# ivclab/CPG

Measured on AMD Instinct MI355X. Metric: images/sec per CPG train-prune-retrain cycle, VGG16 task-1, higher is better.
Workload: dtype f32; 1 GPU; configs[1]: VGG16-BN custom_vgg 224x224, task-1 CPG cycle (finetune -> prune 0.0->0.1 -> recovery, validate after every 20th train step), batch 256 per GPU; task=1, arch=vgg16, global_batch=256, per_gpu_batch=256, parallelism=dp1, epoch_steps=20

## Files before the change

### cpg_amd/_lib.py

```python
import ctypes
import os
import sys

import torch

_HERE = os.path.dirname(os.path.abspath(__file__))
LIB_PATH = os.environ.get('CPG_HIP_LIB') or os.path.join(_HERE, 'lib', 'libcpg_hip.so')

ABI_VERSION = 3
CPG_OK = 0
CPG_E_KRANGE = 2
CPG_E_INVALID = -1
MODE_FINETUNE = 0
MODE_PRUNE = 1



class ConvDesc(ctypes.Structure):
    _fields_ = [(n, ctypes.c_int32) for n in
                ('N', 'C', 'H', 'W', 'K', 'R', 'S', 'stride_h', 'stride_w', 'pad_h', 'pad_w', 'dil_h', 'dil_w', 'groups')]


class PruneResult(ctypes.Structure):
    _fields_ = [('n_candidates', ctypes.c_int64), ('k', ctypes.c_int64), ('n_released', ctypes.c_int64),
# ... 26 lines not shown
assert ctypes.sizeof(ResampleItem) == ctypes.sizeof(TensorItem) == 48

_vp, _int, _i32, _i64, _sz, _f32, _f64 = (ctypes.c_void_p, ctypes.c_int, ctypes.c_int32, ctypes.c_int64, ctypes.c_size_t, ctypes.c_float,
                                         ctypes.c_double)
_desc = ctypes.POINTER(ConvDesc)
_SIGNATURES = {
    'cpg_version': (_int, []),
    'cpg_set_shared_chip_hint': (_int, [_i32]),
    'cpg_get_shared_chip_hint': (_i32, []),
    'cpg_set_option': (_int, [ctypes.c_char_p, _i32]),
    'cpg_get_option': (_int, [ctypes.c_char_p, ctypes.POINTER(_i32)]),
    'cpg_last_error': (ctypes.c_char_p, []),
    'cpg_binarize_mask_weight': (_int, [_vp, _vp, _f32, _vp, _i64, _vp]),
    'cpg_conv2d_workspace_bytes': (_sz, [_desc]),
    'cpg_conv2d_fwd': (_int, [_desc, _vp, _vp, _vp, _f32, _vp, _vp, _vp, _sz, _vp]),
    'cpg_conv2d_dgrad': (_int, [_desc, _vp, _vp, _vp, _f32, _vp, _vp, _sz, _vp]),
    'cpg_conv2d_dgrad_add_supported': (_i32, [_desc]),
    'cpg_conv2d_dgrad_add': (_int, [_desc, _vp, _vp, _vp, _f32, _vp, _vp, _vp, _sz, _vp]),
    'cpg_conv2d_wgrad': (_int, [_desc, _vp, _vp, _vp, _vp, _f32, _vp, _vp, _vp, _vp, _sz, _vp]),
    'cpg_conv2d_pack_bytes': (_sz, [_desc, _i32]),
    'cpg_conv2d_pack': (_int, [_desc, _vp, _vp, _f32, _i32, _vp, _sz, _i32, _vp, _sz, _vp]),
    'cpg_conv2d_use_packed': (_int, [_vp, _sz]),
    'cpg_bn_relu_bwd_reduce': (_int, [_vp] * 9 + [_i32] * 3 + [_vp, _sz, _vp]),
    'cpg_conv2d_wgrad_rider_supported': (_i32, [_desc]),
    'cpg_conv2d_wgrad_attach_bn_bwd': (_int, [_vp] * 4 + [_i32] * 3),
    'cpg_linear_workspace_bytes': (_sz, [_i32, _i32, _i32]),
    'cpg_linear_fwd': (_int, [_vp, _vp, _vp, _f32, _vp, _vp, _i32, _i32, _i32, _vp, _sz, _vp]),
    'cpg_linear_dgrad': (_int, [_vp, _vp, _vp, _f32, _vp, _i32, _i32, _i32, _vp, _sz, _vp]),
    'cpg_linear_wgrad': (_int, [_vp, _vp, _vp, _vp, _f32, _vp, _vp, _vp, _i32, _i32, _i32, _vp, _sz, _vp]),
    'cpg_route_grads': (_int, [_vp, _vp, _vp, _i32, _f32, _vp, _i32, _i64, _vp]),
    'cpg_rank_prune_workspace_bytes': (_sz, []),
    'cpg_rank_prune': (_int, [_vp, _vp, _i32, _f64, _i64, _vp, _vp, _sz, _vp]),
    'cpg_rank_prune_zero': (_int, [_vp, _vp, _i32, _f64, _i64, _vp, _vp, _sz, _vp]),
    'cpg_mask_hist': (_int, [_vp, _vp, _i32, _i64, _vp, _vp]),
    'cpg_apply_mask': (_int, [_vp, _vp, _i32, _i64, _vp]),
    'cpg_zero_pruned': (_int, [_vp, _vp, _i64, _vp]),
    'cpg_claim_free': (_int, [_vp, _i32, _i64, _vp]),
    'cpg_owned_num_blocks': (_i64, [_i64]),
    'cpg_owned_block_counts': (_int, [_vp, _i32, _i32, _i64, _vp, _vp]),
    'cpg_pack_owned': (_int, [_vp, _vp, _i32, _i32, _i64, _vp, _vp, _vp]),
    'cpg_unpack_owned': (_int, [_vp, _vp, _i32, _i32, _i64, _vp, _vp, _vp]),
    'cpg_sgd_route_step': (_int, [_vp, _vp, _vp, _vp, _i32, _f32, _f32, _f32, _i32, _i32, _i64, _vp]),
    'cpg_multi_tensor_max': (_i32, []),
    'cpg_sgd_route_step_multi': (_int, [ctypes.POINTER(SgdItem), _i32, _i32, _f32, _f32, _f32, _i32, _i32, _vp]),
    'cpg_adam_route_step_multi': (_int, [ctypes.POINTER(AdamItem), _i32, _i32, _i32, _f64, _f64, _f64, _f64, _i32, _vp]),
    'cpg_sgd_route_zero_step': (_int, [_vp, _vp, _vp, _vp, _i32, _f32, _f32, _f32, _i32, _i32, _i64, _vp]),
    'cpg_sgd_route_zero_step_multi': (_int, [ctypes.POINTER(SgdItem), _i32, _i32, _f32, _f32, _f32, _i32, _i32, _vp]),
    'cpg_adam_route_step': (_int, [_vp, _vp, _vp, _vp, _vp, _i32, _i32, _f64, _f64, _f64, _f64, _i32, _i64, _vp]),
    'cpg_bn_workspace_bytes': (_sz, [_i32, _i32, _i32]),
    'cpg_bn_relu_fwd_train': (_int, [_vp, _vp, _vp, _f32, _f32, _vp, _vp, _vp, _vp, _vp, _i32, _i32, _i32, _i32, _vp, _sz, _vp]),
    'cpg_bn_relu_fwd_eval': (_int, [_vp, _vp, _vp, _vp, _vp, _vp, _i32, _i32, _i32, _i32, _vp]),
    'cpg_bn_relu_pool_fwd': (_int, [_vp, _vp, _vp, _f32, _f32, _vp, _vp, _vp, _vp, _vp, _i32, _i32, _i32, _i32, _i32, _vp, _sz, _vp]),
    'cpg_bn_relu_pool_bwd': (_int, [_vp, _vp, _vp, _vp, _vp, _vp, _vp, _vp, _vp, _i32, _i32, _i32, _i32, _i32, _vp, _sz, _vp]),
    'cpg_bn_relu_bwd': (_int, [_vp, _vp, _vp, _vp, _vp, _vp, _vp, _vp, _vp, _i32, _i32, _i32, _i32, _i32, _vp, _sz, _vp]),
    'cpg_conv2d_winograd': (_i32, [_desc, _i32]),
    'cpg_conv2d_bnstats_tiles': (_i32, [_desc]),
    'cpg_conv2d_fwd_bnstats': (_int, [_desc, _vp, _vp, _vp, _f32, _vp, _vp, _vp, _sz, _vp, _sz, _vp]),
    'cpg_conv2d_fwd_bn_eval_supported': (_i32, [_desc]),
    'cpg_conv2d_fwd_bn_eval': (_int, [_desc, _vp, _vp, _vp, _f32, _vp, _vp, _vp, _vp, _vp, _f32, _i32, _vp, _vp, _vp, _sz, _vp]),
    'cpg_conv2d_bf16_supported': (_i32, [_desc]),
    'cpg_conv2d_bf16_workspace_bytes': (_sz, [_desc]),
    'cpg_conv2d_fwd_bf16': (_int, [_desc, _vp, _vp, _vp, _f32, _vp, _vp, _vp, _sz, _vp]),
    'cpg_conv2d_wgrad_bf16_supported': (_i32, [_desc]),
    'cpg_conv2d_wgrad_bf16_workspace_bytes': (_sz, [_desc]),
    'cpg_conv2d_wgrad_bf16': (_int, [_desc, _vp, _vp, _vp, _vp, _f32, _vp, _vp, _vp, _sz, _vp]),
    'cpg_conv2d_fwd_bf16x3': (_int, [_desc, _vp, _vp, _vp, _f32, _vp, _vp, _vp, _sz, _vp]),
    'cpg_conv2d_dgrad_bf16x3': (_int, [_desc, _vp, _vp, _vp, _f32, _vp, _vp, _sz, _vp]),
    'cpg_conv2d_wgrad_bf16x3': (_int, [_desc, _vp, _vp, _vp, _vp, _f32, _vp, _vp, _vp, _sz, _vp]),
    'cpg_conv2d_dgrad_bf16': (_int, [_desc, _vp, _vp, _vp, _f32, _vp, _vp, _sz, _vp]),
    'cpg_conv2d_dgrad_bnbwd_tiles': (_i32, [_desc]),
    'cpg_conv2d_dgrad_bnbwd': (_int, [_desc, _vp, _vp, _vp, _f32, _vp, _vp, _vp, _vp, _vp, _vp, _vp, _sz, _vp, _sz, _vp]),
    'cpg_bn_bwd_from_partials': (_int, [_vp, _i32, _vp, _vp, _vp, _vp, _vp, _vp, _vp, _vp, _vp, _i32, _i32, _i32, _vp, _sz, _vp]),
    'cpg_bn_bwd_finalize_partials': (_int, [_vp, _i32, _i32, _i32, _i32, _vp, _vp, _vp, _vp]),
    'cpg_stem_bn_supported': (_i32, [_desc]),
    'cpg_stem_bn_tiles': (_i32, [_desc]),
    'cpg_stem_bn_stats': (_int, [_desc, _vp, _vp, _vp, _f32, _vp, _vp, _sz, _vp]),
    'cpg_stem_bn_relu_fwd': (_int, [_desc, _vp, _vp, _vp, _f32, _vp, _vp, _vp, _vp, _vp, _vp, _vp]),
    'cpg_stem_bn_relu_bwd_reduce': (_int, [_desc, _vp, _vp, _vp, _f32, _vp, _vp, _vp, _vp, _vp, _vp, _vp, _sz, _vp]),
    'cpg_stem_bn_relu_bwd_apply': (_int, [_desc, _vp, _vp, _vp, _f32, _vp, _vp, _vp, _vp, _vp, _vp, _vp, _vp, _vp]),
    'cpg_stem_bn_wgrad_workspace': (_sz, [_desc]),
    'cpg_stem_bn_relu_bwd_wgrad': (_int, [_desc, _vp, _vp, _vp, _f32, _vp, _vp, _vp, _vp, _vp, _vp, _vp, _vp, _vp, _vp, _sz, _vp]),
    'cpg_bn_stats_finalize_count': (_int, [_vp, _i32, _i32, _i32, _i32, _f32, _f32, _vp, _vp, _vp, _vp, _vp, _vp]),
    'cpg_bn_stats_finalize': (_int, [_vp, _i32, _i32, _i32, _i32, _f32, _f32, _vp, _vp, _vp, _vp, _vp]),
    'cpg_bn_add_relu_mask_bytes': (_sz, [_i32, _i32, _i32]),
    'cpg_bn_add_relu_fwd': (_int, [_vp, _vp, _vp, _vp, _f32, _f32, _vp, _vp, _vp, _vp, _vp, _i32, _i32, _i32, _i32, _vp, _sz, _vp, _vp]),
    'cpg_bn_relu_pool3_supported': (_i32, [_i32, _i32]),
    'cpg_bn_relu_pool3_fwd': (_int, [_vp] * 6 + [_i32] * 4 + [_vp]),
    'cpg_bn_relu_pool3_bwd': (_int, [_vp] * 9 + [_i32] * 5 + [_vp, _sz, _vp]),
    'cpg_bn_add_relu_bwd': (_int, [_vp] * 11 + [_i32] * 4 + [_vp, _sz, _vp, _vp]),
    'cpg_prelu_fwd': (_int, [_vp, _vp, _vp, _vp, _i32, _i32, _i32, _i32, _vp]),
    'cpg_prelu_bwd_bias': (_int, [_vp] * 6 + [_i32] * 4 + [_vp, _sz, _vp]),
    'cpg_prelu_workspace_bytes': (_sz, [_i32, _i32, _i32]),
    'cpg_prelu_bwd': (_int, [_vp, _vp, _vp, _vp, _vp, _i32, _i32, _i32, _i32, _vp, _sz, _vp]),
    'cpg_image_resample_workspace_bytes': (_sz, [ctypes.POINTER(ResampleItem), _i32]),
    'cpg_image_resample': (_int, [_vp, _i64, ctypes.POINTER(ResampleItem), _i32, _vp, _i64, _vp, _sz, _vp]),
    'cpg_image_to_tensor': (_int, [_vp, _i64, ctypes.POINTER(TensorItem), _i32, _i32, _i32, ctypes.POINTER(_f32), ctypes.POINTER(_f32), _vp,
                                           _i64, _vp]),
    'cpg_pair_distance': (_int, [_vp, _i64, _vp, _i64, _i64, _i32, _i32, _vp, _vp, _vp]),
    'cpg_pair_sweep': (_int, [_vp, _vp, _i64, ctypes.POINTER(_f64), _i32, _i32, _vp, _vp, _vp]),
    'cpg_loss_heads_workspace_bytes': (_sz, [_i32, _i32, _i32]),
    'cpg_softmax_xent_fwd': (_int, [_vp, _vp, _vp, _i32, _i32, _vp, _vp, _vp, _sz, _vp]),
    'cpg_softmax_xent_fwd_bwd': (_int, [_vp, _vp, _vp, _vp, _i32, _i32, _vp, _vp, _vp, _vp, _sz, _vp]),
    'cpg_angle_head_fwd': (_int, [_vp, _vp, _vp, _i32, _i32, _i32, _i32, _f32, _f64] + [_vp] * 7 + [_sz, _vp]),
    'cpg_angle_head_bwd': (_int, [_vp] * 7 + [_i32, _i32, _i32, _i32, _f32, _f64, _vp, _vp, _vp, _sz, _vp]),
}
EXPORTS = tuple(_SIGNATURES)
# ... 116 lines not shown
```

### cpg_amd/csrc/bn_kernels.hip

```cpp
#include "cpg_common.h"

using namespace cpg;

namespace {

constexpr int kThreads = 256;

struct BnDims {
    int N, C, HW;
    int slices;
    int imgs_per_slice;
};

__device__ __forceinline__ double block_sum(double v, double *red) {
    for (int off = 32; off > 0; off >>= 1) v += __shfl_down(v, off);
    const int w = threadIdx.x >> 6, l = threadIdx.x & 63;
    __syncthreads();
    if (l == 0) red[w] = v;
    __syncthreads();
    return red[0] + red[1] + red[2] + red[3];
}

template <class F, class FL>
__device__ __forceinline__ void walk_planes(int P, int n0, int n1, F &&f, FL &&flush) {
// ... 513 lines not shown
    float *coef = (float *)(partial + (size_t)C * d.slices * 2);
    hipLaunchKernelGGL(k_bn_bwd_reduce<true>, dim3(C, d.slices), dim3(kThreads), 0, stream, x, gy, d, mean, invstd, gamma, beta, partial);
    hipLaunchKernelGGL(k_bn_bwd_finalize, dim3((C + 63) / 64), dim3(64), 0, stream, partial, d, dgamma, dbeta, coef, table, mean, invstd,
                       gamma, beta);
    CPG_CHECK_LAUNCH("cpg_bn_relu_bwd_reduce");
    return CPG_OK;
}

extern "C" int cpg_bn_add_relu_bwd(const float *x, const float *out, const float *gy, const float *gamma, const float *beta,
                                   const float *mean, const float *invstd, float *gx, float *gz, float *dgamma, float *dbeta, int32_t N,
                                   int32_t C, int32_t HW, int32_t train, void *ws, size_t ws_bytes, void *stream_v, const uint8_t *relu_mask) {
    BnDims d;
    int rc = make_dims(N, C, HW, d);
    if (rc) return rc;
    CPG_REQUIRE(x && (out || relu_mask) && gy && gamma && beta && mean && invstd && gx && gz && dgamma && dbeta && ws, "cpg_bn_add_relu_bwd: null pointer");
    if (relu_mask != nullptr)
        CPG_REQUIRE(HW % 4 == 0 && ((((uintptr_t)x) | ((uintptr_t)gy) | ((uintptr_t)gz)) & 15) == 0,
                    "cpg_bn_add_relu_bwd: the ReLU mask needs 4 | HW and 16-byte aligned tensors");
    if (ws_bytes < cpg_bn_workspace_bytes(N, C, HW)) return fail(CPG_E_WORKSPACE, "cpg_bn_add_relu_bwd: workspace too small");
    hipStream_t stream = (hipStream_t)stream_v;
    double *partial = (double *)ws;
    float *coef = (float *)(partial + (size_t)C * d.slices * 2);
    hipLaunchKernelGGL((k_bn_bwd_reduce<false, true>), dim3(C, d.slices), dim3(kThreads), 0, stream, x, gy, d, mean, invstd, gamma, beta,
                       partial, out, gz, relu_mask);
    hipLaunchKernelGGL(k_bn_bwd_finalize, dim3((C + 63) / 64), dim3(64), 0, stream, partial, d, dgamma, dbeta, coef);
    if (train) launch_bwd_apply<false, true>(d, x, gz, gx, mean, invstd, gamma, beta, coef, stream);
    else launch_bwd_apply<false, false>(d, x, gz, gx, mean, invstd, gamma, beta, coef, stream);
    CPG_CHECK_LAUNCH("cpg_bn_add_relu_bwd");
    return CPG_OK;
}

namespace {

struct PoolDims {
    int H, W, OW, wins;
};

struct Win {
    float v[4];
};
__device__ __forceinline__ Win load_win(const float *plane, int W, int pr, int pc) {
    const float2 a = *reinterpret_cast<const float2 *>(plane + (2 * pr) * W + 2 * pc);
    const float2 b = *reinterpret_cast<const float2 *>(plane + (2 * pr + 1) * W + 2 * pc);
    return Win{{a.x, a.y, b.x, b.y}};
}
__device__ __forceinline__ int win_argmax(const float (&y)[4]) {
    int idx = 0;
#pragma unroll
    for (int k = 1; k < 4; ++k)
        if (y[k] > y[idx]) idx = k;
    return idx;
}

template <int GROUP>
__global__ __launch_bounds__(kThreads) void k_bnp_apply(const float *__restrict__ x, float *__restrict__ yp, BnDims d, PoolDims p,
                                                        const float *__restrict__ mean, const float *__restrict__ invstd,
                                                        const float *__restrict__ gamma, const float *__restrict__ beta) {
    const int64_t planes = (int64_t)d.N * d.C;
    const int gl = threadIdx.x % GROUP;
    const int64_t g0 = (int64_t)blockIdx.x * (kThreads / GROUP) + threadIdx.x / GROUP;
    const int64_t gstride = (int64_t)gridDim.x * (kThreads / GROUP);
    for (int64_t pl = g0; pl < planes; pl += gstride) {
        const int c = (int)(pl % d.C);
        const float m = mean[c], is = invstd[c], ga = gamma[c], be = beta[c];
        const float *plane = x + pl * d.HW;
        float *out = yp + pl * p.wins;
        for (int i = gl; i < p.wins; i += GROUP) {
            const int pr = i / p.OW, pc = i - pr * p.OW;
            const Win w = load_win(plane, p.W, pr, pc);
            float best = 0.0f;
#pragma unroll
            for (int k = 0; k < 4; ++k) best = fmaxf(best, bn_affine(w.v[k], m, is, ga, be));
            out[i] = best;
        }
    }
}

__global__ __launch_bounds__(kThreads) void k_bnp_bwd_reduce(const float *__restrict__ x, const float *__restrict__ gp, BnDims d,
                                                             PoolDims p, const float *__restrict__ mean,
                                                             const float *__restrict__ invstd, const float *__restrict__ gamma,
                                                             const float *__restrict__ beta, double *__restrict__ partial) {
    __shared__ double red[4];
    const int c = blockIdx.x, s = blockIdx.y;
    const int n0 = s * d.imgs_per_slice, n1 = min(d.N, n0 + d.imgs_per_slice);
    const float m = mean[c], is = invstd[c], ga = gamma[c], be = beta[c];
    double dsg = 0.0, dsgx = 0.0;
    float sg = 0.f, sgx = 0.f;
    walk_planes(p.wins, n0, n1, [&](int n, int wi) {
        const int pr = wi / p.OW, pc = wi - pr * p.OW;
        const int64_t pl = (int64_t)n * d.C + c;
        const Win w = load_win(x + pl * d.HW, p.W, pr, pc);
        const float g = gp[pl * p.wins + wi];
        float y[4];
#pragma unroll
        for (int k = 0; k < 4; ++k) y[k] = bn_affine(w.v[k], m, is, ga, be);
        const int idx = win_argmax(y);
        if (y[idx] > 0.f) {
            sg += g;
            sgx += g * ((w.v[idx] - m) * is);
        }
    }, [&]() {
        dsg += (double)sg; dsgx += (double)sgx; sg = 0.f; sgx = 0.f;
    });
    const double t0 = block_sum(dsg, red);
    const double t1 = block_sum(dsgx, red);
    if (threadIdx.x == 0) {
        partial[((int64_t)c * d.slices + s) * 2 + 0] = t0;
        partial[((int64_t)c * d.slices + s) * 2 + 1] = t1;
    }
}

template <bool TRAIN, int GROUP>
__global__ __launch_bounds__(kThreads) void k_bnp_bwd_apply(const float *__restrict__ x, const float *__restrict__ gp,
                                                            float *__restrict__ gx, BnDims d, PoolDims p,
                                                            const float *__restrict__ mean, const float *__restrict__ invstd,
                                                            const float *__restrict__ gamma, const float *__restrict__ beta,
                                                            const float *__restrict__ coef) {
    const int64_t planes = (int64_t)d.N * d.C;
    const int gl = threadIdx.x % GROUP;
    const int64_t g0 = (int64_t)blockIdx.x * (kThreads / GROUP) + threadIdx.x / GROUP;
    const int64_t gstride = (int64_t)gridDim.x * (kThreads / GROUP);
    for (int64_t pl = g0; pl < planes; pl += gstride) {
        const int c = (int)(pl % d.C);
        const float m = mean[c], is = invstd[c], ga = gamma[c], be = beta[c];
        const float mg = TRAIN ? coef[2 * c] : 0.f, mgx = TRAIN ? coef[2 * c + 1] : 0.f;
        const float scale = is * ga;
        const float *plane = x + pl * d.HW;
        float *gplane = gx + pl * d.HW;
        for (int i = gl; i < p.wins; i += GROUP) {
            const int pr = i / p.OW, pc = i - pr * p.OW;
            const Win w = load_win(plane, p.W, pr, pc);
            float y[4], r[4];
#pragma unroll
            for (int k = 0; k < 4; ++k) y[k] = bn_affine(w.v[k], m, is, ga, be);
            const int idx = win_argmax(y);
            const float g = (y[idx] > 0.f) ? gp[pl * p.wins + i] : 0.f;
#pragma unroll
            for (int k = 0; k < 4; ++k) {
                const float gk = (k == idx) ? g : 0.f;
                r[k] = TRAIN ? (gk - mg - ((w.v[k] - m) * is) * mgx) * scale : gk * scale;
            }
            *reinterpret_cast<float2 *>(gplane + (2 * pr) * p.W + 2 * pc) = make_float2(r[0], r[1]);
            *reinterpret_cast<float2 *>(gplane + (2 * pr + 1) * p.W + 2 * pc) = make_float2(r[2], r[3]);
        }
    }
}

int make_pool(int H, int W, PoolDims &p) {
    CPG_REQUIRE(H > 0 && W > 0 && (H % 2) == 0 && (W % 2) == 0, "bn_relu_pool: H and W must be even (got %d x %d)", H, W);
    p.H = H; p.W = W; p.OW = W / 2; p.wins = (H / 2) * (W / 2);
    return CPG_OK;
}
unsigned pool_grid(const BnDims &d, const PoolDims &p, bool wave) {
    int64_t groups = (int64_t)d.N * d.C;
    if (wave) groups = (groups + 3) / 4;
    const int64_t cap = (int64_t)kCUs * 16;
    return (unsigned)(groups < cap ? groups : cap);
}

}

extern "C" int cpg_bn_relu_pool_fwd(const float *x, const float *gamma, const float *beta, float eps, float momentum,
                                    float *running_mean, float *running_var, float *mean, float *invstd, float *y_pooled,
                                    int32_t N, int32_t C, int32_t H, int32_t W, int32_t train, void *ws, size_t ws_bytes,
                                    void *stream_v) {
    BnDims d;
    PoolDims p;
    int rc = make_dims(N, C, H * W, d);
    if (rc) return rc;
    rc = make_pool(H, W, p);
    if (rc) return rc;
    CPG_REQUIRE(x && gamma && beta && mean && invstd && y_pooled, "cpg_bn_relu_pool_fwd: null pointer");
    CPG_REQUIRE((((uintptr_t)x) & 7) == 0, "cpg_bn_relu_pool_fwd: x must be 8-byte aligned");
    hipStream_t stream = (hipStream_t)stream_v;
    if (train) {
        CPG_REQUIRE(ws != nullptr, "cpg_bn_relu_pool_fwd: workspace required in training mode");
        if (ws_bytes < cpg_bn_workspace_bytes(N, C, H * W)) return fail(CPG_E_WORKSPACE, "cpg_bn_relu_pool_fwd: workspace too small");
        double *partial = (double *)ws;
        hipLaunchKernelGGL(k_bn_stats, dim3(C, d.slices), dim3(kThreads), 0, stream, x, d, partial);
        hipLaunchKernelGGL(k_bn_finalize, dim3((C + 63) / 64), dim3(64), 0, stream, partial, d, eps, momentum, mean, invstd,
                           running_mean, running_var);
    }
    const bool wave = p.wins < 1024;
    if (wave)
        hipLaunchKernelGGL(k_bnp_apply<64>, dim3(pool_grid(d, p, true)), dim3(kThreads), 0, stream, x, y_pooled, d, p, mean, invstd, gamma, beta);
    else
        hipLaunchKernelGGL(k_bnp_apply<256>, dim3(pool_grid(d, p, false)), dim3(kThreads), 0, stream, x, y_pooled, d, p, mean, invstd, gamma, beta);
    CPG_CHECK_LAUNCH("cpg_bn_relu_pool_fwd");
    return CPG_OK;
}

extern "C" int cpg_bn_relu_pool_bwd(const float *x, const float *g_pooled, const float *gamma, const float *beta,
                                    const float *mean, const float *invstd, float *gx, float *dgamma, float *dbeta, int32_t N,
                                    int32_t C, int32_t H, int32_t W, int32_t train, void *ws, size_t ws_bytes, void *stream_v) {
    BnDims d;
    PoolDims p;
    int rc = make_dims(N, C, H * W, d);
    if (rc) return rc;
    rc = make_pool(H, W, p);
    if (rc) return rc;
    CPG_REQUIRE(x && g_pooled && gamma && beta && mean && invstd && gx && dgamma && dbeta && ws, "cpg_bn_relu_pool_bwd: null pointer");
    CPG_REQUIRE((((uintptr_t)x) & 7) == 0 && (((uintptr_t)gx) & 7) == 0, "cpg_bn_relu_pool_bwd: x / gx must be 8-byte aligned");
    if (ws_bytes < cpg_bn_workspace_bytes(N, C, H * W)) return fail(CPG_E_WORKSPACE, "cpg_bn_relu_pool_bwd: workspace too small");
    hipStream_t stream = (hipStream_t)stream_v;
    double *partial = (double *)ws;
    float *coef = (float *)(partial + (size_t)C * d.slices * 2);
    hipLaunchKernelGGL(k_bnp_bwd_reduce, dim3(C, d.slices), dim3(kThreads), 0, stream, x, g_pooled, d, p, mean, invstd, gamma, beta, partial);
    hipLaunchKernelGGL(k_bn_bwd_finalize, dim3((C + 63) / 64), dim3(64), 0, stream, partial, d, dgamma, dbeta, coef);
    const bool wave = p.wins < 1024;
    const dim3 grid(pool_grid(d, p, wave)), block(kThreads);
    if (wave && train) hipLaunchKernelGGL((k_bnp_bwd_apply<true, 64>), grid, block, 0, stream, x, g_pooled, gx, d, p, mean, invstd, gamma, beta, coef);
    else if (wave) hipLaunchKernelGGL((k_bnp_bwd_apply<false, 64>), grid, block, 0, stream, x, g_pooled, gx, d, p, mean, invstd, gamma, beta, coef);
    else if (train) hipLaunchKernelGGL((k_bnp_bwd_apply<true, 256>), grid, block, 0, stream, x, g_pooled, gx, d, p, mean, invstd, gamma, beta, coef);
    else hipLaunchKernelGGL((k_bnp_bwd_apply<false, 256>), grid, block, 0, stream, x, g_pooled, gx, d, p, mean, invstd, gamma, beta, coef);
    CPG_CHECK_LAUNCH("cpg_bn_relu_pool_bwd");
    return CPG_OK;
}


namespace {

struct Pool3Dims {
    int H, W, OH, OW;
    int strips;
};
constexpr int kPool3SR = 8;

__device__ __forceinline__ void pool3_stage(const float *__restrict__ plane, float *zs, const Pool3Dims &p, int r0, int nrows, float m,
                                            float is, float ga, float be) {
    const int h0 = 2 * r0 - 1;
    const int lo = max(h0, 0), hi = min(h0 + nrows, p.H);
    const float *src = plane + lo * p.W;
    float *dst = zs + (lo - h0) * p.W;
    const int n = (hi - lo) * p.W;
    if ((n & 3) == 0 && (((uintptr_t)src) & 15) == 0 && (((lo - h0) * p.W) & 3) == 0) {
        for (int i = threadIdx.x; i < n / 4; i += kThreads) {
            float4 v = reinterpret_cast<const float4 *>(src)[i];
            v.x = fmaxf(bn_affine(v.x, m, is, ga, be), 0.f); v.y = fmaxf(bn_affine(v.y, m, is, ga, be), 0.f);
            v.z = fmaxf(bn_affine(v.z, m, is, ga, be), 0.f); v.w = fmaxf(bn_affine(v.w, m, is, ga, be), 0.f);
            reinterpret_cast<float4 *>(dst)[i] = v;
        }
    } else {
        for (int i = threadIdx.x; i < n; i += kThreads) dst[i] = fmaxf(bn_affine(src[i], m, is, ga, be), 0.f);
    }
}

__device__ __forceinline__ int pool3_argmax(const float *zs, const Pool3Dims &p, int h0, int ph, int pw, float *best_out = nullptr) {
    float best = -1.0f;
    int arg = 0;
#pragma unroll
    for (int r = 0; r < 3; ++r) {
        const int h = 2 * ph - 1 + r;
        if ((unsigned)h >= (unsigned)p.H) continue;
#pragma unroll
        for (int q = 0; q < 3; ++q) {
            const int w = 2 * pw - 1 + q;
            if ((unsigned)w >= (unsigned)p.W) continue;
            const float v = zs[(h - h0) * p.W + w];
            if (v > best || v != v) best = v, arg = h * p.W + w;
        }
    }
    if (best_out) *best_out = best;
    return arg;
}

__global__ __launch_bounds__(kThreads) void k_bnp3_apply(const float *__restrict__ x, float *__restrict__ y, BnDims d, Pool3Dims p,
                                                         const float *__restrict__ mean, const float *__restrict__ invstd,
                                                         const float *__restrict__ gamma, const float *__restrict__ beta) {
    extern __shared__ __attribute__((aligned(16))) float dyn[];
// ... 349 lines not shown
```

### cpg_amd/csrc/conv3x3_wino_wgrad.hip

```cpp
#include <algorithm>
#include "cpg_dispatch.h"
#include "wino_acc.h"

using namespace cpg;

namespace {

typedef float f32x2 __attribute__((ext_vector_type(2)));
typedef int i32x4 __attribute__((ext_vector_type(4)));
typedef int i32x2 __attribute__((ext_vector_type(2)));

constexpr int WW_XR = 34, WW_XC = 138, WW_GR = 30, WW_GC = 62;
constexpr int WW_XS = 32 * WW_XC;
constexpr int WW_STAGE = WW_XS + 32 * WW_GC;

struct WwGeom {
    int N, C, K, H, W;
    int th, tw, nseg;
    unsigned nstages;
    int nkb, ncb, nsplit;
    unsigned su;
    int span;
    int xcd;
};

struct WwRider {
    const float *y, *gz;
    float *gy;
    const float *table;
    int C, HW, p4, ipp;
    int bytes;
    unsigned total, per;
};

#ifdef WG_TIMING
__device__ unsigned long long ww_dbg[65536 * 8];
#define WW_STAMP(i) do { if (lane == 0 && u < 65536) ww_dbg[u * 8 + (i)] = wall_clock64(); } while (0)
#else
#define WW_STAMP(i)
#endif
template <bool NARROW, int GS = 0, int RI = 0>
__global__ __launch_bounds__(256) __attribute__((amdgpu_waves_per_eu(1, 1)))
void k_wgw(WwGeom g, const float *__restrict__ x, const float *__restrict__ gy, float *__restrict__ part, WwRider rd) {
    static_assert(GS == 0 || GS == 4 || (!NARROW && GS == 2), "shared staging: groups of 4 waves, or 2 on wide maps");
    static_assert(RI == 0 || (GS == 4 && RI <= 2), "the rider's schedule slots exist in the GS = 4 bodies: one or two items per stage");
    constexpr int NG = GS ? 4 / GS : 0;
    constexpr bool TS = GS == 4;
    constexpr int WW_BS = 2 * 16 * 64;
    __shared__ __attribute__((aligned(16))) float smem_all[GS ? NG * 2 * WW_XS + 4 * 32 * WW_GC + (TS ? WW_BS : 0) : 4 * WW_STAGE];
    const int tid = threadIdx.x, lane = tid & 63, wave = __builtin_amdgcn_readfirstlane(tid >> 6);
    const int li = lane & 31, lh = lane >> 5;
    const int gw = GS ? wave % GS : 0;
    float *smem = GS ? smem_all : smem_all + wave * WW_STAGE;
    float *xb0 = GS ? smem_all + (wave / (GS ? GS : 1)) * 2 * WW_XS : smem;
    float *xb1 = GS ? xb0 + WW_XS : smem;
    float *gyp = GS ? smem_all + NG * 2 * WW_XS + wave * 32 * WW_GC : smem + WW_XS;
    float *bsh = smem_all + NG * 2 * WW_XS + 4 * 32 * WW_GC;
    const int HW = g.H * g.W;
    const unsigned npairs = (unsigned)(g.nkb * g.ncb);
    const unsigned u = (g.xcd ? xcd_remap(blockIdx.x, gridDim.x) : blockIdx.x) * 4 + wave;
    if (u >= npairs * (unsigned)g.nsplit) return;
    const unsigned pair = u % npairs, split = u / npairs;
    const int kb = (int)(pair % (unsigned)g.nkb), cb = (int)(pair / (unsigned)g.nkb);
    const int k0 = __builtin_amdgcn_readfirstlane(min(kb * 32, g.K - 32)), c0 = __builtin_amdgcn_readfirstlane(min(cb * 32, g.C - 32));
    const unsigned s_begin = split * g.su;
    const int nst = (int)min(g.su, g.nstages - s_begin);
    WW_STAMP(0);
#ifdef WG_TIMING
    if (lane == 0 && u < 65536) ww_dbg[u * 8 + 6] = __builtin_amdgcn_s_getreg(63492), ww_dbg[u * 8 + 7] = __builtin_amdgcn_s_getreg(63508);
#endif
    const unsigned per_img = (unsigned)(g.th * g.nseg);
    int n = (int)(s_begin / per_img) * (NARROW ? 2 : 1);
    const unsigned r0 = s_begin % per_img;
    int ty = (int)(r0 / (unsigned)g.nseg), tseg = (int)(r0 % (unsigned)g.nseg);
    const int n0 = n;
    const int nimg_here = min(g.span, g.N - n0);
    const __amdgpu_buffer_rsrc_t srd_x = __builtin_amdgcn_make_buffer_rsrc(
        (void *)(x + (int64_t)n0 * g.C * HW - (g.W + 4)), 0, nimg_here * g.C * HW * 4 + (g.W + 4) * 4, 0x00020000);
    const __amdgpu_buffer_rsrc_t srd_g =
        __builtin_amdgcn_make_buffer_rsrc((void *)(gy + (int64_t)n0 * g.K * HW), 0, nimg_here * g.K * HW * 4, 0x00020000);

    constexpr int kOOR = (int)0x80000000;
    const int qd = min(lane & 7, 6), rem = lane >> 3;
    const int xrow = NARROW ? rem >> 1 : rem & 3, half = rem & 1;
    const int vx_const = NARROW ? (half * g.C * HW + xrow * g.W + gw * HW) * 4 + qd * 8 + 16
                                : ((rem >> 2) * HW + xrow * g.W + gw * 2 * HW) * 4 + qd * 16 + 16;
    const int vg_const = NARROW ? ((rem >> 2) * HW + half * g.K * HW + ((rem >> 1) & 1) * g.W) * 4 + qd * 8
                                : ((rem >> 1) * HW + (rem & 1) * g.W) * 4 + qd * 16;
    const int hside = lane & 1, hrow = (lane >> 1) & 3;
    const int vh_const = ((lane >> 3) * HW + hrow * g.W + gw * 8 * HW) * 4 + (hside ? 28 * 4 + 16 : 12);
    const int xw_addr = NARROW ? xrow * WW_XR + 16 * half + 2 + 2 * qd + gw * WW_XC : (rem >> 2) * WW_XC + xrow * WW_XR + 2 + 4 * qd + gw * 2 * WW_XC;
    const int gw_addr = NARROW ? (rem >> 2) * WW_GC + ((rem >> 1) & 1) * WW_GR + 14 * half + 2 * qd
                               : (rem >> 1) * WW_GC + (rem & 1) * WW_GR + 4 * qd;
    const int hw_addr = (lane >> 3) * WW_XC + hrow * WW_XR + (hside ? 30 : 1) + gw * 8 * WW_XC;
    if constexpr (NARROW) {
        for (int i = lane; i < 32 * 4 * 6; i += 64) {
            const int rowi = i / 6, col = i % 6;
            xb0[(rowi >> 2) * WW_XC + (rowi & 3) * WW_XR + (col >> 1) * 16 + (col & 1)] = 0.0f;
// ... 125 lines not shown
            const f32x2 own = *reinterpret_cast<const f32x2 *>(r);
            const f32x2 lo = *reinterpret_cast<const f32x2 *>(r - 2), hi = *reinterpret_cast<const f32x2 *>(r + 2);
            B[m * 4 + 0] = lo[1], B[m * 4 + 1] = own[0], B[m * 4 + 2] = own[1], B[m * 4 + 3] = hi[0];
        } else if (m == 4) {
            const f32x2 y0 = *reinterpret_cast<const f32x2 *>(gyp + gr_base + kKs * ks);
            const f32x2 y1 = *reinterpret_cast<const f32x2 *>(gyp + gr_base + kKs * ks + WW_GR);
            A[0] = y0[0], A[3] = y0[1], A[12] = y1[0], A[15] = y1[1];
        } else if (m < 7) {
#pragma unroll
            for (int j = 2 * (m - 5); j < 2 * (m - 5) + 2; ++j) {
                const float d0 = B[0 * 4 + j], d1 = B[1 * 4 + j], d2 = B[2 * 4 + j], d3 = B[3 * 4 + j];
                B[0 * 4 + j] = d0 - d2, B[1 * 4 + j] = d1 + d2, B[2 * 4 + j] = d2 - d1, B[3 * 4 + j] = d1 - d3;
                asm volatile("" : "+v"(B[0 * 4 + j]), "+v"(B[1 * 4 + j]), "+v"(B[2 * 4 + j]), "+v"(B[3 * 4 + j]));
            }
        } else if (m < 11) {
            const int i = m - 7;
            const float t0 = B[i * 4 + 0], t1 = B[i * 4 + 1], t2 = B[i * 4 + 2], t3 = B[i * 4 + 3];
            B[i * 4 + 0] = t0 - t2, B[i * 4 + 1] = t1 + t2, B[i * 4 + 2] = t2 - t1, B[i * 4 + 3] = t1 - t3;
            asm volatile("" : "+v"(B[i * 4 + 0]), "+v"(B[i * 4 + 1]), "+v"(B[i * 4 + 2]), "+v"(B[i * 4 + 3]));
        } else if (m == 11) {
            A[4] = A[0] + A[12], A[7] = A[3] + A[15], A[8] = A[0] - A[12], A[11] = A[3] - A[15];
            asm volatile("" : "+v"(A[4]), "+v"(A[7]), "+v"(A[8]), "+v"(A[11]));
        } else if (m == 12) {
            A[1] = A[0] + A[3], A[2] = A[0] - A[3], A[5] = A[4] + A[7], A[6] = A[4] - A[7];
            asm volatile("" : "+v"(A[1]), "+v"(A[2]), "+v"(A[5]), "+v"(A[6]));
        } else if (m == 13) {
            A[9] = A[8] + A[11], A[10] = A[8] - A[11], A[13] = A[12] + A[15], A[14] = A[12] - A[15];
            asm volatile("" : "+v"(A[9]), "+v"(A[10]), "+v"(A[13]), "+v"(A[14]));
        }
    };

    const int b_ra = wave == 0 ? 0 : (wave == 2 ? 2 : 1), b_rb = wave == 3 ? 3 : (wave == 2 ? 1 : 2);
    const float b_sg = wave == 1 ? 1.0f : -1.0f;
    float ta[4], tb[4];
    auto b_micro = [&](int m, int ks, int buf, float (&B)[16], const float *xb) {
        if (m < 2) {
            const float *r = xb + xr_base + kKs * ks + (m == 0 ? b_ra : b_rb) * WW_XR;
            const f32x2 own = *reinterpret_cast<const f32x2 *>(r);
            const f32x2 lo = *reinterpret_cast<const f32x2 *>(r - 2), hi = *reinterpret_cast<const f32x2 *>(r + 2);
            float (&t)[4] = m == 0 ? ta : tb;
            t[0] = lo[1], t[1] = own[0], t[2] = own[1], t[3] = hi[0];
        } else if (m == 2) {
            float e[4];
#pragma unroll
            for (int j = 0; j < 4; ++j) e[j] = __builtin_fmaf(b_sg, tb[j], ta[j]);
            f32x4 v;
            v[0] = e[0] - e[2], v[1] = e[1] + e[2], v[2] = e[2] - e[1], v[3] = e[1] - e[3];
            *reinterpret_cast<f32x4 *>(bsh + ((buf * 4 + wave) * 64 + lane) * 4) = v;
        } else {
            const f32x4 v = *reinterpret_cast<const f32x4 *>(bsh + ((buf * 4 + (m - 3)) * 64 + lane) * 4);
            B[(m - 3) * 4 + 0] = v[0], B[(m - 3) * 4 + 1] = v[1], B[(m - 3) * 4 + 2] = v[2], B[(m - 3) * 4 + 3] = v[3];
        }
    };
    constexpr int RJ = RI > 0 ? RI : 1;
    typedef const float __attribute__((address_space(4))) *ww_cptr;
    const __amdgpu_buffer_rsrc_t srd_ry = __builtin_amdgcn_make_buffer_rsrc((void *)rd.y, 0, rd.bytes, 0x00020000);
    const __amdgpu_buffer_rsrc_t srd_rz = __builtin_amdgcn_make_buffer_rsrc((void *)rd.gz, 0, rd.bytes, 0x00020000);
    const __amdgpu_buffer_rsrc_t srd_ro = __builtin_amdgcn_make_buffer_rsrc((void *)rd.gy, 0, rd.bytes, 0x00020000);
    unsigned rq = 0, rq_end = 0, r_plane = 0;
    int r_sub = 0, r_c = 0;
    if constexpr (RI > 0) {
        rq = __builtin_amdgcn_readfirstlane(min(u * rd.per, rd.total));
        rq_end = min(rq + rd.per, rd.total);
        r_plane = rq / (unsigned)rd.ipp, r_sub = (int)(rq % (unsigned)rd.ipp), r_c = (int)(r_plane % (unsigned)rd.C);
    }
    f32x4 r_y[RJ], r_z[RJ];
    float r_t[RJ][7];
    int r_vo[RJ], r_so[RJ];
    auto r_micro = [&](int j, int m) {
        if (m == 0) {
            const int left = rq < rq_end ? rd.p4 - r_sub * 64 : 0;
            r_vo[j] = lane < left ? lane * 16 : kOOR;
            r_so[j] = (int)(r_plane * (unsigned)rd.HW + (unsigned)r_sub * 256u) * 4;
            r_y[j] = __builtin_bit_cast(f32x4, __builtin_amdgcn_raw_buffer_load_b128(srd_ry, r_vo[j], r_so[j], 0));
        } else if (m == 1) {
            r_z[j] = __builtin_bit_cast(f32x4, __builtin_amdgcn_raw_buffer_load_b128(srd_rz, r_vo[j], r_so[j], 0));
            ww_cptr t = (ww_cptr)rd.table + r_c * 8;
#pragma unroll
            for (int k = 0; k < 7; ++k) r_t[j][k] = t[k];
            if (rq < rq_end) {
                ++rq;
                if (++r_sub == rd.ipp) {
                    r_sub = 0, ++r_plane;
                    if (++r_c == rd.C) r_c = 0;
                }
            }
        } else {
            const int e = m - 2;
            r_y[j][e] = bn_bwd_apply_one<true, true>(r_y[j][e], r_z[j][e], r_t[j][0], r_t[j][1], r_t[j][2], r_t[j][3], r_t[j][4], r_t[j][5], r_t[j][6]);
            if (m == 5) __builtin_amdgcn_raw_buffer_store_b128(__builtin_bit_cast(i32x4, r_y[j]), srd_ro, r_vo[j], r_so[j], 0);
        }
    };
    (void)r_micro;
    WW_STAMP(1);
    WACC_ZERO_ALL();
    float A0[16], B0[16], A1[16], B1[16];
    stage_offsets();
    if constexpr (GS > 0) {
#pragma unroll
        for (int i = 0; i < NSI; ++i) g_load_s(i);
#pragma unroll
        for (int i = 0; i < NSI; ++i) w_store_s(i, xb0);
        __syncthreads();
    } else {
#pragma unroll
        for (int i = 0; i < (NARROW ? 48 : 28); ++i) g_load(i, 0);
#pragma unroll
        for (int i = 0; i < (NARROW ? 48 : 28); ++i) w_store(i);
    }
    advance_stage();
    if constexpr (TS) {
#pragma unroll
        for (int m = 0; m < 3; ++m) b_micro(m, 0, 0, B0, xb0);
        WACC_LDS_BARRIER();
#pragma unroll
        for (int m = 3; m < 7; ++m) b_micro(m, 0, 0, B0, xb0);
        t_micro(4, 0, A0, B0, xb0), t_micro(11, 0, A0, B0, xb0), t_micro(12, 0, A0, B0, xb0), t_micro(13, 0, A0, B0, xb0);
    } else {
#pragma unroll
        for (int m = 0; m < 14; ++m) t_micro(m, 0, A0, B0, xb0);
    }

    WW_STAMP(2);
    for (int st = 0; st < nst; st += 2) {
        if constexpr (NARROW && GS == 4) {
        {
            const int nst_idx = st + 0 + 1;
            (void)nst_idx;
            WACC_MMA_0(A0[0], B0[0]); b_micro(0, 1, 1, B1, xb0); WACC_FENCE();
            WACC_MMA_1(A0[1], B0[1]); b_micro(1, 1, 1, B1, xb0); WACC_FENCE();
            WACC_MMA_2(A0[2], B0[2]); t_micro(4, 1, A1, B1, xb0); WACC_FENCE();
            WACC_MMA_3(A0[3], B0[3]); b_micro(2, 1, 1, B1, xb0); WACC_FENCE();
            WACC_MMA_4(A0[4], B0[4]); t_micro(11, 1, A1, B1, xb0); WACC_FENCE();
            WACC_MMA_5(A0[5], B0[5]); t_micro(12, 1, A1, B1, xb0); WACC_FENCE();
            WACC_MMA_6(A0[6], B0[6]); t_micro(13, 1, A1, B1, xb0); WACC_FENCE();
            WACC_MMA_7(A0[7], B0[7]); WACC_LDS_BARRIER(); WACC_FENCE();
            WACC_MMA_8(A0[8], B0[8]); b_micro(3, 1, 1, B1, xb0); WACC_FENCE();
            WACC_MMA_9(A0[9], B0[9]); b_micro(4, 1, 1, B1, xb0); WACC_FENCE();
            WACC_MMA_10(A0[10], B0[10]); b_micro(5, 1, 1, B1, xb0); WACC_FENCE();
            WACC_MMA_11(A0[11], B0[11]); b_micro(6, 1, 1, B1, xb0); WACC_FENCE();
            WACC_MMA_12(A0[12], B0[12]); if constexpr (RI > 0) r_micro(0, 0); WACC_FENCE();
            WACC_MMA_13(A0[13], B0[13]); if constexpr (RI > 0) r_micro(0, 1); WACC_FENCE();
            WACC_MMA_14(A0[14], B0[14]); if constexpr (RI > 1) r_micro(1, 0); WACC_FENCE();
            WACC_MMA_15(A0[15], B0[15]); if constexpr (RI > 1) r_micro(1, 1); WACC_FENCE();
            WACC_MMA_0(A1[0], B1[0]); b_micro(0, 2, 0, B0, xb0); g_load_s(0); WACC_FENCE();
            WACC_MMA_1(A1[1], B1[1]); b_micro(1, 2, 0, B0, xb0); g_load_s(1); WACC_FENCE();
            WACC_MMA_2(A1[2], B1[2]); t_micro(4, 2, A0, B0, xb0); g_load_s(2); WACC_FENCE();
            WACC_MMA_3(A1[3], B1[3]); b_micro(2, 2, 0, B0, xb0); g_load_s(3); WACC_FENCE();
            WACC_MMA_4(A1[4], B1[4]); t_micro(11, 2, A0, B0, xb0); g_load_s(4); WACC_FENCE();
            WACC_MMA_5(A1[5], B1[5]); t_micro(12, 2, A0, B0, xb0); g_load_s(5); WACC_FENCE();
            WACC_MMA_6(A1[6], B1[6]); t_micro(13, 2, A0, B0, xb0); g_load_s(6); WACC_FENCE();
            WACC_MMA_7(A1[7], B1[7]); WACC_LDS_BARRIER(); g_load_s(7); WACC_FENCE();
            WACC_MMA_8(A1[8], B1[8]); b_micro(3, 2, 0, B0, xb0); g_load_s(8); WACC_FENCE();
            WACC_MMA_9(A1[9], B1[9]); b_micro(4, 2, 0, B0, xb0); g_load_s(9); WACC_FENCE();
            WACC_MMA_10(A1[10], B1[10]); b_micro(5, 2, 0, B0, xb0); g_load_s(10); WACC_FENCE();
            WACC_MMA_11(A1[11], B1[11]); b_micro(6, 2, 0, B0, xb0); g_load_s(11); WACC_FENCE();
            WACC_MMA_12(A1[12], B1[12]); g_load_s(12); WACC_FENCE();
            WACC_MMA_13(A1[13], B1[13]); g_load_s(13); WACC_FENCE();
            WACC_MMA_14(A1[14], B1[14]); g_load_s(14); WACC_FENCE();
            WACC_MMA_15(A1[15], B1[15]); g_load_s(15); WACC_FENCE();
            WACC_MMA_0(A0[0], B0[0]); b_micro(0, 3, 1, B1, xb0); g_load_s(16); WACC_FENCE();
            WACC_MMA_1(A0[1], B0[1]); b_micro(1, 3, 1, B1, xb0); g_load_s(17); WACC_FENCE();
            WACC_MMA_2(A0[2], B0[2]); t_micro(4, 3, A1, B1, xb0); g_load_s(18); WACC_FENCE();
            WACC_MMA_3(A0[3], B0[3]); b_micro(2, 3, 1, B1, xb0); g_load_s(19); WACC_FENCE();
            WACC_MMA_4(A0[4], B0[4]); t_micro(11, 3, A1, B1, xb0); g_load_s(20); WACC_FENCE();
            WACC_MMA_5(A0[5], B0[5]); t_micro(12, 3, A1, B1, xb0); g_load_s(21); WACC_FENCE();
            WACC_MMA_6(A0[6], B0[6]); t_micro(13, 3, A1, B1, xb0); g_load_s(22); WACC_FENCE();
            WACC_MMA_7(A0[7], B0[7]); WACC_LDS_BARRIER(); g_load_s(23); WACC_FENCE();
            WACC_MMA_8(A0[8], B0[8]); b_micro(3, 3, 1, B1, xb0); WACC_FENCE();
            WACC_MMA_9(A0[9], B0[9]); b_micro(4, 3, 1, B1, xb0); WACC_FENCE();
            WACC_MMA_10(A0[10], B0[10]); b_micro(5, 3, 1, B1, xb0); WACC_FENCE();
            WACC_MMA_11(A0[11], B0[11]); b_micro(6, 3, 1, B1, xb0); WACC_FENCE();
            WACC_MMA_12(A0[12], B0[12]); ; WACC_FENCE();
            WACC_MMA_13(A0[13], B0[13]); ; WACC_FENCE();
            WACC_MMA_14(A0[14], B0[14]); ; WACC_FENCE();
            WACC_MMA_15(A0[15], B0[15]); ; WACC_FENCE();
            WACC_MMA_0(A1[0], B1[0]); b_micro(0, 4, 0, B0, xb0); WACC_FENCE();
            WACC_MMA_1(A1[1], B1[1]); b_micro(1, 4, 0, B0, xb0); WACC_FENCE();
            WACC_MMA_2(A1[2], B1[2]); t_micro(4, 4, A0, B0, xb0); WACC_FENCE();
            WACC_MMA_3(A1[3], B1[3]); b_micro(2, 4, 0, B0, xb0); WACC_FENCE();
            WACC_MMA_4(A1[4], B1[4]); t_micro(11, 4, A0, B0, xb0); WACC_FENCE();
            WACC_MMA_5(A1[5], B1[5]); t_micro(12, 4, A0, B0, xb0); WACC_FENCE();
            WACC_MMA_6(A1[6], B1[6]); t_micro(13, 4, A0, B0, xb0); WACC_FENCE();
            WACC_MMA_7(A1[7], B1[7]); WACC_LDS_BARRIER(); WACC_FENCE();
            WACC_MMA_8(A1[8], B1[8]); b_micro(3, 4, 0, B0, xb0); WACC_FENCE();
            WACC_MMA_9(A1[9], B1[9]); b_micro(4, 4, 0, B0, xb0); WACC_FENCE();
            WACC_MMA_10(A1[10], B1[10]); b_micro(5, 4, 0, B0, xb0); WACC_FENCE();
            WACC_MMA_11(A1[11], B1[11]); b_micro(6, 4, 0, B0, xb0); WACC_FENCE();
            WACC_MMA_12(A1[12], B1[12]); ; WACC_FENCE();
            WACC_MMA_13(A1[13], B1[13]); ; WACC_FENCE();
            WACC_MMA_14(A1[14], B1[14]); ; WACC_FENCE();
            WACC_MMA_15(A1[15], B1[15]); ; WACC_FENCE();
            WACC_MMA_0(A0[0], B0[0]); b_micro(0, 5, 1, B1, xb0); WACC_FENCE();
            WACC_MMA_1(A0[1], B0[1]); b_micro(1, 5, 1, B1, xb0); WACC_FENCE();
            WACC_MMA_2(A0[2], B0[2]); t_micro(4, 5, A1, B1, xb0); WACC_FENCE();
            WACC_MMA_3(A0[3], B0[3]); b_micro(2, 5, 1, B1, xb0); WACC_FENCE();
            WACC_MMA_4(A0[4], B0[4]); t_micro(11, 5, A1, B1, xb0); WACC_FENCE();
            WACC_MMA_5(A0[5], B0[5]); t_micro(12, 5, A1, B1, xb0); WACC_FENCE();
            WACC_MMA_6(A0[6], B0[6]); t_micro(13, 5, A1, B1, xb0); WACC_FENCE();
            WACC_MMA_7(A0[7], B0[7]); WACC_LDS_BARRIER(); WACC_FENCE();
            WACC_MMA_8(A0[8], B0[8]); b_micro(3, 5, 1, B1, xb0); WACC_FENCE();
            WACC_MMA_9(A0[9], B0[9]); b_micro(4, 5, 1, B1, xb0); WACC_FENCE();
            WACC_MMA_10(A0[10], B0[10]); b_micro(5, 5, 1, B1, xb0); WACC_FENCE();
            WACC_MMA_11(A0[11], B0[11]); b_micro(6, 5, 1, B1, xb0); WACC_FENCE();
            WACC_MMA_12(A0[12], B0[12]); if constexpr (RI > 0) r_micro(0, 2); WACC_FENCE();
            WACC_MMA_13(A0[13], B0[13]); if constexpr (RI > 0) r_micro(0, 3); WACC_FENCE();
            WACC_MMA_14(A0[14], B0[14]); if constexpr (RI > 0) r_micro(0, 4); WACC_FENCE();
            WACC_MMA_15(A0[15], B0[15]); if constexpr (RI > 0) r_micro(0, 5); WACC_FENCE();
            WACC_MMA_0(A1[0], B1[0]); b_micro(0, 6, 0, B0, xb0); WACC_FENCE();
            WACC_MMA_1(A1[1], B1[1]); b_micro(1, 6, 0, B0, xb0); WACC_FENCE();
            WACC_MMA_2(A1[2], B1[2]); t_micro(4, 6, A0, B0, xb0); WACC_FENCE();
            WACC_MMA_3(A1[3], B1[3]); b_micro(2, 6, 0, B0, xb0); WACC_FENCE();
            WACC_MMA_4(A1[4], B1[4]); t_micro(11, 6, A0, B0, xb0); WACC_FENCE();
            WACC_MMA_5(A1[5], B1[5]); t_micro(12, 6, A0, B0, xb0); WACC_FENCE();
            WACC_MMA_6(A1[6], B1[6]); t_micro(13, 6, A0, B0, xb0); WACC_FENCE();
            WACC_MMA_7(A1[7], B1[7]); WACC_LDS_BARRIER(); WACC_FENCE();
            WACC_MMA_8(A1[8], B1[8]); b_micro(3, 6, 0, B0, xb0); WACC_FENCE();
            WACC_MMA_9(A1[9], B1[9]); b_micro(4, 6, 0, B0, xb0); WACC_FENCE();
            WACC_MMA_10(A1[10], B1[10]); b_micro(5, 6, 0, B0, xb0); WACC_FENCE();
            WACC_MMA_11(A1[11], B1[11]); b_micro(6, 6, 0, B0, xb0); WACC_FENCE();
            WACC_MMA_12(A1[12], B1[12]); if constexpr (RI > 1) r_micro(1, 2); WACC_FENCE();
            WACC_MMA_13(A1[13], B1[13]); if constexpr (RI > 1) r_micro(1, 3); WACC_FENCE();
            WACC_MMA_14(A1[14], B1[14]); if constexpr (RI > 1) r_micro(1, 4); WACC_FENCE();
            WACC_MMA_15(A1[15], B1[15]); if constexpr (RI > 1) r_micro(1, 5); WACC_FENCE();
            WACC_MMA_0(A0[0], B0[0]); w_store_s(0, xb1); w_store_s(1, xb1); w_store_s(2, xb1); w_store_s(3, xb1); WACC_FENCE();
            WACC_MMA_1(A0[1], B0[1]); w_store_s(4, xb1); w_store_s(5, xb1); w_store_s(6, xb1); w_store_s(7, xb1); WACC_FENCE();
            WACC_MMA_2(A0[2], B0[2]); w_store_s(8, xb1); w_store_s(9, xb1); w_store_s(10, xb1); w_store_s(11, xb1); WACC_FENCE();
            WACC_MMA_3(A0[3], B0[3]); w_store_s(12, xb1); w_store_s(13, xb1); w_store_s(14, xb1); w_store_s(15, xb1); WACC_FENCE();
            WACC_MMA_4(A0[4], B0[4]); w_store_s(16, xb1); w_store_s(17, xb1); w_store_s(18, xb1); w_store_s(19, xb1); WACC_FENCE();
            WACC_MMA_5(A0[5], B0[5]); w_store_s(20, xb1); w_store_s(21, xb1); w_store_s(22, xb1); w_store_s(23, xb1); WACC_FENCE();
            WACC_MMA_6(A0[6], B0[6]); WACC_LDS_BARRIER(); WACC_FENCE();
            WACC_MMA_7(A0[7], B0[7]); b_micro(0, 0, 1, B1, xb1); WACC_FENCE();
            WACC_MMA_8(A0[8], B0[8]); b_micro(1, 0, 1, B1, xb1); WACC_FENCE();
            WACC_MMA_9(A0[9], B0[9]); t_micro(4, 0, A1, B1, xb1); WACC_FENCE();
            WACC_MMA_10(A0[10], B0[10]); b_micro(2, 0, 1, B1, xb1); WACC_FENCE();
            WACC_MMA_11(A0[11], B0[11]); t_micro(11, 0, A1, B1, xb1); t_micro(12, 0, A1, B1, xb1); t_micro(13, 0, A1, B1, xb1); WACC_FENCE();
            WACC_MMA_12(A0[12], B0[12]); WACC_LDS_BARRIER(); WACC_FENCE();
            WACC_MMA_13(A0[13], B0[13]); b_micro(3, 0, 1, B1, xb1); b_micro(4, 0, 1, B1, xb1); WACC_FENCE();
            WACC_MMA_14(A0[14], B0[14]); b_micro(5, 0, 1, B1, xb1); b_micro(6, 0, 1, B1, xb1); WACC_FENCE();
            WACC_MMA_15(A0[15], B0[15]); ; WACC_FENCE();
            advance_stage();
        }
        {
            const int nst_idx = st + 1 + 1;
            (void)nst_idx;
            if (st + 1 >= nst) break;
            WACC_MMA_0(A1[0], B1[0]); b_micro(0, 1, 0, B0, xb1); WACC_FENCE();
            WACC_MMA_1(A1[1], B1[1]); b_micro(1, 1, 0, B0, xb1); WACC_FENCE();
            WACC_MMA_2(A1[2], B1[2]); t_micro(4, 1, A0, B0, xb1); WACC_FENCE();
            WACC_MMA_3(A1[3], B1[3]); b_micro(2, 1, 0, B0, xb1); WACC_FENCE();
            WACC_MMA_4(A1[4], B1[4]); t_micro(11, 1, A0, B0, xb1); WACC_FENCE();
            WACC_MMA_5(A1[5], B1[5]); t_micro(12, 1, A0, B0, xb1); WACC_FENCE();
            WACC_MMA_6(A1[6], B1[6]); t_micro(13, 1, A0, B0, xb1); WACC_FENCE();
            WACC_MMA_7(A1[7], B1[7]); WACC_LDS_BARRIER(); WACC_FENCE();
            WACC_MMA_8(A1[8], B1[8]); b_micro(3, 1, 0, B0, xb1); WACC_FENCE();
            WACC_MMA_9(A1[9], B1[9]); b_micro(4, 1, 0, B0, xb1); WACC_FENCE();
            WACC_MMA_10(A1[10], B1[10]); b_micro(5, 1, 0, B0, xb1); WACC_FENCE();
            WACC_MMA_11(A1[11], B1[11]); b_micro(6, 1, 0, B0, xb1); WACC_FENCE();
            WACC_MMA_12(A1[12], B1[12]); if constexpr (RI > 0) r_micro(0, 0); WACC_FENCE();
            WACC_MMA_13(A1[13], B1[13]); if constexpr (RI > 0) r_micro(0, 1); WACC_FENCE();
            WACC_MMA_14(A1[14], B1[14]); if constexpr (RI > 1) r_micro(1, 0); WACC_FENCE();
            WACC_MMA_15(A1[15], B1[15]); if constexpr (RI > 1) r_micro(1, 1); WACC_FENCE();
            WACC_MMA_0(A0[0], B0[0]); b_micro(0, 2, 1, B1, xb1); g_load_s(0); WACC_FENCE();
            WACC_MMA_1(A0[1], B0[1]); b_micro(1, 2, 1, B1, xb1); g_load_s(1); WACC_FENCE();
            WACC_MMA_2(A0[2], B0[2]); t_micro(4, 2, A1, B1, xb1); g_load_s(2); WACC_FENCE();
            WACC_MMA_3(A0[3], B0[3]); b_micro(2, 2, 1, B1, xb1); g_load_s(3); WACC_FENCE();
            WACC_MMA_4(A0[4], B0[4]); t_micro(11, 2, A1, B1, xb1); g_load_s(4); WACC_FENCE();
            WACC_MMA_5(A0[5], B0[5]); t_micro(12, 2, A1, B1, xb1); g_load_s(5); WACC_FENCE();
            WACC_MMA_6(A0[6], B0[6]); t_micro(13, 2, A1, B1, xb1); g_load_s(6); WACC_FENCE();
            WACC_MMA_7(A0[7], B0[7]); WACC_LDS_BARRIER(); g_load_s(7); WACC_FENCE();
            WACC_MMA_8(A0[8], B0[8]); b_micro(3, 2, 1, B1, xb1); g_load_s(8); WACC_FENCE();
            WACC_MMA_9(A0[9], B0[9]); b_micro(4, 2, 1, B1, xb1); g_load_s(9); WACC_FENCE();
            WACC_MMA_10(A0[10], B0[10]); b_micro(5, 2, 1, B1, xb1); g_load_s(10); WACC_FENCE();
            WACC_MMA_11(A0[11], B0[11]); b_micro(6, 2, 1, B1, xb1); g_load_s(11); WACC_FENCE();
            WACC_MMA_12(A0[12], B0[12]); g_load_s(12); WACC_FENCE();
            WACC_MMA_13(A0[13], B0[13]); g_load_s(13); WACC_FENCE();
            WACC_MMA_14(A0[14], B0[14]); g_load_s(14); WACC_FENCE();
            WACC_MMA_15(A0[15], B0[15]); g_load_s(15); WACC_FENCE();
            WACC_MMA_0(A1[0], B1[0]); b_micro(0, 3, 0, B0, xb1); g_load_s(16); WACC_FENCE();
            WACC_MMA_1(A1[1], B1[1]); b_micro(1, 3, 0, B0, xb1); g_load_s(17); WACC_FENCE();
            WACC_MMA_2(A1[2], B1[2]); t_micro(4, 3, A0, B0, xb1); g_load_s(18); WACC_FENCE();
            WACC_MMA_3(A1[3], B1[3]); b_micro(2, 3, 0, B0, xb1); g_load_s(19); WACC_FENCE();
            WACC_MMA_4(A1[4], B1[4]); t_micro(11, 3, A0, B0, xb1); g_load_s(20); WACC_FENCE();
            WACC_MMA_5(A1[5], B1[5]); t_micro(12, 3, A0, B0, xb1); g_load_s(21); WACC_FENCE();
            WACC_MMA_6(A1[6], B1[6]); t_micro(13, 3, A0, B0, xb1); g_load_s(22); WACC_FENCE();
            WACC_MMA_7(A1[7], B1[7]); WACC_LDS_BARRIER(); g_load_s(23); WACC_FENCE();
            WACC_MMA_8(A1[8], B1[8]); b_micro(3, 3, 0, B0, xb1); WACC_FENCE();
            WACC_MMA_9(A1[9], B1[9]); b_micro(4, 3, 0, B0, xb1); WACC_FENCE();
            WACC_MMA_10(A1[10], B1[10]); b_micro(5, 3, 0, B0, xb1); WACC_FENCE();
            WACC_MMA_11(A1[11], B1[11]); b_micro(6, 3, 0, B0, xb1); WACC_FENCE();
            WACC_MMA_12(A1[12], B1[12]); ; WACC_FENCE();
            WACC_MMA_13(A1[13], B1[13]); ; WACC_FENCE();
            WACC_MMA_14(A1[14], B1[14]); ; WACC_FENCE();
            WACC_MMA_15(A1[15], B1[15]); ; WACC_FENCE();
            WACC_MMA_0(A0[0], B0[0]); b_micro(0, 4, 1, B1, xb1); WACC_FENCE();
            WACC_MMA_1(A0[1], B0[1]); b_micro(1, 4, 1, B1, xb1); WACC_FENCE();
            WACC_MMA_2(A0[2], B0[2]); t_micro(4, 4, A1, B1, xb1); WACC_FENCE();
            WACC_MMA_3(A0[3], B0[3]); b_micro(2, 4, 1, B1, xb1); WACC_FENCE();
            WACC_MMA_4(A0[4], B0[4]); t_micro(11, 4, A1, B1, xb1); WACC_FENCE();
            WACC_MMA_5(A0[5], B0[5]); t_micro(12, 4, A1, B1, xb1); WACC_FENCE();
            WACC_MMA_6(A0[6], B0[6]); t_micro(13, 4, A1, B1, xb1); WACC_FENCE();
            WACC_MMA_7(A0[7], B0[7]); WACC_LDS_BARRIER(); WACC_FENCE();
            WACC_MMA_8(A0[8], B0[8]); b_micro(3, 4, 1, B1, xb1); WACC_FENCE();
            WACC_MMA_9(A0[9], B0[9]); b_micro(4, 4, 1, B1, xb1); WACC_FENCE();
            WACC_MMA_10(A0[10], B0[10]); b_micro(5, 4, 1, B1, xb1); WACC_FENCE();
            WACC_MMA_11(A0[11], B0[11]); b_micro(6, 4, 1, B1, xb1); WACC_FENCE();
            WACC_MMA_12(A0[12], B0[12]); ; WACC_FENCE();
            WACC_MMA_13(A0[13], B0[13]); ; WACC_FENCE();
            WACC_MMA_14(A0[14], B0[14]); ; WACC_FENCE();
            WACC_MMA_15(A0[15], B0[15]); ; WACC_FENCE();
            WACC_MMA_0(A1[0], B1[0]); b_micro(0, 5, 0, B0, xb1); WACC_FENCE();
            WACC_MMA_1(A1[1], B1[1]); b_micro(1, 5, 0, B0, xb1); WACC_FENCE();
            WACC_MMA_2(A1[2], B1[2]); t_micro(4, 5, A0, B0, xb1); WACC_FENCE();
            WACC_MMA_3(A1[3], B1[3]); b_micro(2, 5, 0, B0, xb1); WACC_FENCE();
            WACC_MMA_4(A1[4], B1[4]); t_micro(11, 5, A0, B0, xb1); WACC_FENCE();
            WACC_MMA_5(A1[5], B1[5]); t_micro(12, 5, A0, B0, xb1); WACC_FENCE();
            WACC_MMA_6(A1[6], B1[6]); t_micro(13, 5, A0, B0, xb1); WACC_FENCE();
            WACC_MMA_7(A1[7], B1[7]); WACC_LDS_BARRIER(); WACC_FENCE();
            WACC_MMA_8(A1[8], B1[8]); b_micro(3, 5, 0, B0, xb1); WACC_FENCE();
            WACC_MMA_9(A1[9], B1[9]); b_micro(4, 5, 0, B0, xb1); WACC_FENCE();
            WACC_MMA_10(A1[10], B1[10]); b_micro(5, 5, 0, B0, xb1); WACC_FENCE();
            WACC_MMA_11(A1[11], B1[11]); b_micro(6, 5, 0, B0, xb1); WACC_FENCE();
            WACC_MMA_12(A1[12], B1[12]); if constexpr (RI > 0) r_micro(0, 2); WACC_FENCE();
            WACC_MMA_13(A1[13], B1[13]); if constexpr (RI > 0) r_micro(0, 3); WACC_FENCE();
            WACC_MMA_14(A1[14], B1[14]); if constexpr (RI > 0) r_micro(0, 4); WACC_FENCE();
            WACC_MMA_15(A1[15], B1[15]); if constexpr (RI > 0) r_micro(0, 5); WACC_FENCE();
            WACC_MMA_0(A0[0], B0[0]); b_micro(0, 6, 1, B1, xb1); WACC_FENCE();
            WACC_MMA_1(A0[1], B0[1]); b_micro(1, 6, 1, B1, xb1); WACC_FENCE();
            WACC_MMA_2(A0[2], B0[2]); t_micro(4, 6, A1, B1, xb1); WACC_FENCE();
            WACC_MMA_3(A0[3], B0[3]); b_micro(2, 6, 1, B1, xb1); WACC_FENCE();
            WACC_MMA_4(A0[4], B0[4]); t_micro(11, 6, A1, B1, xb1); WACC_FENCE();
            WACC_MMA_5(A0[5], B0[5]); t_micro(12, 6, A1, B1, xb1); WACC_FENCE();
            WACC_MMA_6(A0[6], B0[6]); t_micro(13, 6, A1, B1, xb1); WACC_FENCE();
            WACC_MMA_7(A0[7], B0[7]); WACC_LDS_BARRIER(); WACC_FENCE();
            WACC_MMA_8(A0[8], B0[8]); b_micro(3, 6, 1, B1, xb1); WACC_FENCE();
            WACC_MMA_9(A0[9], B0[9]); b_micro(4, 6, 1, B1, xb1); WACC_FENCE();
            WACC_MMA_10(A0[10], B0[10]); b_micro(5, 6, 1, B1, xb1); WACC_FENCE();
            WACC_MMA_11(A0[11], B0[11]); b_micro(6, 6, 1, B1, xb1); WACC_FENCE();
            WACC_MMA_12(A0[12], B0[12]); if constexpr (RI > 1) r_micro(1, 2); WACC_FENCE();
            WACC_MMA_13(A0[13], B0[13]); if constexpr (RI > 1) r_micro(1, 3); WACC_FENCE();
            WACC_MMA_14(A0[14], B0[14]); if constexpr (RI > 1) r_micro(1, 4); WACC_FENCE();
            WACC_MMA_15(A0[15], B0[15]); if constexpr (RI > 1) r_micro(1, 5); WACC_FENCE();
            WACC_MMA_0(A1[0], B1[0]); w_store_s(0, xb0); w_store_s(1, xb0); w_store_s(2, xb0); w_store_s(3, xb0); WACC_FENCE();
            WACC_MMA_1(A1[1], B1[1]); w_store_s(4, xb0); w_store_s(5, xb0); w_store_s(6, xb0); w_store_s(7, xb0); WACC_FENCE();
            WACC_MMA_2(A1[2], B1[2]); w_store_s(8, xb0); w_store_s(9, xb0); w_store_s(10, xb0); w_store_s(11, xb0); WACC_FENCE();
            WACC_MMA_3(A1[3], B1[3]); w_store_s(12, xb0); w_store_s(13, xb0); w_store_s(14, xb0); w_store_s(15, xb0); WACC_FENCE();
            WACC_MMA_4(A1[4], B1[4]); w_store_s(16, xb0); w_store_s(17, xb0); w_store_s(18, xb0); w_store_s(19, xb0); WACC_FENCE();
            WACC_MMA_5(A1[5], B1[5]); w_store_s(20, xb0); w_store_s(21, xb0); w_store_s(22, xb0); w_store_s(23, xb0); WACC_FENCE();
            WACC_MMA_6(A1[6], B1[6]); WACC_LDS_BARRIER(); WACC_FENCE();
            WACC_MMA_7(A1[7], B1[7]); b_micro(0, 0, 0, B0, xb0); WACC_FENCE();
            WACC_MMA_8(A1[8], B1[8]); b_micro(1, 0, 0, B0, xb0); WACC_FENCE();
            WACC_MMA_9(A1[9], B1[9]); t_micro(4, 0, A0, B0, xb0); WACC_FENCE();
            WACC_MMA_10(A1[10], B1[10]); b_micro(2, 0, 0, B0, xb0); WACC_FENCE();
            WACC_MMA_11(A1[11], B1[11]); t_micro(11, 0, A0, B0, xb0); t_micro(12, 0, A0, B0, xb0); t_micro(13, 0, A0, B0, xb0); WACC_FENCE();
            WACC_MMA_12(A1[12], B1[12]); WACC_LDS_BARRIER(); WACC_FENCE();
            WACC_MMA_13(A1[13], B1[13]); b_micro(3, 0, 0, B0, xb0); b_micro(4, 0, 0, B0, xb0); WACC_FENCE();
            WACC_MMA_14(A1[14], B1[14]); b_micro(5, 0, 0, B0, xb0); b_micro(6, 0, 0, B0, xb0); WACC_FENCE();
            WACC_MMA_15(A1[15], B1[15]); ; WACC_FENCE();
            advance_stage();
        }

        } else if constexpr (NARROW) {
        {
            const int nst_idx = st + 0 + 1;
            (void)nst_idx;
            WACC_MMA_0(A0[0], B0[0]); t_micro(0, 1, A1, B1, xb0); WACC_FENCE();
            WACC_MMA_1(A0[1], B0[1]); t_micro(1, 1, A1, B1, xb0); WACC_FENCE();
            WACC_MMA_2(A0[2], B0[2]); t_micro(2, 1, A1, B1, xb0); WACC_FENCE();
            WACC_MMA_3(A0[3], B0[3]); t_micro(3, 1, A1, B1, xb0); WACC_FENCE();
            WACC_MMA_4(A0[4], B0[4]); t_micro(4, 1, A1, B1, xb0); WACC_FENCE();
            WACC_MMA_5(A0[5], B0[5]); t_micro(5, 1, A1, B1, xb0); WACC_FENCE();
            WACC_MMA_6(A0[6], B0[6]); t_micro(6, 1, A1, B1, xb0); WACC_FENCE();
            WACC_MMA_7(A0[7], B0[7]); t_micro(7, 1, A1, B1, xb0); WACC_FENCE();
            WACC_MMA_8(A0[8], B0[8]); t_micro(8, 1, A1, B1, xb0); WACC_FENCE();
            WACC_MMA_9(A0[9], B0[9]); t_micro(9, 1, A1, B1, xb0); WACC_FENCE();
            WACC_MMA_10(A0[10], B0[10]); t_micro(10, 1, A1, B1, xb0); WACC_FENCE();
            WACC_MMA_11(A0[11], B0[11]); t_micro(11, 1, A1, B1, xb0); WACC_FENCE();
            WACC_MMA_12(A0[12], B0[12]); t_micro(12, 1, A1, B1, xb0); WACC_FENCE();
            WACC_MMA_13(A0[13], B0[13]); t_micro(13, 1, A1, B1, xb0); WACC_FENCE();
            WACC_MMA_14(A0[14], B0[14]); ; WACC_FENCE();
            WACC_MMA_15(A0[15], B0[15]); ; WACC_FENCE();
            WACC_MMA_0(A1[0], B1[0]); t_micro(0, 2, A0, B0, xb0); g_load(0, nst_idx); WACC_FENCE();
            WACC_MMA_1(A1[1], B1[1]); t_micro(1, 2, A0, B0, xb0); g_load(1, nst_idx); WACC_FENCE();
            WACC_MMA_2(A1[2], B1[2]); t_micro(2, 2, A0, B0, xb0); g_load(2, nst_idx); WACC_FENCE();
            WACC_MMA_3(A1[3], B1[3]); t_micro(3, 2, A0, B0, xb0); g_load(3, nst_idx); WACC_FENCE();
            WACC_MMA_4(A1[4], B1[4]); t_micro(4, 2, A0, B0, xb0); g_load(4, nst_idx); WACC_FENCE();
            WACC_MMA_5(A1[5], B1[5]); t_micro(5, 2, A0, B0, xb0); g_load(5, nst_idx); WACC_FENCE();
            WACC_MMA_6(A1[6], B1[6]); t_micro(6, 2, A0, B0, xb0); g_load(6, nst_idx); WACC_FENCE();
            WACC_MMA_7(A1[7], B1[7]); t_micro(7, 2, A0, B0, xb0); g_load(7, nst_idx); WACC_FENCE();
            WACC_MMA_8(A1[8], B1[8]); t_micro(8, 2, A0, B0, xb0); g_load(8, nst_idx); WACC_FENCE();
            WACC_MMA_9(A1[9], B1[9]); t_micro(9, 2, A0, B0, xb0); g_load(9, nst_idx); WACC_FENCE();
            WACC_MMA_10(A1[10], B1[10]); t_micro(10, 2, A0, B0, xb0); g_load(10, nst_idx); WACC_FENCE();
            WACC_MMA_11(A1[11], B1[11]); t_micro(11, 2, A0, B0, xb0); g_load(11, nst_idx); WACC_FENCE();
            WACC_MMA_12(A1[12], B1[12]); t_micro(12, 2, A0, B0, xb0); g_load(12, nst_idx); WACC_FENCE();
            WACC_MMA_13(A1[13], B1[13]); t_micro(13, 2, A0, B0, xb0); g_load(13, nst_idx); WACC_FENCE();
// ... 166 lines not shown
            WACC_MMA_14(A1[14], B1[14]); ; WACC_FENCE();
            WACC_MMA_15(A1[15], B1[15]); ; WACC_FENCE();
            WACC_MMA_0(A0[0], B0[0]); t_micro(0, 6, A1, B1, xb1); WACC_FENCE();
            WACC_MMA_1(A0[1], B0[1]); t_micro(1, 6, A1, B1, xb1); WACC_FENCE();
            WACC_MMA_2(A0[2], B0[2]); t_micro(2, 6, A1, B1, xb1); WACC_FENCE();
            WACC_MMA_3(A0[3], B0[3]); t_micro(3, 6, A1, B1, xb1); WACC_FENCE();
            WACC_MMA_4(A0[4], B0[4]); t_micro(4, 6, A1, B1, xb1); WACC_FENCE();
            WACC_MMA_5(A0[5], B0[5]); t_micro(5, 6, A1, B1, xb1); WACC_FENCE();
            WACC_MMA_6(A0[6], B0[6]); t_micro(6, 6, A1, B1, xb1); WACC_FENCE();
            WACC_MMA_7(A0[7], B0[7]); t_micro(7, 6, A1, B1, xb1); WACC_FENCE();
            WACC_MMA_8(A0[8], B0[8]); t_micro(8, 6, A1, B1, xb1); WACC_FENCE();
            WACC_MMA_9(A0[9], B0[9]); t_micro(9, 6, A1, B1, xb1); WACC_FENCE();
            WACC_MMA_10(A0[10], B0[10]); t_micro(10, 6, A1, B1, xb1); WACC_FENCE();
            WACC_MMA_11(A0[11], B0[11]); t_micro(11, 6, A1, B1, xb1); WACC_FENCE();
            WACC_MMA_12(A0[12], B0[12]); t_micro(12, 6, A1, B1, xb1); WACC_FENCE();
            WACC_MMA_13(A0[13], B0[13]); t_micro(13, 6, A1, B1, xb1); WACC_FENCE();
            WACC_MMA_14(A0[14], B0[14]); ; WACC_FENCE();
            WACC_MMA_15(A0[15], B0[15]); ; WACC_FENCE();
            WACC_MMA_0(A1[0], B1[0]); w_store(0); w_store(1); w_store(2); w_store(3); w_store(4); w_store(5); w_store(6); WACC_FENCE();
            WACC_MMA_1(A1[1], B1[1]); w_store(7); w_store(8); w_store(9); w_store(10); w_store(11); w_store(12); w_store(13); WACC_FENCE();
            WACC_MMA_2(A1[2], B1[2]); w_store(14); w_store(15); w_store(16); w_store(17); w_store(18); w_store(19); w_store(20); WACC_FENCE();
            WACC_MMA_3(A1[3], B1[3]); w_store(21); w_store(22); w_store(23); w_store(24); w_store(25); w_store(26); w_store(27); WACC_FENCE();
            WACC_MMA_4(A1[4], B1[4]); w_store(28); w_store(29); w_store(30); w_store(31); w_store(32); w_store(33); w_store(34); WACC_FENCE();
            WACC_MMA_5(A1[5], B1[5]); w_store(35); w_store(36); w_store(37); w_store(38); w_store(39); w_store(40); w_store(41); WACC_FENCE();
            WACC_MMA_6(A1[6], B1[6]); w_store(42); w_store(43); w_store(44); w_store(45); w_store(46); w_store(47); WACC_FENCE();
            WACC_MMA_7(A1[7], B1[7]); t_micro(0, 0, A0, B0, xb0); t_micro(1, 0, A0, B0, xb0); WACC_FENCE();
            WACC_MMA_8(A1[8], B1[8]); t_micro(2, 0, A0, B0, xb0); t_micro(3, 0, A0, B0, xb0); WACC_FENCE();
            WACC_MMA_9(A1[9], B1[9]); t_micro(4, 0, A0, B0, xb0); WACC_FENCE();
            WACC_MMA_10(A1[10], B1[10]); t_micro(5, 0, A0, B0, xb0); t_micro(6, 0, A0, B0, xb0); WACC_FENCE();
            WACC_MMA_11(A1[11], B1[11]); t_micro(7, 0, A0, B0, xb0); t_micro(8, 0, A0, B0, xb0); WACC_FENCE();
            WACC_MMA_12(A1[12], B1[12]); t_micro(9, 0, A0, B0, xb0); t_micro(10, 0, A0, B0, xb0); WACC_FENCE();
            WACC_MMA_13(A1[13], B1[13]); t_micro(11, 0, A0, B0, xb0); WACC_FENCE();
            WACC_MMA_14(A1[14], B1[14]); t_micro(12, 0, A0, B0, xb0); WACC_FENCE();
            WACC_MMA_15(A1[15], B1[15]); t_micro(13, 0, A0, B0, xb0); WACC_FENCE();
            advance_stage();
        }

        } else if constexpr (GS == 4) {
        {
            const int nst_idx = st + 0 + 1;
            (void)nst_idx;
            WACC_MMA_0(A0[0], B0[0]); b_micro(0, 1, 1, B1, xb0); WACC_FENCE();
            WACC_MMA_1(A0[1], B0[1]); b_micro(1, 1, 1, B1, xb0); WACC_FENCE();
            WACC_MMA_2(A0[2], B0[2]); t_micro(4, 1, A1, B1, xb0); WACC_FENCE();
            WACC_MMA_3(A0[3], B0[3]); b_micro(2, 1, 1, B1, xb0); WACC_FENCE();
            WACC_MMA_4(A0[4], B0[4]); t_micro(11, 1, A1, B1, xb0); WACC_FENCE();
            WACC_MMA_5(A0[5], B0[5]); t_micro(12, 1, A1, B1, xb0); WACC_FENCE();
            WACC_MMA_6(A0[6], B0[6]); t_micro(13, 1, A1, B1, xb0); WACC_FENCE();
            WACC_MMA_7(A0[7], B0[7]); WACC_LDS_BARRIER(); WACC_FENCE();
            WACC_MMA_8(A0[8], B0[8]); b_micro(3, 1, 1, B1, xb0); WACC_FENCE();
            WACC_MMA_9(A0[9], B0[9]); b_micro(4, 1, 1, B1, xb0); WACC_FENCE();
            WACC_MMA_10(A0[10], B0[10]); b_micro(5, 1, 1, B1, xb0); WACC_FENCE();
            WACC_MMA_11(A0[11], B0[11]); b_micro(6, 1, 1, B1, xb0); WACC_FENCE();
            WACC_MMA_12(A0[12], B0[12]); if constexpr (RI > 0) r_micro(0, 0); WACC_FENCE();
            WACC_MMA_13(A0[13], B0[13]); if constexpr (RI > 0) r_micro(0, 1); WACC_FENCE();
            WACC_MMA_14(A0[14], B0[14]); if constexpr (RI > 1) r_micro(1, 0); WACC_FENCE();
            WACC_MMA_15(A0[15], B0[15]); if constexpr (RI > 1) r_micro(1, 1); WACC_FENCE();
            WACC_MMA_0(A1[0], B1[0]); b_micro(0, 2, 0, B0, xb0); g_load_s(0); WACC_FENCE();
            WACC_MMA_1(A1[1], B1[1]); b_micro(1, 2, 0, B0, xb0); g_load_s(1); WACC_FENCE();
            WACC_MMA_2(A1[2], B1[2]); t_micro(4, 2, A0, B0, xb0); g_load_s(2); WACC_FENCE();
            WACC_MMA_3(A1[3], B1[3]); b_micro(2, 2, 0, B0, xb0); g_load_s(3); WACC_FENCE();
            WACC_MMA_4(A1[4], B1[4]); t_micro(11, 2, A0, B0, xb0); g_load_s(4); WACC_FENCE();
            WACC_MMA_5(A1[5], B1[5]); t_micro(12, 2, A0, B0, xb0); g_load_s(5); WACC_FENCE();
            WACC_MMA_6(A1[6], B1[6]); t_micro(13, 2, A0, B0, xb0); g_load_s(6); WACC_FENCE();
            WACC_MMA_7(A1[7], B1[7]); WACC_LDS_BARRIER(); g_load_s(7); WACC_FENCE();
            WACC_MMA_8(A1[8], B1[8]); b_micro(3, 2, 0, B0, xb0); g_load_s(8); WACC_FENCE();
            WACC_MMA_9(A1[9], B1[9]); b_micro(4, 2, 0, B0, xb0); g_load_s(9); WACC_FENCE();
            WACC_MMA_10(A1[10], B1[10]); b_micro(5, 2, 0, B0, xb0); g_load_s(10); WACC_FENCE();
            WACC_MMA_11(A1[11], B1[11]); b_micro(6, 2, 0, B0, xb0); g_load_s(11); WACC_FENCE();
            WACC_MMA_12(A1[12], B1[12]); g_load_s(12); WACC_FENCE();
            WACC_MMA_13(A1[13], B1[13]); ; WACC_FENCE();
            WACC_MMA_14(A1[14], B1[14]); ; WACC_FENCE();
            WACC_MMA_15(A1[15], B1[15]); ; WACC_FENCE();
            WACC_MMA_0(A0[0], B0[0]); b_micro(0, 3, 1, B1, xb0); WACC_FENCE();
            WACC_MMA_1(A0[1], B0[1]); b_micro(1, 3, 1, B1, xb0); WACC_FENCE();
            WACC_MMA_2(A0[2], B0[2]); t_micro(4, 3, A1, B1, xb0); WACC_FENCE();
            WACC_MMA_3(A0[3], B0[3]); b_micro(2, 3, 1, B1, xb0); WACC_FENCE();
            WACC_MMA_4(A0[4], B0[4]); t_micro(11, 3, A1, B1, xb0); WACC_FENCE();
            WACC_MMA_5(A0[5], B0[5]); t_micro(12, 3, A1, B1, xb0); WACC_FENCE();
            WACC_MMA_6(A0[6], B0[6]); t_micro(13, 3, A1, B1, xb0); WACC_FENCE();
            WACC_MMA_7(A0[7], B0[7]); WACC_LDS_BARRIER(); WACC_FENCE();
            WACC_MMA_8(A0[8], B0[8]); b_micro(3, 3, 1, B1, xb0); WACC_FENCE();
            WACC_MMA_9(A0[9], B0[9]); b_micro(4, 3, 1, B1, xb0); WACC_FENCE();
            WACC_MMA_10(A0[10], B0[10]); b_micro(5, 3, 1, B1, xb0); WACC_FENCE();
            WACC_MMA_11(A0[11], B0[11]); b_micro(6, 3, 1, B1, xb0); WACC_FENCE();
            WACC_MMA_12(A0[12], B0[12]); ; WACC_FENCE();
            WACC_MMA_13(A0[13], B0[13]); ; WACC_FENCE();
            WACC_MMA_14(A0[14], B0[14]); ; WACC_FENCE();
            WACC_MMA_15(A0[15], B0[15]); ; WACC_FENCE();
            WACC_MMA_0(A1[0], B1[0]); b_micro(0, 4, 0, B0, xb0); WACC_FENCE();
            WACC_MMA_1(A1[1], B1[1]); b_micro(1, 4, 0, B0, xb0); WACC_FENCE();
            WACC_MMA_2(A1[2], B1[2]); t_micro(4, 4, A0, B0, xb0); WACC_FENCE();
            WACC_MMA_3(A1[3], B1[3]); b_micro(2, 4, 0, B0, xb0); WACC_FENCE();
            WACC_MMA_4(A1[4], B1[4]); t_micro(11, 4, A0, B0, xb0); WACC_FENCE();
            WACC_MMA_5(A1[5], B1[5]); t_micro(12, 4, A0, B0, xb0); WACC_FENCE();
            WACC_MMA_6(A1[6], B1[6]); t_micro(13, 4, A0, B0, xb0); WACC_FENCE();
            WACC_MMA_7(A1[7], B1[7]); WACC_LDS_BARRIER(); WACC_FENCE();
            WACC_MMA_8(A1[8], B1[8]); b_micro(3, 4, 0, B0, xb0); WACC_FENCE();
            WACC_MMA_9(A1[9], B1[9]); b_micro(4, 4, 0, B0, xb0); WACC_FENCE();
            WACC_MMA_10(A1[10], B1[10]); b_micro(5, 4, 0, B0, xb0); WACC_FENCE();
            WACC_MMA_11(A1[11], B1[11]); b_micro(6, 4, 0, B0, xb0); WACC_FENCE();
            WACC_MMA_12(A1[12], B1[12]); ; WACC_FENCE();
            WACC_MMA_13(A1[13], B1[13]); ; WACC_FENCE();
            WACC_MMA_14(A1[14], B1[14]); ; WACC_FENCE();
            WACC_MMA_15(A1[15], B1[15]); ; WACC_FENCE();
            WACC_MMA_0(A0[0], B0[0]); b_micro(0, 5, 1, B1, xb0); WACC_FENCE();
            WACC_MMA_1(A0[1], B0[1]); b_micro(1, 5, 1, B1, xb0); WACC_FENCE();
            WACC_MMA_2(A0[2], B0[2]); t_micro(4, 5, A1, B1, xb0); WACC_FENCE();
            WACC_MMA_3(A0[3], B0[3]); b_micro(2, 5, 1, B1, xb0); WACC_FENCE();
            WACC_MMA_4(A0[4], B0[4]); t_micro(11, 5, A1, B1, xb0); WACC_FENCE();
            WACC_MMA_5(A0[5], B0[5]); t_micro(12, 5, A1, B1, xb0); WACC_FENCE();
            WACC_MMA_6(A0[6], B0[6]); t_micro(13, 5, A1, B1, xb0); WACC_FENCE();
            WACC_MMA_7(A0[7], B0[7]); WACC_LDS_BARRIER(); WACC_FENCE();
            WACC_MMA_8(A0[8], B0[8]); b_micro(3, 5, 1, B1, xb0); WACC_FENCE();
            WACC_MMA_9(A0[9], B0[9]); b_micro(4, 5, 1, B1, xb0); WACC_FENCE();
            WACC_MMA_10(A0[10], B0[10]); b_micro(5, 5, 1, B1, xb0); WACC_FENCE();
            WACC_MMA_11(A0[11], B0[11]); b_micro(6, 5, 1, B1, xb0); WACC_FENCE();
            WACC_MMA_12(A0[12], B0[12]); if constexpr (RI > 0) r_micro(0, 2); WACC_FENCE();
            WACC_MMA_13(A0[13], B0[13]); if constexpr (RI > 0) r_micro(0, 3); WACC_FENCE();
            WACC_MMA_14(A0[14], B0[14]); if constexpr (RI > 0) r_micro(0, 4); WACC_FENCE();
            WACC_MMA_15(A0[15], B0[15]); if constexpr (RI > 0) r_micro(0, 5); WACC_FENCE();
            WACC_MMA_0(A1[0], B1[0]); b_micro(0, 6, 0, B0, xb0); WACC_FENCE();
            WACC_MMA_1(A1[1], B1[1]); b_micro(1, 6, 0, B0, xb0); WACC_FENCE();
            WACC_MMA_2(A1[2], B1[2]); t_micro(4, 6, A0, B0, xb0); WACC_FENCE();
            WACC_MMA_3(A1[3], B1[3]); b_micro(2, 6, 0, B0, xb0); WACC_FENCE();
            WACC_MMA_4(A1[4], B1[4]); t_micro(11, 6, A0, B0, xb0); WACC_FENCE();
            WACC_MMA_5(A1[5], B1[5]); t_micro(12, 6, A0, B0, xb0); WACC_FENCE();
            WACC_MMA_6(A1[6], B1[6]); t_micro(13, 6, A0, B0, xb0); WACC_FENCE();
            WACC_MMA_7(A1[7], B1[7]); WACC_LDS_BARRIER(); WACC_FENCE();
            WACC_MMA_8(A1[8], B1[8]); b_micro(3, 6, 0, B0, xb0); WACC_FENCE();
            WACC_MMA_9(A1[9], B1[9]); b_micro(4, 6, 0, B0, xb0); WACC_FENCE();
            WACC_MMA_10(A1[10], B1[10]); b_micro(5, 6, 0, B0, xb0); WACC_FENCE();
            WACC_MMA_11(A1[11], B1[11]); b_micro(6, 6, 0, B0, xb0); WACC_FENCE();
            WACC_MMA_12(A1[12], B1[12]); if constexpr (RI > 1) r_micro(1, 2); WACC_FENCE();
            WACC_MMA_13(A1[13], B1[13]); if constexpr (RI > 1) r_micro(1, 3); WACC_FENCE();
            WACC_MMA_14(A1[14], B1[14]); if constexpr (RI > 1) r_micro(1, 4); WACC_FENCE();
            WACC_MMA_15(A1[15], B1[15]); if constexpr (RI > 1) r_micro(1, 5); WACC_FENCE();
            WACC_MMA_0(A0[0], B0[0]); w_store_s(0, xb1); w_store_s(1, xb1); w_store_s(2, xb1); WACC_FENCE();
            WACC_MMA_1(A0[1], B0[1]); w_store_s(3, xb1); w_store_s(4, xb1); WACC_FENCE();
            WACC_MMA_2(A0[2], B0[2]); w_store_s(5, xb1); w_store_s(6, xb1); WACC_FENCE();
            WACC_MMA_3(A0[3], B0[3]); w_store_s(7, xb1); w_store_s(8, xb1); WACC_FENCE();
            WACC_MMA_4(A0[4], B0[4]); w_store_s(9, xb1); w_store_s(10, xb1); WACC_FENCE();
            WACC_MMA_5(A0[5], B0[5]); w_store_s(11, xb1); w_store_s(12, xb1); WACC_FENCE();
            WACC_MMA_6(A0[6], B0[6]); WACC_LDS_BARRIER(); WACC_FENCE();
            WACC_MMA_7(A0[7], B0[7]); b_micro(0, 0, 1, B1, xb1); WACC_FENCE();
            WACC_MMA_8(A0[8], B0[8]); b_micro(1, 0, 1, B1, xb1); WACC_FENCE();
            WACC_MMA_9(A0[9], B0[9]); t_micro(4, 0, A1, B1, xb1); WACC_FENCE();
            WACC_MMA_10(A0[10], B0[10]); b_micro(2, 0, 1, B1, xb1); WACC_FENCE();
            WACC_MMA_11(A0[11], B0[11]); t_micro(11, 0, A1, B1, xb1); t_micro(12, 0, A1, B1, xb1); t_micro(13, 0, A1, B1, xb1); WACC_FENCE();
            WACC_MMA_12(A0[12], B0[12]); WACC_LDS_BARRIER(); WACC_FENCE();
            WACC_MMA_13(A0[13], B0[13]); b_micro(3, 0, 1, B1, xb1); b_micro(4, 0, 1, B1, xb1); WACC_FENCE();
            WACC_MMA_14(A0[14], B0[14]); b_micro(5, 0, 1, B1, xb1); b_micro(6, 0, 1, B1, xb1); WACC_FENCE();
            WACC_MMA_15(A0[15], B0[15]); ; WACC_FENCE();
            advance_stage();
        }
        {
            const int nst_idx = st + 1 + 1;
            (void)nst_idx;
            if (st + 1 >= nst) break;
            WACC_MMA_0(A1[0], B1[0]); b_micro(0, 1, 0, B0, xb1); WACC_FENCE();
            WACC_MMA_1(A1[1], B1[1]); b_micro(1, 1, 0, B0, xb1); WACC_FENCE();
            WACC_MMA_2(A1[2], B1[2]); t_micro(4, 1, A0, B0, xb1); WACC_FENCE();
            WACC_MMA_3(A1[3], B1[3]); b_micro(2, 1, 0, B0, xb1); WACC_FENCE();
            WACC_MMA_4(A1[4], B1[4]); t_micro(11, 1, A0, B0, xb1); WACC_FENCE();
            WACC_MMA_5(A1[5], B1[5]); t_micro(12, 1, A0, B0, xb1); WACC_FENCE();
            WACC_MMA_6(A1[6], B1[6]); t_micro(13, 1, A0, B0, xb1); WACC_FENCE();
            WACC_MMA_7(A1[7], B1[7]); WACC_LDS_BARRIER(); WACC_FENCE();
            WACC_MMA_8(A1[8], B1[8]); b_micro(3, 1, 0, B0, xb1); WACC_FENCE();
            WACC_MMA_9(A1[9], B1[9]); b_micro(4, 1, 0, B0, xb1); WACC_FENCE();
            WACC_MMA_10(A1[10], B1[10]); b_micro(5, 1, 0, B0, xb1); WACC_FENCE();
            WACC_MMA_11(A1[11], B1[11]); b_micro(6, 1, 0, B0, xb1); WACC_FENCE();
            WACC_MMA_12(A1[12], B1[12]); if constexpr (RI > 0) r_micro(0, 0); WACC_FENCE();
            WACC_MMA_13(A1[13], B1[13]); if constexpr (RI > 0) r_micro(0, 1); WACC_FENCE();
            WACC_MMA_14(A1[14], B1[14]); if constexpr (RI > 1) r_micro(1, 0); WACC_FENCE();
            WACC_MMA_15(A1[15], B1[15]); if constexpr (RI > 1) r_micro(1, 1); WACC_FENCE();
            WACC_MMA_0(A0[0], B0[0]); b_micro(0, 2, 1, B1, xb1); g_load_s(0); WACC_FENCE();
            WACC_MMA_1(A0[1], B0[1]); b_micro(1, 2, 1, B1, xb1); g_load_s(1); WACC_FENCE();
            WACC_MMA_2(A0[2], B0[2]); t_micro(4, 2, A1, B1, xb1); g_load_s(2); WACC_FENCE();
            WACC_MMA_3(A0[3], B0[3]); b_micro(2, 2, 1, B1, xb1); g_load_s(3); WACC_FENCE();
            WACC_MMA_4(A0[4], B0[4]); t_micro(11, 2, A1, B1, xb1); g_load_s(4); WACC_FENCE();
            WACC_MMA_5(A0[5], B0[5]); t_micro(12, 2, A1, B1, xb1); g_load_s(5); WACC_FENCE();
            WACC_MMA_6(A0[6], B0[6]); t_micro(13, 2, A1, B1, xb1); g_load_s(6); WACC_FENCE();
            WACC_MMA_7(A0[7], B0[7]); WACC_LDS_BARRIER(); g_load_s(7); WACC_FENCE();
            WACC_MMA_8(A0[8], B0[8]); b_micro(3, 2, 1, B1, xb1); g_load_s(8); WACC_FENCE();
            WACC_MMA_9(A0[9], B0[9]); b_micro(4, 2, 1, B1, xb1); g_load_s(9); WACC_FENCE();
            WACC_MMA_10(A0[10], B0[10]); b_micro(5, 2, 1, B1, xb1); g_load_s(10); WACC_FENCE();
            WACC_MMA_11(A0[11], B0[11]); b_micro(6, 2, 1, B1, xb1); g_load_s(11); WACC_FENCE();
            WACC_MMA_12(A0[12], B0[12]); g_load_s(12); WACC_FENCE();
            WACC_MMA_13(A0[13], B0[13]); ; WACC_FENCE();
            WACC_MMA_14(A0[14], B0[14]); ; WACC_FENCE();
            WACC_MMA_15(A0[15], B0[15]); ; WACC_FENCE();
            WACC_MMA_0(A1[0], B1[0]); b_micro(0, 3, 0, B0, xb1); WACC_FENCE();
            WACC_MMA_1(A1[1], B1[1]); b_micro(1, 3, 0, B0, xb1); WACC_FENCE();
            WACC_MMA_2(A1[2], B1[2]); t_micro(4, 3, A0, B0, xb1); WACC_FENCE();
            WACC_MMA_3(A1[3], B1[3]); b_micro(2, 3, 0, B0, xb1); WACC_FENCE();
            WACC_MMA_4(A1[4], B1[4]); t_micro(11, 3, A0, B0, xb1); WACC_FENCE();
            WACC_MMA_5(A1[5], B1[5]); t_micro(12, 3, A0, B0, xb1); WACC_FENCE();
            WACC_MMA_6(A1[6], B1[6]); t_micro(13, 3, A0, B0, xb1); WACC_FENCE();
            WACC_MMA_7(A1[7], B1[7]); WACC_LDS_BARRIER(); WACC_FENCE();
            WACC_MMA_8(A1[8], B1[8]); b_micro(3, 3, 0, B0, xb1); WACC_FENCE();
            WACC_MMA_9(A1[9], B1[9]); b_micro(4, 3, 0, B0, xb1); WACC_FENCE();
            WACC_MMA_10(A1[10], B1[10]); b_micro(5, 3, 0, B0, xb1); WACC_FENCE();
            WACC_MMA_11(A1[11], B1[11]); b_micro(6, 3, 0, B0, xb1); WACC_FENCE();
            WACC_MMA_12(A1[12], B1[12]); ; WACC_FENCE();
            WACC_MMA_13(A1[13], B1[13]); ; WACC_FENCE();
            WACC_MMA_14(A1[14], B1[14]); ; WACC_FENCE();
            WACC_MMA_15(A1[15], B1[15]); ; WACC_FENCE();
            WACC_MMA_0(A0[0], B0[0]); b_micro(0, 4, 1, B1, xb1); WACC_FENCE();
            WACC_MMA_1(A0[1], B0[1]); b_micro(1, 4, 1, B1, xb1); WACC_FENCE();
            WACC_MMA_2(A0[2], B0[2]); t_micro(4, 4, A1, B1, xb1); WACC_FENCE();
            WACC_MMA_3(A0[3], B0[3]); b_micro(2, 4, 1, B1, xb1); WACC_FENCE();
            WACC_MMA_4(A0[4], B0[4]); t_micro(11, 4, A1, B1, xb1); WACC_FENCE();
            WACC_MMA_5(A0[5], B0[5]); t_micro(12, 4, A1, B1, xb1); WACC_FENCE();
            WACC_MMA_6(A0[6], B0[6]); t_micro(13, 4, A1, B1, xb1); WACC_FENCE();
            WACC_MMA_7(A0[7], B0[7]); WACC_LDS_BARRIER(); WACC_FENCE();
            WACC_MMA_8(A0[8], B0[8]); b_micro(3, 4, 1, B1, xb1); WACC_FENCE();
            WACC_MMA_9(A0[9], B0[9]); b_micro(4, 4, 1, B1, xb1); WACC_FENCE();
            WACC_MMA_10(A0[10], B0[10]); b_micro(5, 4, 1, B1, xb1); WACC_FENCE();
            WACC_MMA_11(A0[11], B0[11]); b_micro(6, 4, 1, B1, xb1); WACC_FENCE();
            WACC_MMA_12(A0[12], B0[12]); ; WACC_FENCE();
            WACC_MMA_13(A0[13], B0[13]); ; WACC_FENCE();
            WACC_MMA_14(A0[14], B0[14]); ; WACC_FENCE();
            WACC_MMA_15(A0[15], B0[15]); ; WACC_FENCE();
            WACC_MMA_0(A1[0], B1[0]); b_micro(0, 5, 0, B0, xb1); WACC_FENCE();
            WACC_MMA_1(A1[1], B1[1]); b_micro(1, 5, 0, B0, xb1); WACC_FENCE();
            WACC_MMA_2(A1[2], B1[2]); t_micro(4, 5, A0, B0, xb1); WACC_FENCE();
            WACC_MMA_3(A1[3], B1[3]); b_micro(2, 5, 0, B0, xb1); WACC_FENCE();
            WACC_MMA_4(A1[4], B1[4]); t_micro(11, 5, A0, B0, xb1); WACC_FENCE();
            WACC_MMA_5(A1[5], B1[5]); t_micro(12, 5, A0, B0, xb1); WACC_FENCE();
            WACC_MMA_6(A1[6], B1[6]); t_micro(13, 5, A0, B0, xb1); WACC_FENCE();
            WACC_MMA_7(A1[7], B1[7]); WACC_LDS_BARRIER(); WACC_FENCE();
            WACC_MMA_8(A1[8], B1[8]); b_micro(3, 5, 0, B0, xb1); WACC_FENCE();
            WACC_MMA_9(A1[9], B1[9]); b_micro(4, 5, 0, B0, xb1); WACC_FENCE();
            WACC_MMA_10(A1[10], B1[10]); b_micro(5, 5, 0, B0, xb1); WACC_FENCE();
            WACC_MMA_11(A1[11], B1[11]); b_micro(6, 5, 0, B0, xb1); WACC_FENCE();
            WACC_MMA_12(A1[12], B1[12]); if constexpr (RI > 0) r_micro(0, 2); WACC_FENCE();
            WACC_MMA_13(A1[13], B1[13]); if constexpr (RI > 0) r_micro(0, 3); WACC_FENCE();
            WACC_MMA_14(A1[14], B1[14]); if constexpr (RI > 0) r_micro(0, 4); WACC_FENCE();
            WACC_MMA_15(A1[15], B1[15]); if constexpr (RI > 0) r_micro(0, 5); WACC_FENCE();
            WACC_MMA_0(A0[0], B0[0]); b_micro(0, 6, 1, B1, xb1); WACC_FENCE();
            WACC_MMA_1(A0[1], B0[1]); b_micro(1, 6, 1, B1, xb1); WACC_FENCE();
            WACC_MMA_2(A0[2], B0[2]); t_micro(4, 6, A1, B1, xb1); WACC_FENCE();
            WACC_MMA_3(A0[3], B0[3]); b_micro(2, 6, 1, B1, xb1); WACC_FENCE();
            WACC_MMA_4(A0[4], B0[4]); t_micro(11, 6, A1, B1, xb1); WACC_FENCE();
            WACC_MMA_5(A0[5], B0[5]); t_micro(12, 6, A1, B1, xb1); WACC_FENCE();
            WACC_MMA_6(A0[6], B0[6]); t_micro(13, 6, A1, B1, xb1); WACC_FENCE();
            WACC_MMA_7(A0[7], B0[7]); WACC_LDS_BARRIER(); WACC_FENCE();
            WACC_MMA_8(A0[8], B0[8]); b_micro(3, 6, 1, B1, xb1); WACC_FENCE();
            WACC_MMA_9(A0[9], B0[9]); b_micro(4, 6, 1, B1, xb1); WACC_FENCE();
            WACC_MMA_10(A0[10], B0[10]); b_micro(5, 6, 1, B1, xb1); WACC_FENCE();
            WACC_MMA_11(A0[11], B0[11]); b_micro(6, 6, 1, B1, xb1); WACC_FENCE();
            WACC_MMA_12(A0[12], B0[12]); if constexpr (RI > 1) r_micro(1, 2); WACC_FENCE();
            WACC_MMA_13(A0[13], B0[13]); if constexpr (RI > 1) r_micro(1, 3); WACC_FENCE();
            WACC_MMA_14(A0[14], B0[14]); if constexpr (RI > 1) r_micro(1, 4); WACC_FENCE();
            WACC_MMA_15(A0[15], B0[15]); if constexpr (RI > 1) r_micro(1, 5); WACC_FENCE();
            WACC_MMA_0(A1[0], B1[0]); w_store_s(0, xb0); w_store_s(1, xb0); w_store_s(2, xb0); WACC_FENCE();
            WACC_MMA_1(A1[1], B1[1]); w_store_s(3, xb0); w_store_s(4, xb0); WACC_FENCE();
            WACC_MMA_2(A1[2], B1[2]); w_store_s(5, xb0); w_store_s(6, xb0); WACC_FENCE();
            WACC_MMA_3(A1[3], B1[3]); w_store_s(7, xb0); w_store_s(8, xb0); WACC_FENCE();
            WACC_MMA_4(A1[4], B1[4]); w_store_s(9, xb0); w_store_s(10, xb0); WACC_FENCE();
            WACC_MMA_5(A1[5], B1[5]); w_store_s(11, xb0); w_store_s(12, xb0); WACC_FENCE();
            WACC_MMA_6(A1[6], B1[6]); WACC_LDS_BARRIER(); WACC_FENCE();
            WACC_MMA_7(A1[7], B1[7]); b_micro(0, 0, 0, B0, xb0); WACC_FENCE();
            WACC_MMA_8(A1[8], B1[8]); b_micro(1, 0, 0, B0, xb0); WACC_FENCE();
            WACC_MMA_9(A1[9], B1[9]); t_micro(4, 0, A0, B0, xb0); WACC_FENCE();
            WACC_MMA_10(A1[10], B1[10]); b_micro(2, 0, 0, B0, xb0); WACC_FENCE();
            WACC_MMA_11(A1[11], B1[11]); t_micro(11, 0, A0, B0, xb0); t_micro(12, 0, A0, B0, xb0); t_micro(13, 0, A0, B0, xb0); WACC_FENCE();
            WACC_MMA_12(A1[12], B1[12]); WACC_LDS_BARRIER(); WACC_FENCE();
            WACC_MMA_13(A1[13], B1[13]); b_micro(3, 0, 0, B0, xb0); b_micro(4, 0, 0, B0, xb0); WACC_FENCE();
            WACC_MMA_14(A1[14], B1[14]); b_micro(5, 0, 0, B0, xb0); b_micro(6, 0, 0, B0, xb0); WACC_FENCE();
            WACC_MMA_15(A1[15], B1[15]); ; WACC_FENCE();
            advance_stage();
        }

        } else if constexpr (GS == 2) {
        {
            const int nst_idx = st + 0 + 1;
            (void)nst_idx;
            WACC_MMA_0(A0[0], B0[0]); t_micro(0, 1, A1, B1, xb0); WACC_FENCE();
            WACC_MMA_1(A0[1], B0[1]); t_micro(1, 1, A1, B1, xb0); WACC_FENCE();
            WACC_MMA_2(A0[2], B0[2]); t_micro(2, 1, A1, B1, xb0); WACC_FENCE();
            WACC_MMA_3(A0[3], B0[3]); t_micro(3, 1, A1, B1, xb0); WACC_FENCE();
            WACC_MMA_4(A0[4], B0[4]); t_micro(4, 1, A1, B1, xb0); WACC_FENCE();
            WACC_MMA_5(A0[5], B0[5]); t_micro(5, 1, A1, B1, xb0); WACC_FENCE();
            WACC_MMA_6(A0[6], B0[6]); t_micro(6, 1, A1, B1, xb0); WACC_FENCE();
            WACC_MMA_7(A0[7], B0[7]); t_micro(7, 1, A1, B1, xb0); WACC_FENCE();
            WACC_MMA_8(A0[8], B0[8]); t_micro(8, 1, A1, B1, xb0); WACC_FENCE();
            WACC_MMA_9(A0[9], B0[9]); t_micro(9, 1, A1, B1, xb0); WACC_FENCE();
            WACC_MMA_10(A0[10], B0[10]); t_micro(10, 1, A1, B1, xb0); WACC_FENCE();
            WACC_MMA_11(A0[11], B0[11]); t_micro(11, 1, A1, B1, xb0); WACC_FENCE();
            WACC_MMA_12(A0[12], B0[12]); t_micro(12, 1, A1, B1, xb0); WACC_FENCE();
            WACC_MMA_13(A0[13], B0[13]); t_micro(13, 1, A1, B1, xb0); WACC_FENCE();
            WACC_MMA_14(A0[14], B0[14]); ; WACC_FENCE();
            WACC_MMA_15(A0[15], B0[15]); ; WACC_FENCE();
            WACC_MMA_0(A1[0], B1[0]); t_micro(0, 2, A0, B0, xb0); g_load_s(0); WACC_FENCE();
            WACC_MMA_1(A1[1], B1[1]); t_micro(1, 2, A0, B0, xb0); g_load_s(1); WACC_FENCE();
            WACC_MMA_2(A1[2], B1[2]); t_micro(2, 2, A0, B0, xb0); g_load_s(2); WACC_FENCE();
            WACC_MMA_3(A1[3], B1[3]); t_micro(3, 2, A0, B0, xb0); g_load_s(3); WACC_FENCE();
            WACC_MMA_4(A1[4], B1[4]); t_micro(4, 2, A0, B0, xb0); g_load_s(4); WACC_FENCE();
            WACC_MMA_5(A1[5], B1[5]); t_micro(5, 2, A0, B0, xb0); g_load_s(5); WACC_FENCE();
            WACC_MMA_6(A1[6], B1[6]); t_micro(6, 2, A0, B0, xb0); g_load_s(6); WACC_FENCE();
            WACC_MMA_7(A1[7], B1[7]); t_micro(7, 2, A0, B0, xb0); g_load_s(7); WACC_FENCE();
            WACC_MMA_8(A1[8], B1[8]); t_micro(8, 2, A0, B0, xb0); g_load_s(8); WACC_FENCE();
            WACC_MMA_9(A1[9], B1[9]); t_micro(9, 2, A0, B0, xb0); g_load_s(9); WACC_FENCE();
            WACC_MMA_10(A1[10], B1[10]); t_micro(10, 2, A0, B0, xb0); g_load_s(10); WACC_FENCE();
            WACC_MMA_11(A1[11], B1[11]); t_micro(11, 2, A0, B0, xb0); g_load_s(11); WACC_FENCE();
            WACC_MMA_12(A1[12], B1[12]); t_micro(12, 2, A0, B0, xb0); g_load_s(12); WACC_FENCE();
            WACC_MMA_13(A1[13], B1[13]); t_micro(13, 2, A0, B0, xb0); g_load_s(13); WACC_FENCE();
// ... 391 lines not shown
            WACC_MMA_2(A1[2], B1[2]); t_micro(2, 5, A0, B0, xb1); WACC_FENCE();
            WACC_MMA_3(A1[3], B1[3]); t_micro(3, 5, A0, B0, xb1); WACC_FENCE();
            WACC_MMA_4(A1[4], B1[4]); t_micro(4, 5, A0, B0, xb1); WACC_FENCE();
            WACC_MMA_5(A1[5], B1[5]); t_micro(5, 5, A0, B0, xb1); WACC_FENCE();
            WACC_MMA_6(A1[6], B1[6]); t_micro(6, 5, A0, B0, xb1); WACC_FENCE();
            WACC_MMA_7(A1[7], B1[7]); t_micro(7, 5, A0, B0, xb1); WACC_FENCE();
            WACC_MMA_8(A1[8], B1[8]); t_micro(8, 5, A0, B0, xb1); WACC_FENCE();
            WACC_MMA_9(A1[9], B1[9]); t_micro(9, 5, A0, B0, xb1); WACC_FENCE();
            WACC_MMA_10(A1[10], B1[10]); t_micro(10, 5, A0, B0, xb1); WACC_FENCE();
            WACC_MMA_11(A1[11], B1[11]); t_micro(11, 5, A0, B0, xb1); WACC_FENCE();
            WACC_MMA_12(A1[12], B1[12]); t_micro(12, 5, A0, B0, xb1); WACC_FENCE();
            WACC_MMA_13(A1[13], B1[13]); t_micro(13, 5, A0, B0, xb1); WACC_FENCE();
            WACC_MMA_14(A1[14], B1[14]); ; WACC_FENCE();
            WACC_MMA_15(A1[15], B1[15]); ; WACC_FENCE();
            WACC_MMA_0(A0[0], B0[0]); t_micro(0, 6, A1, B1, xb1); WACC_FENCE();
            WACC_MMA_1(A0[1], B0[1]); t_micro(1, 6, A1, B1, xb1); WACC_FENCE();
            WACC_MMA_2(A0[2], B0[2]); t_micro(2, 6, A1, B1, xb1); WACC_FENCE();
            WACC_MMA_3(A0[3], B0[3]); t_micro(3, 6, A1, B1, xb1); WACC_FENCE();
            WACC_MMA_4(A0[4], B0[4]); t_micro(4, 6, A1, B1, xb1); WACC_FENCE();
            WACC_MMA_5(A0[5], B0[5]); t_micro(5, 6, A1, B1, xb1); WACC_FENCE();
            WACC_MMA_6(A0[6], B0[6]); t_micro(6, 6, A1, B1, xb1); WACC_FENCE();
            WACC_MMA_7(A0[7], B0[7]); t_micro(7, 6, A1, B1, xb1); WACC_FENCE();
            WACC_MMA_8(A0[8], B0[8]); t_micro(8, 6, A1, B1, xb1); WACC_FENCE();
            WACC_MMA_9(A0[9], B0[9]); t_micro(9, 6, A1, B1, xb1); WACC_FENCE();
            WACC_MMA_10(A0[10], B0[10]); t_micro(10, 6, A1, B1, xb1); WACC_FENCE();
            WACC_MMA_11(A0[11], B0[11]); t_micro(11, 6, A1, B1, xb1); WACC_FENCE();
            WACC_MMA_12(A0[12], B0[12]); t_micro(12, 6, A1, B1, xb1); WACC_FENCE();
            WACC_MMA_13(A0[13], B0[13]); t_micro(13, 6, A1, B1, xb1); WACC_FENCE();
            WACC_MMA_14(A0[14], B0[14]); ; WACC_FENCE();
            WACC_MMA_15(A0[15], B0[15]); ; WACC_FENCE();
            WACC_MMA_0(A1[0], B1[0]); w_store(0); w_store(1); w_store(2); w_store(3); WACC_FENCE();
            WACC_MMA_1(A1[1], B1[1]); w_store(4); w_store(5); w_store(6); w_store(7); WACC_FENCE();
            WACC_MMA_2(A1[2], B1[2]); w_store(8); w_store(9); w_store(10); w_store(11); WACC_FENCE();
            WACC_MMA_3(A1[3], B1[3]); w_store(12); w_store(13); w_store(14); w_store(15); WACC_FENCE();
            WACC_MMA_4(A1[4], B1[4]); w_store(16); w_store(17); w_store(18); w_store(19); WACC_FENCE();
            WACC_MMA_5(A1[5], B1[5]); w_store(20); w_store(21); w_store(22); w_store(23); WACC_FENCE();
            WACC_MMA_6(A1[6], B1[6]); w_store(24); w_store(25); w_store(26); w_store(27); WACC_FENCE();
            WACC_MMA_7(A1[7], B1[7]); t_micro(0, 0, A0, B0, xb0); t_micro(1, 0, A0, B0, xb0); WACC_FENCE();
            WACC_MMA_8(A1[8], B1[8]); t_micro(2, 0, A0, B0, xb0); t_micro(3, 0, A0, B0, xb0); WACC_FENCE();
            WACC_MMA_9(A1[9], B1[9]); t_micro(4, 0, A0, B0, xb0); WACC_FENCE();
            WACC_MMA_10(A1[10], B1[10]); t_micro(5, 0, A0, B0, xb0); t_micro(6, 0, A0, B0, xb0); WACC_FENCE();
            WACC_MMA_11(A1[11], B1[11]); t_micro(7, 0, A0, B0, xb0); t_micro(8, 0, A0, B0, xb0); WACC_FENCE();
            WACC_MMA_12(A1[12], B1[12]); t_micro(9, 0, A0, B0, xb0); t_micro(10, 0, A0, B0, xb0); WACC_FENCE();
            WACC_MMA_13(A1[13], B1[13]); t_micro(11, 0, A0, B0, xb0); WACC_FENCE();
            WACC_MMA_14(A1[14], B1[14]); t_micro(12, 0, A0, B0, xb0); WACC_FENCE();
            WACC_MMA_15(A1[15], B1[15]); t_micro(13, 0, A0, B0, xb0); WACC_FENCE();
            advance_stage();
        }

        }
    }

    WW_STAMP(3);
    if constexpr (RI > 0) {
        while (rq < rq_end) {
#pragma unroll
            for (int m = 0; m < 6; ++m) r_micro(0, m);
        }
    }
    WACC_DRAIN();
    float *pout = part + ((int64_t)split * 9 * g.K + k0) * g.C + c0 + li;
    const int64_t tap_plane = (int64_t)g.K * g.C;
    auto out_e = [&](int e, float (&m)[16]) {
        m[3] = -m[3], m[7] = -m[7], m[11] = -m[11], m[12] = -m[12], m[13] = -m[13], m[14] = -m[14];
        float t[3][4];
#pragma unroll
        for (int j = 0; j < 4; ++j) {
            const float s = 0.5f * (m[4 + j] + m[8 + j]), d = 0.5f * (m[4 + j] - m[8 + j]);
            t[0][j] = m[j] + s, t[1][j] = d, t[2][j] = s + m[12 + j];
        }
        float *dst = pout + (int64_t)((e & 3) + 8 * (e >> 2) + 4 * lh) * g.C;
#pragma unroll
        for (int r = 0; r < 3; ++r) {
            const float s = 0.5f * (t[r][1] + t[r][2]), d = 0.5f * (t[r][1] - t[r][2]);
            dst[(r * 3 + 0) * tap_plane] = t[r][0] + s;
            dst[(r * 3 + 1) * tap_plane] = d;
            dst[(r * 3 + 2) * tap_plane] = s + t[r][3];
        }
    };
    {
        float m[16];
#define WW_OUT(e) WACC_RD16_##e(m); out_e(e, m);
        WACC_EACH16(WW_OUT)
#undef WW_OUT
    }
    WW_STAMP(4);
}

inline int pad_to(int v, int m) { return (v + m - 1) / m * m; }

struct WwPlan {
    WwGeom g;
    size_t ws_bytes;
    int64_t blocks;
    bool narrow;
    int gs;
};

bool ww_plan(const cpg_conv_desc *d, WwPlan &p) {
    if (opt_on(OPT_NO_WINO) || opt_on(OPT_NO_WINO_WGRAD)) return false;
    if (d->R != 3 || d->S != 3 || d->stride_h != 1 || d->stride_w != 1 || d->pad_h != 1 || d->pad_w != 1 || d->dil_h != 1 ||
        d->dil_w != 1 || d->groups != 1)
        return false;
    p.narrow = d->W == 14;
    if (d->H % 2 || (d->W % 28 && !p.narrow) || d->C < 32 || d->K < 32 || d->N < 1) return false;
    WwGeom &g = p.g;
    g.N = d->N, g.C = d->C, g.K = d->K, g.H = d->H, g.W = d->W;
    g.th = d->H / 2, g.tw = d->W / 2, g.nseg = p.narrow ? 1 : g.tw / 14;
    const int64_t nstages = (int64_t)(p.narrow ? (d->N + 1) / 2 : d->N) * g.th * g.nseg;
    if (nstages >= (1ll << 28)) return false;
    g.nstages = (unsigned)nstages;
    g.nkb = (d->K + 31) / 32, g.ncb = (d->C + 31) / 32;
    const int64_t npairs = (int64_t)g.nkb * g.ncb;
    int upw = shared_chip_hint() ? 2 : 1;
    const int64_t slots = 4 * kCUs;
    if (const int forced = opt(OPT_WW_UNITS); forced != OPT_UNSET) {
        upw = std::max(1, forced);
    } else {
        double best = -1.0;
        int best_r = upw;
        for (int r = upw; r <= upw + 2; ++r) {
            const int64_t w = std::min<int64_t>(std::max<int64_t>(1, r * slots / npairs), nstages);
            const int64_t units = npairs * w, rounds = (units + slots - 1) / slots;
            const double eff = (double)units / (double)(rounds * slots) - 0.015 * (double)(rounds - upw);
            if (eff > best + 1e-9) best = eff, best_r = r;
        }
        upw = best_r;
    }
    int64_t want = std::max<int64_t>(1, ((int64_t)upw * slots) / npairs);
    want = std::min<int64_t>(want, nstages);
    g.su = (unsigned)((nstages + want - 1) / want);
    g.nsplit = (int)((nstages + g.su - 1) / g.su);
    const int64_t per_img = (int64_t)g.th * g.nseg;
    g.span = ((int)((g.su + per_img - 1) / per_img) + 1) * (p.narrow ? 2 : 1);
    const int64_t HW = (int64_t)d->H * d->W;
    if ((int64_t)g.span * std::max(d->C, d->K) * HW * 4 + (d->W + 4) * 4 >= (1ll << 31)) return false;
    p.ws_bytes = (size_t)g.nsplit * 9 * d->K * d->C * sizeof(float);
    p.blocks = (npairs * g.nsplit + 3) / 4;
    g.xcd = opt_or(OPT_WW_XCD, 1) != 0;
    p.gs = 0;
    if (npairs % 4 == 0) p.gs = g.nkb % 4 == 0 ? 4 : ((g.nkb % 2 == 0 && !p.narrow) ? 2 : 0);
    if (const int f = opt(OPT_WW_SHARE); f != OPT_UNSET && (f == 0 || (p.gs != 0 && (f == 2 || (f == 4 && p.gs == 4))))) p.gs = f;
    return p.blocks <= 0x7FFFFFFFll;
}

bool ww_rider_ok(const WwPlan &p) { return p.gs == 4 && !opt_on(OPT_NO_WW_RIDER); }
bool ww_rider_plan(const WwPlan &p, const WgradRider &r, WwRider &rd, int &ri) {
    if (r.N < 1 || r.C < 1 || r.HW < 4 || r.HW % 4 || (int64_t)r.N * r.C * r.HW * 4 >= (1ll << 31)) return false;
    if ((((uintptr_t)r.y) | ((uintptr_t)r.gz) | ((uintptr_t)r.gy) | ((uintptr_t)r.table)) & 15) return false;
    rd.y = r.y, rd.gz = r.gz, rd.gy = r.gy, rd.table = r.table;
    rd.C = r.C, rd.HW = r.HW, rd.p4 = r.HW / 4, rd.ipp = (rd.p4 + 63) / 64;
    rd.bytes = r.N * r.C * r.HW * 4;
    const int64_t total = (int64_t)r.N * r.C * rd.ipp, waves = (int64_t)p.g.nkb * p.g.ncb * p.g.nsplit;
    if (waves % 4 != 0 || (waves + 3) / 4 != p.blocks) return false;
    rd.total = (unsigned)total;
    rd.per = (unsigned)((total + waves - 1) / waves);
    ri = rd.per <= p.g.su ? 1 : 2;
    return true;
}

}

#ifdef WG_TIMING
extern "C" int cpg_debug_ww_timing(unsigned long long *dst, int n) {
    return (int)hipMemcpyFromSymbol(dst, HIP_SYMBOL(ww_dbg), (size_t)n * 8 * sizeof(unsigned long long));
}
#endif
extern "C" int cpg_conv3x3_wino_wgrad_ok(const cpg_conv_desc *d) {
    WwPlan p;
    return ww_plan(d, p) ? 1 : 0;
}

extern "C" int cpg_conv3x3_wino_wgrad_rider_ok(const cpg_conv_desc *d) {
    WwPlan p;
    return ww_plan(d, p) && ww_rider_ok(p) ? 1 : 0;
}

extern "C" size_t cpg_conv3x3_wino_wgrad_workspace(const cpg_conv_desc *d) {
    WwPlan p;
    return ww_plan(d, p) ? p.ws_bytes : 0;
}

extern "C" int cpg_conv3x3_wino_wgrad(const cpg_conv_desc *d, const float *x, const float *gy, const float *w, const float *pm, float thr,
                                      float *gw, float *gpm, void *ws, size_t ws_bytes, hipStream_t stream) {
    WwPlan p;
    if (!ww_plan(d, p)) return fail(CPG_E_UNSUPPORTED, "cpg_conv2d_wgrad(winograd): shape not supported");
    if (ws == nullptr || ws_bytes < p.ws_bytes)
        return fail(CPG_E_WORKSPACE, "cpg_conv2d_wgrad(winograd): workspace %zu < %zu bytes", ws_bytes, p.ws_bytes);
    WwRider rd{};
    int ri = 0;
    if (WgradRider &r = wgrad_rider(); r.armed) {
        if (!ww_rider_ok(p) || !ww_rider_plan(p, r, rd, ri))
            return fail(CPG_E_UNSUPPORTED, "cpg_conv2d_wgrad(winograd): the attached BatchNorm backward cannot ride in this launch "
                                           "(cpg_conv2d_wgrad_rider_supported, 4 | HW, < 2 GiB, 16-byte aligned pointers)");
        if (rd.y == x || rd.gz == x || rd.gy == x || rd.gy == gy || (const float *)rd.gy == rd.y || (const float *)rd.gy == rd.gz)
            return fail(CPG_E_INVALID, "cpg_conv2d_wgrad(winograd): the rider's result may not alias its inputs or the weight gradient's");
    }
    const dim3 grid((unsigned)p.blocks), block(256);
    if (p.narrow && ri == 2)
        hipLaunchKernelGGL((k_wgw<true, 4, 2>), grid, block, 0, stream, p.g, x, gy, (float *)ws, rd);
    else if (p.narrow && ri == 1)
        hipLaunchKernelGGL((k_wgw<true, 4, 1>), grid, block, 0, stream, p.g, x, gy, (float *)ws, rd);
    else if (ri == 2)
        hipLaunchKernelGGL((k_wgw<false, 4, 2>), grid, block, 0, stream, p.g, x, gy, (float *)ws, rd);
    else if (ri == 1)
        hipLaunchKernelGGL((k_wgw<false, 4, 1>), grid, block, 0, stream, p.g, x, gy, (float *)ws, rd);
    else if (p.narrow && p.gs == 4)
        hipLaunchKernelGGL((k_wgw<true, 4>), grid, block, 0, stream, p.g, x, gy, (float *)ws, rd);
    else if (p.narrow)
        hipLaunchKernelGGL(k_wgw<true>, grid, block, 0, stream, p.g, x, gy, (float *)ws, rd);
    else if (p.gs == 4)
        hipLaunchKernelGGL((k_wgw<false, 4>), grid, block, 0, stream, p.g, x, gy, (float *)ws, rd);
    else if (p.gs == 2)
        hipLaunchKernelGGL((k_wgw<false, 2>), grid, block, 0, stream, p.g, x, gy, (float *)ws, rd);
    else
        hipLaunchKernelGGL(k_wgw<false>, grid, block, 0, stream, p.g, x, gy, (float *)ws, rd);
    Epilogue ep{gw, nullptr, BIAS_NONE, 1, 1, pm, w, gpm, thr};
    const int64_t out_elems = (int64_t)d->K * d->C * 9;
    launch_split_reduce((const float *)ws, p.g.nsplit, out_elems, (int64_t)d->K * d->C, ep, stream);
    CPG_CHECK_LAUNCH("cpg_conv2d_wgrad(winograd)");
    return CPG_OK;
}
```

### cpg_amd/csrc/cpg_common.cpp

```cpp
#include "cpg_common.h"
#include <stdarg.h>
#include <stdlib.h>
#include <string.h>
#include <atomic>

namespace cpg {

static thread_local char g_err[512] = "";

char *err_buf() { return g_err; }

int fail(int code, const char *fmt, ...) {
    va_list ap;
    va_start(ap, fmt);
    vsnprintf(g_err, sizeof(g_err), fmt, ap);
    va_end(ap);
    return code;
}

static thread_local PackCtx g_pack = {};
PackCtx &pack_ctx() { return g_pack; }
static thread_local WgradRider g_rider = {};
WgradRider &wgrad_rider() { return g_rider; }

int take_packed(size_t bytes, const float **pre, const char *what) {
    PackCtx &c = g_pack;
    *pre = nullptr;
    if (!c.armed) return CPG_OK;
    if (c.use == nullptr || c.use_bytes != bytes || (((uintptr_t)c.use) & 15) != 0)
        return fail(CPG_E_INVALID, "%s: the packed operand handed in (%zu bytes) is not the one this launch streams (%zu bytes, 16-byte aligned)",
                    what, c.use_bytes, bytes);
    *pre = c.use;
    c.armed = false;
    return CPG_OK;
}

static std::atomic<int> g_shared_chip{0};
int shared_chip_hint() { return g_shared_chip.load(std::memory_order_relaxed); }

namespace {
enum Kind { BOOL, INT, WINO_KERNEL };
struct OptDef {
    const char *name;
    Kind kind;
};
const OptDef kDefs[OPT_COUNT] = {
    {"CPG_NO_WINO", BOOL},          {"CPG_NO_WINO_WGRAD", BOOL},   {"CPG_NO_WINO_ODD", BOOL},      {"CPG_NO_STEM", BOOL},
    {"CPG_NO_STEM_FUSE", BOOL},     {"CPG_NO_DEAD_SKIP", BOOL},    {"CPG_NO_S2", BOOL},            {"CPG_NO_V14", BOOL},
    {"CPG_DISABLE_CONV3X3", BOOL},  {"CPG_DISABLE_CONV1X1", BOOL}, {"CPG_DISABLE_CONV1X1_WGRAD", BOOL}, {"CPG_DISABLE_PW_GEMM", BOOL},
    {"CPG_C3_FORCE", INT},          {"CPG_C3W_BPC", INT},          {"CPG_W3_PICK", INT},           {"CPG_PWW_BPC", INT},
    {"CPG_STEM_BLOCKS", INT},       {"CPG_WINO_KERNEL", WINO_KERNEL}, {"CPG_WINO_NW", INT},        {"CPG_WINO_PERSIST", INT},
    {"CPG_WINO_GRIDS", INT},        {"CPG_WW_UNITS", INT},         {"CPG_WW_XCD", INT},            {"CPG_PW_TILE", INT},           {"CPG_WG3_SHARE", INT},
    {"CPG_WW_SHARE", INT},          {"CPG_WINO_TAIL", INT},         {"CPG_FC_SMALL", INT},
    {"CPG_NO_WW_RIDER", BOOL},      {"CPG_NO_GROUPED", BOOL},       {"CPG_GROUPED_WIDE_MIN", INT},
};

struct Table {
    std::atomic<int> v[OPT_COUNT];
    Table() {
        for (int i = 0; i < OPT_COUNT; ++i) {
            int val = OPT_UNSET;
            if (const char *f = getenv(kDefs[i].name)) {
                switch (kDefs[i].kind) {
                    case BOOL: val = (f[0] == 0 || (f[0] == '0' && f[1] == 0)) ? 0 : 1; break;
                    case INT: val = atoi(f); break;
                    case WINO_KERNEL: val = f[0] == 'b' ? 0 : f[0] == 'p' ? 2 : f[0] == '6' ? 3 : 1; break;
                }
            }
            v[i].store(val, std::memory_order_relaxed);
        }
    }
};
Table g_opts;

int find_opt(const char *name) {
    if (name == nullptr) return -1;
    for (int i = 0; i < OPT_COUNT; ++i)
        if (strcmp(name, kDefs[i].name) == 0) return i;
    return -1;
}
}

int opt(Opt o) { return g_opts.v[o].load(std::memory_order_relaxed); }

}

extern "C" int cpg_set_shared_chip_hint(int32_t shared) {
    cpg::g_shared_chip.store(shared ? 1 : 0, std::memory_order_relaxed);
    return CPG_OK;
}
extern "C" int32_t cpg_get_shared_chip_hint(void) { return cpg::shared_chip_hint(); }
extern "C" int cpg_set_option(const char *name, int32_t value) {
    const int i = cpg::find_opt(name);
    if (i < 0) return cpg::fail(CPG_E_INVALID, "cpg_set_option: unknown option '%s'", name ? name : "(null)");
    cpg::g_opts.v[i].store(value, std::memory_order_relaxed);
    return CPG_OK;
}
extern "C" int cpg_get_option(const char *name, int32_t *value) {
    const int i = cpg::find_opt(name);
    if (i < 0 || value == nullptr) return cpg::fail(CPG_E_INVALID, "cpg_get_option: unknown option '%s'", name ? name : "(null)");
    *value = cpg::g_opts.v[i].load(std::memory_order_relaxed);
    return CPG_OK;
}
extern "C" int cpg_version(void) { return CPG_ABI_VERSION; }
extern "C" const char *cpg_last_error(void) { return cpg::err_buf(); }
```

### cpg_amd/csrc/cpg_common.h

```cpp
#pragma once
#include <hip/hip_runtime.h>
#include <stdint.h>
#include <stdio.h>
#include "../../include/cpg_hip.h"

namespace cpg {

char *err_buf();
int fail(int code, const char *fmt, ...);
int shared_chip_hint();

enum Opt {
    OPT_NO_WINO,
    OPT_NO_WINO_WGRAD,
    OPT_NO_WINO_ODD,
    OPT_NO_STEM,
    OPT_NO_STEM_FUSE,
    OPT_NO_DEAD_SKIP,
    OPT_NO_S2,
    OPT_NO_V14,
    OPT_DISABLE_CONV3X3,
    OPT_DISABLE_CONV1X1,
    OPT_DISABLE_CONV1X1_WGRAD,
    OPT_DISABLE_PW_GEMM,
    OPT_C3_FORCE,
    OPT_C3W_BPC,
    OPT_W3_PICK,
    OPT_PWW_BPC,
    OPT_STEM_BLOCKS,
    OPT_WINO_KERNEL,
    OPT_WINO_NW,
    OPT_WINO_PERSIST,
    OPT_WINO_GRIDS,
    OPT_WW_UNITS,
    OPT_WW_XCD,
    OPT_PW_TILE,
    OPT_WG3_SHARE,
    OPT_WW_SHARE,
    OPT_WINO_TAIL,
    OPT_FC_SMALL,
    OPT_NO_WW_RIDER,
    OPT_NO_GROUPED,
    OPT_GROUPED_WIDE_MIN,
    OPT_COUNT
};
constexpr int OPT_UNSET = INT32_MIN;
int opt(Opt o);
inline bool opt_on(Opt o) { const int v = opt(o); return v != OPT_UNSET && v != 0; }
inline int opt_or(Opt o, int dflt) { const int v = opt(o); return v == OPT_UNSET ? dflt : v; }

struct PackJob {
    int family;
    int K, C;
    int a, b, c, d;
    long long total;
    size_t bytes;
};
struct PackCtx {
    bool armed;
    const float *use;
    size_t use_bytes;
};
PackCtx &pack_ctx();
int take_packed(size_t bytes, const float **pre, const char *what);
int pack_jobs_launch(const PackJob *ja, float *dst_a, const PackJob *jb, float *dst_b, const float *w, const float *pm, float thr,
                     hipStream_t stream);

struct WgradRider {
    bool armed;
    const float *y, *gz, *table;
    float *gy;
    int N, C, HW;
};
WgradRider &wgrad_rider();

inline int hip_status(hipError_t e, const char *what) {
    if (e == hipSuccess) return CPG_OK;
    return fail(CPG_E_HIP_BASE + (int)e, "%s: %s", what, hipGetErrorString(e));
}

#define CPG_CHECK_LAUNCH(what)                                   \
    do {                                                         \
        hipError_t e__ = hipGetLastError();                      \
        if (e__ != hipSuccess) return cpg::hip_status(e__, what); \
    } while (0)

#define CPG_REQUIRE(cond, ...)                                  \
    do {                                                        \
        if (!(cond)) return cpg::fail(CPG_E_INVALID, __VA_ARGS__); \
    } while (0)

__device__ __forceinline__ float binarize(float pm, float thr) {
    return pm > thr ? 1.0f : (pm <= thr ? 0.0f : pm);
}

__device__ __forceinline__ float bn_affine(float x, float mean, float invstd, float gamma, float beta) {
// ... 23 lines not shown
```

### cpg_amd/models/fused_bn.py

```python
import ctypes

import torch
import torch.nn as nn

from .. import _lib
from .layers import BiasGradSink, BnBwdHint, _conv_desc

ENABLED = True
ENABLE_BWD_HINT = False
ENABLE_WGRAD_RIDER = True
RELU_BYTE_MASK = True
FUSE_STEM = True
FUSE_STEM_WGRAD = True
FUSE_SKIP_ADD = True


def _batch_stats(stats, nbt, N, C, HW, eps, momentum, running_mean, running_var, training, device):
    if not training:
        return running_mean, torch.rsqrt(running_var + eps), nbt
    mean = torch.empty(C, dtype=torch.float32, device=device)
    invstd = torch.empty(C, dtype=torch.float32, device=device)
    if stats is not None:
        args = (_lib.dptr(stats, name='bn partial sums'), stats.shape[1], N, C, HW, float(eps), float(momentum),
                _lib.dptr(running_mean, name='running_mean'), _lib.dptr(running_var, name='running_var'), _lib.dptr(mean), _lib.dptr(invstd))
        if nbt is not None and running_mean is not None and nbt.is_cuda and nbt.dtype == torch.int64 and nbt.numel() == 1:
            _lib.call('cpg_bn_stats_finalize_count', *args, _lib.dptr(nbt, torch.int64, 'num_batches_tracked'), _lib.stream_ptr())
            nbt = None
        else:
            _lib.call('cpg_bn_stats_finalize', *args, _lib.stream_ptr())
    return mean, invstd, nbt


def _count(nbt):
    if nbt is not None:
        nbt.add_(1)


def _bn_args(bn):
    training = bn.training or not bn.track_running_stats
    rm, rv = (bn.running_mean, bn.running_var) if bn.track_running_stats else (None, None)
    nbt = bn.num_batches_tracked if (training and bn.track_running_stats) else None
    return (bn.weight, bn.bias, rm, rv, bn.eps, bn.momentum, training), training, nbt


class _BnReluFn(torch.autograd.Function):
    @staticmethod
    def forward(ctx, x, gamma, beta, running_mean, running_var, eps, momentum, training, relu, stats=None, hint=None, nbt=None):
        x = x.contiguous()
        N, C = x.shape[0], x.shape[1]
        HW = x.numel() // (N * C)
        L = _lib.lib()
        y = torch.empty_like(x)
        s = _lib.stream_ptr()
        mean, invstd, nbt = _batch_stats(stats, nbt, N, C, HW, eps, momentum, running_mean, running_var, training, x.device)
        if training and stats is None:
            ws, nb = _lib.workspace(L.cpg_bn_workspace_bytes(N, C, HW), x.device)
            _lib.call('cpg_bn_relu_fwd_train', _lib.dptr(x, name='input'), _lib.dptr(gamma, name='bn.weight'), _lib.dptr(beta, name='bn.bias'),
                      float(eps), float(momentum), _lib.dptr(running_mean, name='running_mean'), _lib.dptr(running_var, name='running_var'),
                      _lib.dptr(mean), _lib.dptr(invstd), _lib.dptr(y), N, C, HW, int(relu), _lib.dptr(ws), nb, s)
        else:
            _lib.call('cpg_bn_relu_fwd_eval', _lib.dptr(x, name='input'), _lib.dptr(gamma), _lib.dptr(beta), _lib.dptr(mean),
                      _lib.dptr(invstd), _lib.dptr(y), N, C, HW, int(relu), s)
        _count(nbt)
        ctx.save_for_backward(x, gamma, beta, mean, invstd)
        ctx.cfg = (N, C, HW, bool(relu), bool(training))
        ctx.hint = None
        if hint is not None and relu and training:
# ... 25 lines not shown
        else:
            _lib.call('cpg_bn_relu_bwd', _lib.dptr(x), _lib.dptr(gy, name='grad_output'), _lib.dptr(gamma), _lib.dptr(beta), _lib.dptr(mean),
                      _lib.dptr(invstd), _lib.dptr(gx), _lib.dptr(dgamma), _lib.dptr(dbeta), N, C, HW, int(relu), int(training),
                      _lib.dptr(ws), nb, _lib.stream_ptr())
        return (gx, dgamma, dbeta) + (None,) * 9


class _BnAddReluFn(torch.autograd.Function):

    @staticmethod
    def forward(ctx, x, res, gamma, beta, running_mean, running_var, eps, momentum, training, stats=None, nbt=None):
        x, res = x.contiguous(), res.contiguous()
        N, C = x.shape[0], x.shape[1]
        HW = x.numel() // (N * C)
        L = _lib.lib()
        y = torch.empty_like(x)
        apply_only = not training or stats is not None
        mean, invstd, nbt = _batch_stats(stats, nbt, N, C, HW, eps, momentum, running_mean, running_var, training, x.device)
        ws, nb = (None, 0) if apply_only else _lib.workspace(L.cpg_bn_workspace_bytes(N, C, HW), x.device)
        mask = None
        nmask = L.cpg_bn_add_relu_mask_bytes(N, C, HW) if (RELU_BYTE_MASK and any(ctx.needs_input_grad)) else 0
        if nmask and x.data_ptr() % 16 == 0 and res.data_ptr() % 16 == 0 and y.data_ptr() % 16 == 0:
            mask = torch.empty(nmask, dtype=torch.uint8, device=x.device)
        _lib.call('cpg_bn_add_relu_fwd', _lib.dptr(x, name='input'), _lib.dptr(res, name='residual'), _lib.dptr(gamma), _lib.dptr(beta),
                  float(eps), float(momentum), _lib.dptr(None if apply_only else running_mean),
                  _lib.dptr(None if apply_only else running_var), _lib.dptr(mean), _lib.dptr(invstd), _lib.dptr(y),
                  N, C, HW, int(not apply_only), _lib.dptr(ws), nb, _lib.stream_ptr(), _lib.dptr(mask, torch.uint8))
        _count(nbt)
        ctx.save_for_backward(x, y if mask is None else mask, gamma, beta, mean, invstd)
        ctx.has_mask = mask is not None
        ctx.cfg = (N, C, HW, bool(training))
        return y

    @staticmethod
    def backward(ctx, gy):
        x, y, gamma, beta, mean, invstd = ctx.saved_tensors
        mask, y = (y, None) if ctx.has_mask else (None, y)
        N, C, HW, training = ctx.cfg
        gy = gy.contiguous()
        if mask is not None and gy.data_ptr() % 16:
            gy = gy.clone()
        L = _lib.lib()
        gx = torch.empty_like(x)
        gz = torch.empty_like(x)
        dgamma, dbeta = torch.empty_like(gamma), torch.empty_like(beta)
        ws, nb = _lib.workspace(L.cpg_bn_workspace_bytes(N, C, HW), x.device)
        _lib.call('cpg_bn_add_relu_bwd', _lib.dptr(x), _lib.dptr(y), _lib.dptr(gy, name='grad_output'), _lib.dptr(gamma), _lib.dptr(beta),
                  _lib.dptr(mean), _lib.dptr(invstd), _lib.dptr(gx), _lib.dptr(gz), _lib.dptr(dgamma), _lib.dptr(dbeta),
                  N, C, HW, int(training), _lib.dptr(ws), nb, _lib.stream_ptr(), _lib.dptr(mask, torch.uint8))
        return (gx, gz, dgamma, dbeta) + (None,) * 7


def _pool_backward(name, ctx, gp):
    x, gamma, beta, mean, invstd = ctx.saved_tensors
    N, C, H, W = x.shape
    gp = gp.contiguous()
    gx = torch.empty_like(x)
    dgamma, dbeta = torch.empty_like(gamma), torch.empty_like(beta)
    ws, nb = _lib.workspace(_lib.lib().cpg_bn_workspace_bytes(N, C, H * W), x.device)
    _lib.call(name, _lib.dptr(x), _lib.dptr(gp, name='grad_output'), _lib.dptr(gamma), _lib.dptr(beta), _lib.dptr(mean),
              _lib.dptr(invstd), _lib.dptr(gx), _lib.dptr(dgamma), _lib.dptr(dbeta), N, C, H, W, int(ctx.training), _lib.dptr(ws), nb,
              _lib.stream_ptr())
    return (gx, dgamma, dbeta) + (None,) * 7


class _BnReluPoolFn(torch.autograd.Function):

    @staticmethod
    def forward(ctx, x, gamma, beta, running_mean, running_var, eps, momentum, training, stats=None, nbt=None):
        x = x.contiguous()
        N, C, H, W = x.shape
        L = _lib.lib()
        y = torch.empty((N, C, H // 2, W // 2), dtype=torch.float32, device=x.device)
        compute_stats = training and stats is None
        mean, invstd, nbt = _batch_stats(stats, nbt, N, C, H * W, eps, momentum, running_mean, running_var, training, x.device)
        ws, nb = _lib.workspace(L.cpg_bn_workspace_bytes(N, C, H * W), x.device)
        _lib.call('cpg_bn_relu_pool_fwd', _lib.dptr(x, name='input'), _lib.dptr(gamma, name='bn.weight'), _lib.dptr(beta, name='bn.bias'),
                  float(eps), float(momentum), _lib.dptr(running_mean if compute_stats else None),
                  _lib.dptr(running_var if compute_stats else None), _lib.dptr(mean), _lib.dptr(invstd),
                  _lib.dptr(y), N, C, H, W, int(compute_stats), _lib.dptr(ws), nb, _lib.stream_ptr())
        _count(nbt)
        ctx.save_for_backward(x, gamma, beta, mean, invstd)
        ctx.training = bool(training)
        return y

    @staticmethod
    def backward(ctx, gp):
        return _pool_backward('cpg_bn_relu_pool_bwd', ctx, gp)


class _BnReluPool3Fn(torch.autograd.Function):

    @staticmethod
    def forward(ctx, x, gamma, beta, running_mean, running_var, eps, momentum, training, stats, nbt=None):
        x = x.contiguous()
        N, C, H, W = x.shape
        mean, invstd, nbt = _batch_stats(stats, nbt, N, C, H * W, eps, momentum, running_mean, running_var, training, x.device)
        if training and stats is None:
            var, mu = torch.var_mean(x, dim=(0, 2, 3), unbiased=False)
            mean.copy_(mu)
            invstd.copy_(torch.rsqrt(var + eps))
            n = x.numel() // C
            with torch.no_grad():
                running_mean.mul_(1 - momentum).add_(mu, alpha=momentum)
                running_var.mul_(1 - momentum).add_(var * (n / max(n - 1, 1)), alpha=momentum)
        y = torch.empty((N, C, (H - 1) // 2 + 1, (W - 1) // 2 + 1), dtype=torch.float32, device=x.device)
        _lib.call('cpg_bn_relu_pool3_fwd', _lib.dptr(x, name='input'), _lib.dptr(gamma, name='bn.weight'), _lib.dptr(beta, name='bn.bias'),
                  _lib.dptr(mean), _lib.dptr(invstd), _lib.dptr(y), N, C, H, W, _lib.stream_ptr())
        _count(nbt)
        ctx.save_for_backward(x, gamma, beta, mean, invstd)
        ctx.training = bool(training)
        return y

    @staticmethod
    def backward(ctx, gp):
        return _pool_backward('cpg_bn_relu_pool3_bwd', ctx, gp)


def _is_pool(m, kernel, stride, padding):
    def pair(v):
        return tuple(v) if isinstance(v, (tuple, list)) else (v, v)
    return (isinstance(m, nn.MaxPool2d) and pair(m.kernel_size) == (kernel, kernel) and pair(m.stride) == (stride, stride)
            and pair(m.padding) == (padding, padding) and pair(m.dilation) == (1, 1) and not m.ceil_mode and not m.return_indices)


def _is_pool2(m):
    return _is_pool(m, 2, 2, 0)


def _is_pool3(m):
    return _is_pool(m, 3, 2, 1)


def _stats_from_conv(bn, fuse_stats, x=None, need_grad=False):
    return (fuse_stats and isinstance(bn, nn.BatchNorm2d) and bn.training and bn.track_running_stats and bn.affine
            and bn.momentum is not None and (x is None or x.is_cuda) and (not need_grad or torch.is_grad_enabled()))


def conv_bn_act_pool(conv, bn, act, pool, x):
    y, stats = _conv_with_stats(conv, bn, x)
    if (ENABLED and FusedSequential.fuse_pool and type(act) is nn.ReLU and _is_pool3(pool) and fusable(bn, y) and bn.track_running_stats
# ... 287 lines not shown
```

### include/cpg_hip.h

```cpp
#ifndef CPG_HIP_H
#define CPG_HIP_H

#include <stddef.h>
#include <stdint.h>

#ifdef __cplusplus
extern "C" {
#endif

#define CPG_ABI_VERSION 3

#define CPG_OK 0
#define CPG_E_INVALID (-1)
#define CPG_E_UNSUPPORTED (-2)
#define CPG_E_WORKSPACE (-3)
#define CPG_E_KRANGE 2
#define CPG_E_HIP_BASE 1000

#define CPG_MODE_FINETUNE 0
#define CPG_MODE_PRUNE 1

typedef struct cpg_conv_desc {
    int32_t N, C, H, W;
    int32_t K;
// ... 149 lines not shown
                            float threshold, float *gw, float *gpm, void *workspace, size_t workspace_bytes, void *stream);
size_t cpg_conv2d_bf16_workspace_bytes(const cpg_conv_desc *desc);
int cpg_conv2d_fwd_bf16(const cpg_conv_desc *desc, const float *x, const float *w, const float *piggymask, float threshold,
                        const float *bias, float *y, void *workspace, size_t workspace_bytes, void *stream);
int cpg_conv2d_dgrad_bf16(const cpg_conv_desc *desc, const float *gy, const float *w, const float *piggymask, float threshold,
                          float *gx, void *workspace, size_t workspace_bytes, void *stream);

int32_t cpg_conv2d_dgrad_bnbwd_tiles(const cpg_conv_desc *desc);
int cpg_conv2d_dgrad_bnbwd(const cpg_conv_desc *desc, const float *gy, const float *w, const float *piggymask, float threshold,
                           const float *ypre, const float *gamma, const float *beta, const float *mean, const float *invstd,
                           float *gm, float *partials, size_t partial_bytes, void *workspace, size_t workspace_bytes, void *stream);
int cpg_bn_bwd_from_partials(const float *partials, int32_t tiles, const float *x, const float *gm, const float *gamma,
                             const float *beta, const float *mean, const float *invstd, float *gx, float *dgamma, float *dbeta,
                             int32_t N, int32_t C, int32_t HW, void *workspace, size_t workspace_bytes, void *stream);

int cpg_bn_bwd_finalize_partials(const float *partials, int32_t tiles, int32_t N, int32_t C, int32_t HW, float *dgamma, float *dbeta,
                                 float *coef, void *stream);

int32_t cpg_stem_bn_supported(const cpg_conv_desc *desc);
int32_t cpg_stem_bn_tiles(const cpg_conv_desc *desc);
int cpg_stem_bn_stats(const cpg_conv_desc *desc, const float *x, const float *w, const float *piggymask, float threshold,
                      const float *bias, float *stats, size_t stats_bytes, void *stream);
int cpg_stem_bn_relu_fwd(const cpg_conv_desc *desc, const float *x, const float *w, const float *piggymask, float threshold,
                         const float *bias, const float *gamma, const float *beta, const float *mean, const float *invstd, float *z,
                         void *stream);
int cpg_stem_bn_relu_bwd_reduce(const cpg_conv_desc *desc, const float *x, const float *w, const float *piggymask, float threshold,
                                const float *bias, const float *gamma, const float *beta, const float *mean, const float *invstd,
                                const float *gz, float *partials, size_t partials_bytes, void *stream);
int cpg_stem_bn_relu_bwd_apply(const cpg_conv_desc *desc, const float *x, const float *w, const float *piggymask, float threshold,
                               const float *bias, const float *gamma, const float *beta, const float *mean, const float *invstd,
                               const float *coef, const float *gz, float *gy, void *stream);
size_t cpg_stem_bn_wgrad_workspace(const cpg_conv_desc *desc);
int cpg_stem_bn_relu_bwd_wgrad(const cpg_conv_desc *desc, const float *x, const float *w, const float *piggymask, float threshold,
                               const float *bias, const float *gamma, const float *beta, const float *mean, const float *invstd,
                               const float *coef, const float *gz, float *gw, float *gpm, void *workspace, size_t workspace_bytes,
                               void *stream);

size_t cpg_bn_add_relu_mask_bytes(int32_t N, int32_t C, int32_t HW);
int cpg_bn_add_relu_fwd(const float *x, const float *res, const float *gamma, const float *beta, float eps,
                        float momentum, float *running_mean, float *running_var, float *mean, float *invstd, float *y,
                        int32_t N, int32_t C, int32_t HW, int32_t train, void *ws, size_t ws_bytes, void *stream, uint8_t *relu_mask);
int cpg_bn_add_relu_bwd(const float *x, const float *out, const float *gy, const float *gamma, const float *beta,
                        const float *mean, const float *invstd, float *gx, float *gz, float *dgamma, float *dbeta, int32_t N,
                        int32_t C, int32_t HW, int32_t train, void *ws, size_t ws_bytes, void *stream, const uint8_t *relu_mask);

int cpg_bn_relu_pool_fwd(const float *x, const float *gamma, const float *beta, float eps, float momentum,
                         float *running_mean, float *running_var, float *mean, float *invstd, float *y_pooled,
                         int32_t N, int32_t C, int32_t H, int32_t W, int32_t train, void *ws, size_t ws_bytes,
                         void *stream);
int cpg_bn_relu_pool_bwd(const float *x, const float *g_pooled, const float *gamma, const float *beta,
                         const float *mean, const float *invstd, float *gx, float *dgamma, float *dbeta,
                         int32_t N, int32_t C, int32_t H, int32_t W, int32_t train, void *ws, size_t ws_bytes,
                         void *stream);

int32_t cpg_bn_relu_pool3_supported(int32_t H, int32_t W);
int cpg_bn_relu_pool3_fwd(const float *x, const float *gamma, const float *beta, const float *mean, const float *invstd,
                          float *y_pooled, int32_t N, int32_t C, int32_t H, int32_t W, void *stream);
int cpg_bn_relu_pool3_bwd(const float *x, const float *g_pooled, const float *gamma, const float *beta, const float *mean,
                          const float *invstd, float *gx, float *dgamma, float *dbeta, int32_t N, int32_t C, int32_t H,
                          int32_t W, int32_t train, void *workspace, size_t workspace_bytes, void *stream);

size_t cpg_prelu_workspace_bytes(int32_t N, int32_t C, int32_t HW);
int cpg_prelu_bwd(const float *x, const float *gy, const float *slope, float *gx, float *gslope, int32_t N,
                  int32_t C, int32_t HW, int32_t n_slopes, void *ws, size_t ws_bytes, void *stream);
int cpg_prelu_bwd_bias(const float *x, const float *gy, const float *slope, float *gx, float *gslope, float *gbias, int32_t N,
                       int32_t C, int32_t HW, int32_t n_slopes, void *workspace, size_t workspace_bytes, void *stream);
int cpg_prelu_fwd(const float *x, const float *residual, const float *slope, float *y, int32_t N, int32_t C, int32_t HW,
                  int32_t n_slopes, void *stream);

typedef struct cpg_resample_item {
    int64_t src_off;
    int32_t src_h, src_w;
    int32_t crop_y, crop_x, crop_h, crop_w;
    int64_t dst_off;
    int32_t out_h, out_w;
} cpg_resample_item;
typedef struct cpg_tensor_item {
    int64_t src_off;
    int32_t src_h, src_w;
    int32_t y0, x0;
    int32_t flip;
    int32_t cut_y0, cut_y1, cut_x0, cut_x1;
    int32_t reserved;
} cpg_tensor_item;
size_t cpg_image_resample_workspace_bytes(const cpg_resample_item *items_host, int32_t n_items);
int cpg_image_resample(const uint8_t *src, int64_t src_bytes, const cpg_resample_item *items_host, int32_t n_items, uint8_t *dst,
                       int64_t dst_bytes, void *workspace, size_t workspace_bytes, void *stream);
int cpg_image_to_tensor(const uint8_t *src, int64_t src_bytes, const cpg_tensor_item *items_host, int32_t n_items, int32_t out_h,
                        int32_t out_w, const float *mean_host, const float *std_host, float *dst, int64_t dst_bytes, void *stream);

int cpg_pair_distance(const float *a, int64_t lda, const float *b, int64_t ldb, int64_t n, int32_t d, int32_t metric, float *dist, float *sim,
                      void *stream);
int cpg_pair_sweep(const float *dist, const uint8_t *issame, int64_t n, const double *thr_host, int32_t n_thr, int32_t nfolds, int64_t *counts,
                   int64_t *best, void *stream);

size_t cpg_loss_heads_workspace_bytes(int32_t B, int32_t D, int32_t C);
int cpg_softmax_xent_fwd(const float *logits, const int64_t *target, const float *class_weight, int32_t B, int32_t C, float *loss,
                         float *correct, void *workspace, size_t workspace_bytes, void *stream);
int cpg_softmax_xent_fwd_bwd(const float *logits, const int64_t *target, const float *class_weight, const float *gscale, int32_t B,
                             int32_t C, float *loss, float *correct, float *dlogits, void *workspace, size_t workspace_bytes,
                             void *stream);
int cpg_angle_head_fwd(const float *x, const float *w, const int64_t *target, int32_t B, int32_t D, int32_t C, int32_t m, float gamma,
                       double lamb, float *what, float *colnorm, float *f, float *saved, float *loss, float *correct, void *workspace,
                       size_t workspace_bytes, void *stream);
int cpg_angle_head_bwd(const float *x, const float *what, const float *colnorm, const float *f, const float *saved,
                       const int64_t *target, const float *gscale, int32_t B, int32_t D, int32_t C, int32_t m, float gamma, double lamb,
// ... 7 lines not shown
```

Baseline: 2397 images/sec.

## Save pooled-window argmax inputs for BN-ReLU-pool backward and add wgrad rider v2 schedules

New measurement: 2405 images/sec, median of 6. No clear change (+0.3%).

```diff
diff --git a/cpg_amd/_lib.py b/cpg_amd/_lib.py
--- a/cpg_amd/_lib.py
+++ b/cpg_amd/_lib.py
@@ -102,6 +102,8 @@
     'cpg_bn_relu_fwd_eval': (_int, [_vp, _vp, _vp, _vp, _vp, _vp, _i32, _i32, _i32, _i32, _vp]),
     'cpg_bn_relu_pool_fwd': (_int, [_vp, _vp, _vp, _f32, _f32, _vp, _vp, _vp, _vp, _vp, _i32, _i32, _i32, _i32, _i32, _vp, _sz, _vp]),
     'cpg_bn_relu_pool_bwd': (_int, [_vp, _vp, _vp, _vp, _vp, _vp, _vp, _vp, _vp, _i32, _i32, _i32, _i32, _i32, _vp, _sz, _vp]),
+    'cpg_bn_relu_pool_fwd_xmax': (_int, [_vp, _vp, _vp, _f32, _f32] + [_vp] * 5 + [_i32] * 5 + [_vp, _sz, _vp, _vp]),
+    'cpg_bn_relu_pool_bwd_xmax': (_int, [_vp] * 9 + [_i32] * 5 + [_vp, _sz, _vp, _vp]),
     'cpg_bn_relu_bwd': (_int, [_vp, _vp, _vp, _vp, _vp, _vp, _vp, _vp, _vp, _i32, _i32, _i32, _i32, _i32, _vp, _sz, _vp]),
     'cpg_conv2d_winograd': (_i32, [_desc, _i32]),
     'cpg_conv2d_bnstats_tiles': (_i32, [_desc]),
diff --git a/cpg_amd/csrc/bn_kernels.hip b/cpg_amd/csrc/bn_kernels.hip
--- a/cpg_amd/csrc/bn_kernels.hip
+++ b/cpg_amd/csrc/bn_kernels.hip
@@ -589,10 +589,11 @@
     return idx;
 }
 
-template <int GROUP>
+template <int GROUP, bool XMAX>
 __global__ __launch_bounds__(kThreads) void k_bnp_apply(const float *__restrict__ x, float *__restrict__ yp, BnDims d, PoolDims p,
                                                         const float *__restrict__ mean, const float *__restrict__ invstd,
-                                                        const float *__restrict__ gamma, const float *__restrict__ beta) {
+                                                        const float *__restrict__ gamma, const float *__restrict__ beta,
+                                                        float *__restrict__ xm) {
     const int64_t planes = (int64_t)d.N * d.C;
     const int gl = threadIdx.x % GROUP;
     const int64_t g0 = (int64_t)blockIdx.x * (kThreads / GROUP) + threadIdx.x / GROUP;
@@ -605,10 +606,14 @@
         for (int i = gl; i < p.wins; i += GROUP) {
             const int pr = i / p.OW, pc = i - pr * p.OW;
             const Win w = load_win(plane, p.W, pr, pc);
+            float y[4];
+#pragma unroll
+            for (int k = 0; k < 4; ++k) y[k] = bn_affine(w.v[k], m, is, ga, be);
             float best = 0.0f;
 #pragma unroll
-            for (int k = 0; k < 4; ++k) best = fmaxf(best, bn_affine(w.v[k], m, is, ga, be));
+            for (int k = 0; k < 4; ++k) best = fmaxf(best, y[k]);
             out[i] = best;
+            if (XMAX) xm[pl * p.wins + i] = w.v[win_argmax(y)];
         }
     }
 }
@@ -635,6 +640,35 @@
         if (y[idx] > 0.f) {
             sg += g;
             sgx += g * ((w.v[idx] - m) * is);
+        }
+    }, [&]() {
+        dsg += (double)sg; dsgx += (double)sgx; sg = 0.f; sgx = 0.f;
+    });
+    const double t0 = block_sum(dsg, red);
+    const double t1 = block_sum(dsgx, red);
+    if (threadIdx.x == 0) {
+        partial[((int64_t)c * d.slices + s) * 2 + 0] = t0;
+        partial[((int64_t)c * d.slices + s) * 2 + 1] = t1;
+    }
+}
+
+__global__ __launch_bounds__(kThreads) void k_bnp_bwd_reduce_saved(const float *__restrict__ xm, const float *__restrict__ gp, BnDims d,
+                                                                   PoolDims p, const float *__restrict__ mean,
+                                                                   const float *__restrict__ invstd, const float *__restrict__ gamma,
+                                                                   const float *__restrict__ beta, double *__restrict__ partial) {
+    __shared__ double red[4];
+    const int c = blockIdx.x, s = blockIdx.y;
+    const int n0 = s * d.imgs_per_slice, n1 = min(d.N, n0 + d.imgs_per_slice);
+    const float m = mean[c], is = invstd[c], ga = gamma[c], be = beta[c];
+    double dsg = 0.0, dsgx = 0.0;
+    float sg = 0.f, sgx = 0.f;
+    walk_planes(p.wins, n0, n1, [&](int n, int wi) {
+        const int64_t i = ((int64_t)n * d.C + c) * p.wins + wi;
+        const float xv = xm[i];
+        const float g = gp[i];
+        if (bn_affine(xv, m, is, ga, be) > 0.f) {
+            sg += g;
+            sgx += g * ((xv - m) * is);
         }
     }, [&]() {
         dsg += (double)sg; dsgx += (double)sgx; sg = 0.f; sgx = 0.f;
@@ -695,54 +729,55 @@
     return (unsigned)(groups < cap ? groups : cap);
 }
 
-}
-
-extern "C" int cpg_bn_relu_pool_fwd(const float *x, const float *gamma, const float *beta, float eps, float momentum,
-                                    float *running_mean, float *running_var, float *mean, float *invstd, float *y_pooled,
-                                    int32_t N, int32_t C, int32_t H, int32_t W, int32_t train, void *ws, size_t ws_bytes,
-                                    void *stream_v) {
+int pool_fwd(const char *who, const float *x, const float *gamma, const float *beta, float eps, float momentum, float *running_mean,
+             float *running_var, float *mean, float *invstd, float *y_pooled, float *x_max, int32_t N, int32_t C, int32_t H, int32_t W,
+             int32_t train, void *ws, size_t ws_bytes, void *stream_v) {
     BnDims d;
     PoolDims p;
     int rc = make_dims(N, C, H * W, d);
     if (rc) return rc;
     rc = make_pool(H, W, p);
     if (rc) return rc;
-    CPG_REQUIRE(x && gamma && beta && mean && invstd && y_pooled, "cpg_bn_relu_pool_fwd: null pointer");
-    CPG_REQUIRE((((uintptr_t)x) & 7) == 0, "cpg_bn_relu_pool_fwd: x must be 8-byte aligned");
+    CPG_REQUIRE(x && gamma && beta && mean && invstd && y_pooled, "%s: null pointer", who);
+    CPG_REQUIRE((((uintptr_t)x) & 7) == 0, "%s: x must be 8-byte aligned", who);
     hipStream_t stream = (hipStream_t)stream_v;
     if (train) {
-        CPG_REQUIRE(ws != nullptr, "cpg_bn_relu_pool_fwd: workspace required in training mode");
-        if (ws_bytes < cpg_bn_workspace_bytes(N, C, H * W)) return fail(CPG_E_WORKSPACE, "cpg_bn_relu_pool_fwd: workspace too small");
+        CPG_REQUIRE(ws != nullptr, "%s: workspace required in training mode", who);
+        if (ws_bytes < cpg_bn_workspace_bytes(N, C, H * W)) return fail(CPG_E_WORKSPACE, "%s: workspace too small", who);
         double *partial = (double *)ws;
         hipLaunchKernelGGL(k_bn_stats, dim3(C, d.slices), dim3(kThreads), 0, stream, x, d, partial);
         hipLaunchKernelGGL(k_bn_finalize, dim3((C + 63) / 64), dim3(64), 0, stream, partial, d, eps, momentum, mean, invstd,
                            running_mean, running_var);
     }
     const bool wave = p.wins < 1024;
-    if (wave)
-        hipLaunchKernelGGL(k_bnp_apply<64>, dim3(pool_grid(d, p, true)), dim3(kThreads), 0, stream, x, y_pooled, d, p, mean, invstd, gamma, beta);
-    else
-        hipLaunchKernelGGL(k_bnp_apply<256>, dim3(pool_grid(d, p, false)), dim3(kThreads), 0, stream, x, y_pooled, d, p, mean, invstd, gamma, beta);
-    CPG_CHECK_LAUNCH("cpg_bn_relu_pool_fwd");
-    return CPG_OK;
-}
-
-extern "C" int cpg_bn_relu_pool_bwd(const float *x, const float *g_pooled, const float *gamma, const float *beta,
-                                    const float *mean, const float *invstd, float *gx, float *dgamma, float *dbeta, int32_t N,
-                                    int32_t C, int32_t H, int32_t W, int32_t train, void *ws, size_t ws_bytes, void *stream_v) {
+    const dim3 grid(pool_grid(d, p, wave)), block(kThreads);
+    if (wave && x_max) hipLaunchKernelGGL((k_bnp_apply<64, true>), grid, block, 0, stream, x, y_pooled, d, p, mean, invstd, gamma, beta, x_max);
+    else if (wave) hipLaunchKernelGGL((k_bnp_apply<64, false>), grid, block, 0, stream, x, y_pooled, d, p, mean, invstd, gamma, beta, x_max);
+    else if (x_max) hipLaunchKernelGGL((k_bnp_apply<256, true>), grid, block, 0, stream, x, y_pooled, d, p, mean, invstd, gamma, beta, x_max);
+    else hipLaunchKernelGGL((k_bnp_apply<256, false>), grid, block, 0, stream, x, y_pooled, d, p, mean, invstd, gamma, beta, x_max);
+    CPG_CHECK_LAUNCH(who);
+    return CPG_OK;
+}
+
+int pool_bwd(const char *who, const float *x, const float *x_max, const float *g_pooled, const float *gamma, const float *beta,
+             const float *mean, const float *invstd, float *gx, float *dgamma, float *dbeta, int32_t N, int32_t C, int32_t H, int32_t W,
+             int32_t train, void *ws, size_t ws_bytes, void *stream_v) {
     BnDims d;
     PoolDims p;
     int rc = make_dims(N, C, H * W, d);
     if (rc) return rc;
     rc = make_pool(H, W, p);
     if (rc) return rc;
-    CPG_REQUIRE(x && g_pooled && gamma && beta && mean && invstd && gx && dgamma && dbeta && ws, "cpg_bn_relu_pool_bwd: null pointer");
-    CPG_REQUIRE((((uintptr_t)x) & 7) == 0 && (((uintptr_t)gx) & 7) == 0, "cpg_bn_relu_pool_bwd: x / gx must be 8-byte aligned");
-    if (ws_bytes < cpg_bn_workspace_bytes(N, C, H * W)) return fail(CPG_E_WORKSPACE, "cpg_bn_relu_pool_bwd: workspace too small");
+    CPG_REQUIRE(x && g_pooled && gamma && beta && mean && invstd && gx && dgamma && dbeta && ws, "%s: null pointer", who);
+    CPG_REQUIRE((((uintptr_t)x) & 7) == 0 && (((uintptr_t)gx) & 7) == 0, "%s: x / gx must be 8-byte aligned", who);
+    if (ws_bytes < cpg_bn_workspace_bytes(N, C, H * W)) return fail(CPG_E_WORKSPACE, "%s: workspace too small", who);
     hipStream_t stream = (hipStream_t)stream_v;
     double *partial = (double *)ws;
     float *coef = (float *)(partial + (size_t)C * d.slices * 2);
-    hipLaunchKernelGGL(k_bnp_bwd_reduce, dim3(C, d.slices), dim3(kThreads), 0, stream, x, g_pooled, d, p, mean, invstd, gamma, beta, partial);
+    if (x_max)
+        hipLaunchKernelGGL(k_bnp_bwd_reduce_saved, dim3(C, d.slices), dim3(kThreads), 0, stream, x_max, g_pooled, d, p, mean, invstd, gamma, beta, partial);
+    else
+        hipLaunchKernelGGL(k_bnp_bwd_reduce, dim3(C, d.slices), dim3(kThreads), 0, stream, x, g_pooled, d, p, mean, invstd, gamma, beta, partial);
     hipLaunchKernelGGL(k_bn_bwd_finalize, dim3((C + 63) / 64), dim3(64), 0, stream, partial, d, dgamma, dbeta, coef);
     const bool wave = p.wins < 1024;
     const dim3 grid(pool_grid(d, p, wave)), block(kThreads);
@@ -750,8 +785,43 @@
     else if (wave) hipLaunchKernelGGL((k_bnp_bwd_apply<false, 64>), grid, block, 0, stream, x, g_pooled, gx, d, p, mean, invstd, gamma, beta, coef);
     else if (train) hipLaunchKernelGGL((k_bnp_bwd_apply<true, 256>), grid, block, 0, stream, x, g_pooled, gx, d, p, mean, invstd, gamma, beta, coef);
     else hipLaunchKernelGGL((k_bnp_bwd_apply<false, 256>), grid, block, 0, stream, x, g_pooled, gx, d, p, mean, invstd, gamma, beta, coef);
-    CPG_CHECK_LAUNCH("cpg_bn_relu_pool_bwd");
-    return CPG_OK;
+    CPG_CHECK_LAUNCH(who);
+    return CPG_OK;
+}
+
+}
+
+extern "C" int cpg_bn_relu_pool_fwd(const float *x, const float *gamma, const float *beta, float eps, float momentum,
+                                    float *running_mean, float *running_var, float *mean, float *invstd, float *y_pooled,
+                                    int32_t N, int32_t C, int32_t H, int32_t W, int32_t train, void *ws, size_t ws_bytes,
+                                    void *stream_v) {
+    return pool_fwd("cpg_bn_relu_pool_fwd", x, gamma, beta, eps, momentum, running_mean, running_var, mean, invstd, y_pooled, nullptr, N, C,
+                    H, W, train, ws, ws_bytes, stream_v);
+}
+
+extern "C" int cpg_bn_relu_pool_bwd(const float *x, const float *g_pooled, const float *gamma, const float *beta,
+                                    const float *mean, const float *invstd, float *gx, float *dgamma, float *dbeta, int32_t N,
+                                    int32_t C, int32_t H, int32_t W, int32_t train, void *ws, size_t ws_bytes, void *stream_v) {
+    return pool_bwd("cpg_bn_relu_pool_bwd", x, nullptr, g_pooled, gamma, beta, mean, invstd, gx, dgamma, dbeta, N, C, H, W, train, ws,
+                    ws_bytes, stream_v);
+}
+
+extern "C" int cpg_bn_relu_pool_fwd_xmax(const float *x, const float *gamma, const float *beta, float eps, float momentum,
+                                         float *running_mean, float *running_var, float *mean, float *invstd, float *y_pooled,
+                                         int32_t N, int32_t C, int32_t H, int32_t W, int32_t train, void *ws, size_t ws_bytes,
+                                         void *stream_v, float *x_max) {
+    CPG_REQUIRE(x_max != nullptr, "cpg_bn_relu_pool_fwd_xmax: null x_max");
+    return pool_fwd("cpg_bn_relu_pool_fwd_xmax", x, gamma, beta, eps, momentum, running_mean, running_var, mean, invstd, y_pooled, x_max, N,
+                    C, H, W, train, ws, ws_bytes, stream_v);
+}
+
+extern "C" int cpg_bn_relu_pool_bwd_xmax(const float *x, const float *g_pooled, const float *gamma, const float *beta,
+                                         const float *mean, const float *invstd, float *gx, float *dgamma, float *dbeta, int32_t N,
+                                         int32_t C, int32_t H, int32_t W, int32_t train, void *ws, size_t ws_bytes, void *stream_v,
+                                         const float *x_max) {
+    CPG_REQUIRE(x_max != nullptr, "cpg_bn_relu_pool_bwd_xmax: null x_max");
+    return pool_bwd("cpg_bn_relu_pool_bwd_xmax", x, x_max, g_pooled, gamma, beta, mean, invstd, gx, dgamma, dbeta, N, C, H, W, train, ws,
+                    ws_bytes, stream_v);
 }
 
 
diff --git a/cpg_amd/csrc/conv3x3_wino_wgrad.hip b/cpg_amd/csrc/conv3x3_wino_wgrad.hip
--- a/cpg_amd/csrc/conv3x3_wino_wgrad.hip
+++ b/cpg_amd/csrc/conv3x3_wino_wgrad.hip
@@ -24,6 +24,7 @@
     int xcd;
 };
 
+constexpr unsigned kWwContig = 0x80000000u;
 struct WwRider {
     const float *y, *gz;
     float *gy;
@@ -43,7 +44,7 @@
 __global__ __launch_bounds__(256) __attribute__((amdgpu_waves_per_eu(1, 1)))
 void k_wgw(WwGeom g, const float *__restrict__ x, const float *__restrict__ gy, float *__restrict__ part, WwRider rd) {
     static_assert(GS == 0 || GS == 4 || (!NARROW && GS == 2), "shared staging: groups of 4 waves, or 2 on wide maps");
-    static_assert(RI == 0 || (GS == 4 && RI <= 2), "the rider's schedule slots exist in the GS = 4 bodies: one or two items per stage");
+    static_assert(RI == 0 || (GS == 4 && RI <= 4), "the rider's schedule slots exist in the GS = 4 bodies: one or two items per stage");
     constexpr int NG = GS ? 4 / GS : 0;
     constexpr bool TS = GS == 4;
     constexpr int WW_BS = 2 * 16 * 64;
@@ -275,45 +276,81 @@
             B[(m - 3) * 4 + 0] = v[0], B[(m - 3) * 4 + 1] = v[1], B[(m - 3) * 4 + 2] = v[2], B[(m - 3) * 4 + 3] = v[3];
         }
     };
-    constexpr int RJ = RI > 0 ? RI : 1;
+    constexpr bool RV2 = RI > 2;
+    constexpr int RN = RV2 ? RI - 2 : RI;
+    constexpr int RJ = RN > 0 ? RN : 1, RS = RV2 ? 2 : 1;
     typedef const float __attribute__((address_space(4))) *ww_cptr;
     const __amdgpu_buffer_rsrc_t srd_ry = __builtin_amdgcn_make_buffer_rsrc((void *)rd.y, 0, rd.bytes, 0x00020000);
     const __amdgpu_buffer_rsrc_t srd_rz = __builtin_amdgcn_make_buffer_rsrc((void *)rd.gz, 0, rd.bytes, 0x00020000);
     const __amdgpu_buffer_rsrc_t srd_ro = __builtin_amdgcn_make_buffer_rsrc((void *)rd.gy, 0, rd.bytes, 0x00020000);
     unsigned rq = 0, rq_end = 0, r_plane = 0;
     int r_sub = 0, r_c = 0;
-    if constexpr (RI > 0) {
+    unsigned r_dq = 0;
+    int r_dr = 0, r_dc = 0;
+    unsigned r_step = 1;
+    if constexpr (RV2) {
+        const bool contig = (rd.per & kWwContig) != 0;
+        const unsigned n = rd.per & ~kWwContig;
+        r_step = contig ? 1u : n;
+        rq = __builtin_amdgcn_readfirstlane(min(contig ? u * n : u, rd.total));
+        rq_end = contig ? min(rq + n, rd.total) : rd.total;
+        r_dq = r_step / (unsigned)rd.ipp, r_dr = (int)(r_step % (unsigned)rd.ipp), r_dc = (int)(r_dq % (unsigned)rd.C);
+    } else if constexpr (RI > 0) {
         rq = __builtin_amdgcn_readfirstlane(min(u * rd.per, rd.total));
         rq_end = min(rq + rd.per, rd.total);
-        r_plane = rq / (unsigned)rd.ipp, r_sub = (int)(rq % (unsigned)rd.ipp), r_c = (int)(r_plane % (unsigned)rd.C);
     }
-    f32x4 r_y[RJ], r_z[RJ];
+    if constexpr (RI > 0) r_plane = rq / (unsigned)rd.ipp, r_sub = (int)(rq % (unsigned)rd.ipp), r_c = (int)(r_plane % (unsigned)rd.C);
+    f32x4 r_y[RS][RJ], r_z[RS][RJ];
     float r_t[RJ][7];
-    int r_vo[RJ], r_so[RJ];
-    auto r_micro = [&](int j, int m) {
+    int r_vo[RS][RJ], r_so[RJ], r_cs[RS][RJ];
+    auto r_table = [&](int j, int c) {
+        ww_cptr t = (ww_cptr)rd.table + c * 8;
+#pragma unroll
+        for (int k = 0; k < 7; ++k) r_t[j][k] = t[k];
+    };
+    auto r_micro = [&](int j, int m, int set) {
+        const int s = RV2 ? set : 0;
         if (m == 0) {
             const int left = rq < rq_end ? rd.p4 - r_sub * 64 : 0;
-            r_vo[j] = lane < left ? lane * 16 : kOOR;
-            r_so[j] = (int)(r_plane * (unsigned)rd.HW + (unsigned)r_sub * 256u) * 4;
-            r_y[j] = __builtin_bit_cast(f32x4, __builtin_amdgcn_raw_buffer_load_b128(srd_ry, r_vo[j], r_so[j], 0));
+            const int so = (int)(r_plane * (unsigned)rd.HW + (unsigned)r_sub * 256u) * 4;
+            if constexpr (RV2) {
+                r_vo[s][j] = lane < left ? lane * 16 + so : kOOR;
+            } else {
+                r_vo[s][j] = lane < left ? lane * 16 : kOOR;
+                r_so[j] = so;
+            }
+            r_y[s][j] = __builtin_bit_cast(f32x4, __builtin_amdgcn_raw_buffer_load_b128(srd_ry, r_vo[s][j], RV2 ? 0 : r_so[j], 0));
         } else if (m == 1) {
-            r_z[j] = __builtin_bit_cast(f32x4, __builtin_amdgcn_raw_buffer_load_b128(srd_rz, r_vo[j], r_so[j], 0));
-            ww_cptr t = (ww_cptr)rd.table + r_c * 8;
-#pragma unroll
-            for (int k = 0; k < 7; ++k) r_t[j][k] = t[k];
+            r_z[s][j] = __builtin_bit_cast(f32x4, __builtin_amdgcn_raw_buffer_load_b128(srd_rz, r_vo[s][j], RV2 ? 0 : r_so[j], 0));
+            if constexpr (RV2) r_cs[s][j] = r_c;
+            else r_table(j, r_c);
             if (rq < rq_end) {
-                ++rq;
-                if (++r_sub == rd.ipp) {
-                    r_sub = 0, ++r_plane;
-                    if (++r_c == rd.C) r_c = 0;
+                if constexpr (RV2) {
+                    rq += r_step;
+                    r_plane += r_dq, r_sub += r_dr, r_c += r_dc;
+                    if (r_sub >= rd.ipp) r_sub -= rd.ipp, ++r_plane, ++r_c;
+                    if (r_c >= rd.C) r_c -= rd.C;
+                } else {
+                    ++rq;
+                    if (++r_sub == rd.ipp) {
+                        r_sub = 0, ++r_plane;
+                        if (++r_c == rd.C) r_c = 0;
+                    }
                 }
             }
+        } else if (m == 6) {
+            if constexpr (RV2) r_table(j, r_cs[s][j]);
         } else {
             const int e = m - 2;
-            r_y[j][e] = bn_bwd_apply_one<true, true>(r_y[j][e], r_z[j][e], r_t[j][0], r_t[j][1], r_t[j][2], r_t[j][3], r_t[j][4], r_t[j][5], r_t[j][6]);
-            if (m == 5) __builtin_amdgcn_raw_buffer_store_b128(__builtin_bit_cast(i32x4, r_y[j]), srd_ro, r_vo[j], r_so[j], 0);
+            r_y[s][j][e] = bn_bwd_apply_one<true, true>(r_y[s][j][e], r_z[s][j][e], r_t[j][0], r_t[j][1], r_t[j][2], r_t[j][3], r_t[j][4],
+                                                        r_t[j][5], r_t[j][6]);
+            if (m == 5) __builtin_amdgcn_raw_buffer_store_b128(__builtin_bit_cast(i32x4, r_y[s][j]), srd_ro, r_vo[s][j], RV2 ? 0 : r_so[j], 0);
         }
     };
+    if constexpr (RV2) {
+#pragma unroll
+        for (int j = 0; j < RN; ++j) r_micro(j, 0, 0), r_micro(j, 1, 0);
+    }
     (void)r_micro;
     WW_STAMP(1);
     WACC_ZERO_ALL();
@@ -362,10 +399,10 @@
             WACC_MMA_9(A0[9], B0[9]); b_micro(4, 1, 1, B1, xb0); WACC_FENCE();
             WACC_MMA_10(A0[10], B0[10]); b_micro(5, 1, 1, B1, xb0); WACC_FENCE();
             WACC_MMA_11(A0[11], B0[11]); b_micro(6, 1, 1, B1, xb0); WACC_FENCE();
-            WACC_MMA_12(A0[12], B0[12]); if constexpr (RI > 0) r_micro(0, 0); WACC_FENCE();
-            WACC_MMA_13(A0[13], B0[13]); if constexpr (RI > 0) r_micro(0, 1); WACC_FENCE();
-            WACC_MMA_14(A0[14], B0[14]); if constexpr (RI > 1) r_micro(1, 0); WACC_FENCE();
-            WACC_MMA_15(A0[15], B0[15]); if constexpr (RI > 1) r_micro(1, 1); WACC_FENCE();
+            WACC_MMA_12(A0[12], B0[12]); if constexpr (RN > 0) r_micro(0, 0, 1); WACC_FENCE();
+            WACC_MMA_13(A0[13], B0[13]); if constexpr (RN > 0) r_micro(0, 1, 1), r_micro(0, 6, 0); WACC_FENCE();
+            WACC_MMA_14(A0[14], B0[14]); if constexpr (RN > 1) r_micro(1, 0, 1); WACC_FENCE();
+            WACC_MMA_15(A0[15], B0[15]); if constexpr (RN > 1) r_micro(1, 1, 1), r_micro(1, 6, 0); WACC_FENCE();
             WACC_MMA_0(A1[0], B1[0]); b_micro(0, 2, 0, B0, xb0); g_load_s(0); WACC_FENCE();
             WACC_MMA_1(A1[1], B1[1]); b_micro(1, 2, 0, B0, xb0); g_load_s(1); WACC_FENCE();
             WACC_MMA_2(A1[2], B1[2]); t_micro(4, 2, A0, B0, xb0); g_load_s(2); WACC_FENCE();
@@ -426,10 +463,10 @@
             WACC_MMA_9(A0[9], B0[9]); b_micro(4, 5, 1, B1, xb0); WACC_FENCE();
             WACC_MMA_10(A0[10], B0[10]); b_micro(5, 5, 1, B1, xb0); WACC_FENCE();
             WACC_MMA_11(A0[11], B0[11]); b_micro(6, 5, 1, B1, xb0); WACC_FENCE();
-            WACC_MMA_12(A0[12], B0[12]); if constexpr (RI > 0) r_micro(0, 2); WACC_FENCE();
-            WACC_MMA_13(A0[13], B0[13]); if constexpr (RI > 0) r_micro(0, 3); WACC_FENCE();
-            WACC_MMA_14(A0[14], B0[14]); if constexpr (RI > 0) r_micro(0, 4); WACC_FENCE();
-            WACC_MMA_15(A0[15], B0[15]); if constexpr (RI > 0) r_micro(0, 5); WACC_FENCE();
+            WACC_MMA_12(A0[12], B0[12]); if constexpr (RN > 0) r_micro(0, 2, 0); WACC_FENCE();
+            WACC_MMA_13(A0[13], B0[13]); if constexpr (RN > 0) r_micro(0, 3, 0); WACC_FENCE();
+            WACC_MMA_14(A0[14], B0[14]); if constexpr (RN > 0) r_micro(0, 4, 0); WACC_FENCE();
+            WACC_MMA_15(A0[15], B0[15]); if constexpr (RN > 0) r_micro(0, 5, 0); WACC_FENCE();
             WACC_MMA_0(A1[0], B1[0]); b_micro(0, 6, 0, B0, xb0); WACC_FENCE();
             WACC_MMA_1(A1[1], B1[1]); b_micro(1, 6, 0, B0, xb0); WACC_FENCE();
             WACC_MMA_2(A1[2], B1[2]); t_micro(4, 6, A0, B0, xb0); WACC_FENCE();
@@ -442,10 +479,10 @@
             WACC_MMA_9(A1[9], B1[9]); b_micro(4, 6, 0, B0, xb0); WACC_FENCE();
             WACC_MMA_10(A1[10], B1[10]); b_micro(5, 6, 0, B0, xb0); WACC_FENCE();
             WACC_MMA_11(A1[11], B1[11]); b_micro(6, 6, 0, B0, xb0); WACC_FENCE();
-            WACC_MMA_12(A1[12], B1[12]); if constexpr (RI > 1) r_micro(1, 2); WACC_FENCE();
-            WACC_MMA_13(A1[13], B1[13]); if constexpr (RI > 1) r_micro(1, 3); WACC_FENCE();
-            WACC_MMA_14(A1[14], B1[14]); if constexpr (RI > 1) r_micro(1, 4); WACC_FENCE();
-            WACC_MMA_15(A1[15], B1[15]); if constexpr (RI > 1) r_micro(1, 5); WACC_FENCE();
+            WACC_MMA_12(A1[12], B1[12]); if constexpr (RN > 1) r_micro(1, 2, 0); WACC_FENCE();
+            WACC_MMA_13(A1[13], B1[13]); if constexpr (RN > 1) r_micro(1, 3, 0); WACC_FENCE();
+            WACC_MMA_14(A1[14], B1[14]); if constexpr (RN > 1) r_micro(1, 4, 0); WACC_FENCE();
+            WACC_MMA_15(A1[15], B1[15]); if constexpr (RN > 1) r_micro(1, 5, 0); WACC_FENCE();
             WACC_MMA_0(A0[0], B0[0]); w_store_s(0, xb1); w_store_s(1, xb1); w_store_s(2, xb1); w_store_s(3, xb1); WACC_FENCE();
             WACC_MMA_1(A0[1], B0[1]); w_store_s(4, xb1); w_store_s(5, xb1); w_store_s(6, xb1); w_store_s(7, xb1); WACC_FENCE();
             WACC_MMA_2(A0[2], B0[2]); w_store_s(8, xb1); w_store_s(9, xb1); w_store_s(10, xb1); w_store_s(11, xb1); WACC_FENCE();
@@ -480,10 +517,10 @@
             WACC_MMA_9(A1[9], B1[9]); b_micro(4, 1, 0, B0, xb1); WACC_FENCE();
             WACC_MMA_10(A1[10], B1[10]); b_micro(5, 1, 0, B0, xb1); WACC_FENCE();
             WACC_MMA_11(A1[11], B1[11]); b_micro(6, 1, 0, B0, xb1); WACC_FENCE();
-            WACC_MMA_12(A1[12], B1[12]); if constexpr (RI > 0) r_micro(0, 0); WACC_FENCE();
-            WACC_MMA_13(A1[13], B1[13]); if constexpr (RI > 0) r_micro(0, 1); WACC_FENCE();
-            WACC_MMA_14(A1[14], B1[14]); if constexpr (RI > 1) r_micro(1, 0); WACC_FENCE();
-            WACC_MMA_15(A1[15], B1[15]); if constexpr (RI > 1) r_micro(1, 1); WACC_FENCE();
+            WACC_MMA_12(A1[12], B1[12]); if constexpr (RN > 0) r_micro(0, 0, 0); WACC_FENCE();
+            WACC_MMA_13(A1[13], B1[13]); if constexpr (RN > 0) r_micro(0, 1, 0), r_micro(0, 6, 1); WACC_FENCE();
+            WACC_MMA_14(A1[14], B1[14]); if constexpr (RN > 1) r_micro(1, 0, 0); WACC_FENCE();
+            WACC_MMA_15(A1[15], B1[15]); if constexpr (RN > 1) r_micro(1, 1, 0), r_micro(1, 6, 1); WACC_FENCE();
             WACC_MMA_0(A0[0], B0[0]); b_micro(0, 2, 1, B1, xb1); g_load_s(0); WACC_FENCE();
             WACC_MMA_1(A0[1], B0[1]); b_micro(1, 2, 1, B1, xb1); g_load_s(1); WACC_FENCE();
             WACC_MMA_2(A0[2], B0[2]); t_micro(4, 2, A1, B1, xb1); g_load_s(2); WACC_FENCE();
@@ -544,10 +581,10 @@
             WACC_MMA_9(A1[9], B1[9]); b_micro(4, 5, 0, B0, xb1); WACC_FENCE();
             WACC_MMA_10(A1[10], B1[10]); b_micro(5, 5, 0, B0, xb1); WACC_FENCE();
             WACC_MMA_11(A1[11], B1[11]); b_micro(6, 5, 0, B0, xb1); WACC_FENCE();
-            WACC_MMA_12(A1[12], B1[12]); if constexpr (RI > 0) r_micro(0, 2); WACC_FENCE();
-            WACC_MMA_13(A1[13], B1[13]); if constexpr (RI > 0) r_micro(0, 3); WACC_FENCE();
-            WACC_MMA_14(A1[14], B1[14]); if constexpr (RI > 0) r_micro(0, 4); WACC_FENCE();
-            WACC_MMA_15(A1[15], B1[15]); if constexpr (RI > 0) r_micro(0, 5); WACC_FENCE();
+            WACC_MMA_12(A1[12], B1[12]); if constexpr (RN > 0) r_micro(0, 2, 1); WACC_FENCE();
+            WACC_MMA_13(A1[13], B1[13]); if constexpr (RN > 0) r_micro(0, 3, 1); WACC_FENCE();
+            WACC_MMA_14(A1[14], B1[14]); if constexpr (RN > 0) r_micro(0, 4, 1); WACC_FENCE();
+            WACC_MMA_15(A1[15], B1[15]); if constexpr (RN > 0) r_micro(0, 5, 1); WACC_FENCE();
             WACC_MMA_0(A0[0], B0[0]); b_micro(0, 6, 1, B1, xb1); WACC_FENCE();
             WACC_MMA_1(A0[1], B0[1]); b_micro(1, 6, 1, B1, xb1); WACC_FENCE();
             WACC_MMA_2(A0[2], B0[2]); t_micro(4, 6, A1, B1, xb1); WACC_FENCE();
@@ -560,10 +597,10 @@
             WACC_MMA_9(A0[9], B0[9]); b_micro(4, 6, 1, B1, xb1); WACC_FENCE();
             WACC_MMA_10(A0[10], B0[10]); b_micro(5, 6, 1, B1, xb1); WACC_FENCE();
             WACC_MMA_11(A0[11], B0[11]); b_micro(6, 6, 1, B1, xb1); WACC_FENCE();
-            WACC_MMA_12(A0[12], B0[12]); if constexpr (RI > 1) r_micro(1, 2); WACC_FENCE();
-            WACC_MMA_13(A0[13], B0[13]); if constexpr (RI > 1) r_micro(1, 3); WACC_FENCE();
-            WACC_MMA_14(A0[14], B0[14]); if constexpr (RI > 1) r_micro(1, 4); WACC_FENCE();
-            WACC_MMA_15(A0[15], B0[15]); if constexpr (RI > 1) r_micro(1, 5); WACC_FENCE();
+            WACC_MMA_12(A0[12], B0[12]); if constexpr (RN > 1) r_micro(1, 2, 1); WACC_FENCE();
+            WACC_MMA_13(A0[13], B0[13]); if constexpr (RN > 1) r_micro(1, 3, 1); WACC_FENCE();
+            WACC_MMA_14(A0[14], B0[14]); if constexpr (RN > 1) r_micro(1, 4, 1); WACC_FENCE();
+            WACC_MMA_15(A0[15], B0[15]); if constexpr (RN > 1) r_micro(1, 5, 1); WACC_FENCE();
             WACC_MMA_0(A1[0], B1[0]); w_store_s(0, xb0); w_store_s(1, xb0); w_store_s(2, xb0); w_store_s(3, xb0); WACC_FENCE();
             WACC_MMA_1(A1[1], B1[1]); w_store_s(4, xb0); w_store_s(5, xb0); w_store_s(6, xb0); w_store_s(7, xb0); WACC_FENCE();
             WACC_MMA_2(A1[2], B1[2]); w_store_s(8, xb0); w_store_s(9, xb0); w_store_s(10, xb0); w_store_s(11, xb0); WACC_FENCE();
@@ -836,10 +873,10 @@
             WACC_MMA_9(A0[9], B0[9]); b_micro(4, 1, 1, B1, xb0); WACC_FENCE();
             WACC_MMA_10(A0[10], B0[10]); b_micro(5, 1, 1, B1, xb0); WACC_FENCE();
             WACC_MMA_11(A0[11], B0[11]); b_micro(6, 1, 1, B1, xb0); WACC_FENCE();
-            WACC_MMA_12(A0[12], B0[12]); if constexpr (RI > 0) r_micro(0, 0); WACC_FENCE();
-            WACC_MMA_13(A0[13], B0[13]); if constexpr (RI > 0) r_micro(0, 1); WACC_FENCE();
-            WACC_MMA_14(A0[14], B0[14]); if constexpr (RI > 1) r_micro(1, 0); WACC_FENCE();
-            WACC_MMA_15(A0[15], B0[15]); if constexpr (RI > 1) r_micro(1, 1); WACC_FENCE();
+            WACC_MMA_12(A0[12], B0[12]); if constexpr (RN > 0) r_micro(0, 0, 1); WACC_FENCE();
+            WACC_MMA_13(A0[13], B0[13]); if constexpr (RN > 0) r_micro(0, 1, 1), r_micro(0, 6, 0); WACC_FENCE();
+            WACC_MMA_14(A0[14], B0[14]); if constexpr (RN > 1) r_micro(1, 0, 1); WACC_FENCE();
+            WACC_MMA_15(A0[15], B0[15]); if constexpr (RN > 1) r_micro(1, 1, 1), r_micro(1, 6, 0); WACC_FENCE();
             WACC_MMA_0(A1[0], B1[0]); b_micro(0, 2, 0, B0, xb0); g_load_s(0); WACC_FENCE();
             WACC_MMA_1(A1[1], B1[1]); b_micro(1, 2, 0, B0, xb0); g_load_s(1); WACC_FENCE();
             WACC_MMA_2(A1[2], B1[2]); t_micro(4, 2, A0, B0, xb0); g_load_s(2); WACC_FENCE();
@@ -900,10 +937,10 @@
             WACC_MMA_9(A0[9], B0[9]); b_micro(4, 5, 1, B1, xb0); WACC_FENCE();
             WACC_MMA_10(A0[10], B0[10]); b_micro(5, 5, 1, B1, xb0); WACC_FENCE();
             WACC_MMA_11(A0[11], B0[11]); b_micro(6, 5, 1, B1, xb0); WACC_FENCE();
-            WACC_MMA_12(A0[12], B0[12]); if constexpr (RI > 0) r_micro(0, 2); WACC_FENCE();
-            WACC_MMA_13(A0[13], B0[13]); if constexpr (RI > 0) r_micro(0, 3); WACC_FENCE();
-            WACC_MMA_14(A0[14], B0[14]); if constexpr (RI > 0) r_micro(0, 4); WACC_FENCE();
-            WACC_MMA_15(A0[15], B0[15]); if constexpr (RI > 0) r_micro(0, 5); WACC_FENCE();
+            WACC_MMA_12(A0[12], B0[12]); if constexpr (RN > 0) r_micro(0, 2, 0); WACC_FENCE();
+            WACC_MMA_13(A0[13], B0[13]); if constexpr (RN > 0) r_micro(0, 3, 0); WACC_FENCE();
+            WACC_MMA_14(A0[14], B0[14]); if constexpr (RN > 0) r_micro(0, 4, 0); WACC_FENCE();
+            WACC_MMA_15(A0[15], B0[15]); if constexpr (RN > 0) r_micro(0, 5, 0); WACC_FENCE();
             WACC_MMA_0(A1[0], B1[0]); b_micro(0, 6, 0, B0, xb0); WACC_FENCE();
             WACC_MMA_1(A1[1], B1[1]); b_micro(1, 6, 0, B0, xb0); WACC_FENCE();
             WACC_MMA_2(A1[2], B1[2]); t_micro(4, 6, A0, B0, xb0); WACC_FENCE();
@@ -916,10 +953,10 @@
             WACC_MMA_9(A1[9], B1[9]); b_micro(4, 6, 0, B0, xb0); WACC_FENCE();
             WACC_MMA_10(A1[10], B1[10]); b_micro(5, 6, 0, B0, xb0); WACC_FENCE();
             WACC_MMA_11(A1[11], B1[11]); b_micro(6, 6, 0, B0, xb0); WACC_FENCE();
-            WACC_MMA_12(A1[12], B1[12]); if constexpr (RI > 1) r_micro(1, 2); WACC_FENCE();
-            WACC_MMA_13(A1[13], B1[13]); if constexpr (RI > 1) r_micro(1, 3); WACC_FENCE();
-            WACC_MMA_14(A1[14], B1[14]); if constexpr (RI > 1) r_micro(1, 4); WACC_FENCE();
-            WACC_MMA_15(A1[15], B1[15]); if constexpr (RI > 1) r_micro(1, 5); WACC_FENCE();
+            WACC_MMA_12(A1[12], B1[12]); if constexpr (RN > 1) r_micro(1, 2, 0); WACC_FENCE();
+            WACC_MMA_13(A1[13], B1[13]); if constexpr (RN > 1) r_micro(1, 3, 0); WACC_FENCE();
+            WACC_MMA_14(A1[14], B1[14]); if constexpr (RN > 1) r_micro(1, 4, 0); WACC_FENCE();
+            WACC_MMA_15(A1[15], B1[15]); if constexpr (RN > 1) r_micro(1, 5, 0); WACC_FENCE();
             WACC_MMA_0(A0[0], B0[0]); w_store_s(0, xb1); w_store_s(1, xb1); w_store_s(2, xb1); WACC_FENCE();
             WACC_MMA_1(A0[1], B0[1]); w_store_s(3, xb1); w_store_s(4, xb1); WACC_FENCE();
             WACC_MMA_2(A0[2], B0[2]); w_store_s(5, xb1); w_store_s(6, xb1); WACC_FENCE();
@@ -954,10 +991,10 @@
             WACC_MMA_9(A1[9], B1[9]); b_micro(4, 1, 0, B0, xb1); WACC_FENCE();
             WACC_MMA_10(A1[10], B1[10]); b_micro(5, 1, 0, B0, xb1); WACC_FENCE();
             WACC_MMA_11(A1[11], B1[11]); b_micro(6, 1, 0, B0, xb1); WACC_FENCE();
-            WACC_MMA_12(A1[12], B1[12]); if constexpr (RI > 0) r_micro(0, 0); WACC_FENCE();
-            WACC_MMA_13(A1[13], B1[13]); if constexpr (RI > 0) r_micro(0, 1); WACC_FENCE();
-            WACC_MMA_14(A1[14], B1[14]); if constexpr (RI > 1) r_micro(1, 0); WACC_FENCE();
-            WACC_MMA_15(A1[15], B1[15]); if constexpr (RI > 1) r_micro(1, 1); WACC_FENCE();
+            WACC_MMA_12(A1[12], B1[12]); if constexpr (RN > 0) r_micro(0, 0, 0); WACC_FENCE();
+            WACC_MMA_13(A1[13], B1[13]); if constexpr (RN > 0) r_micro(0, 1, 0), r_micro(0, 6, 1); WACC_FENCE();
+            WACC_MMA_14(A1[14], B1[14]); if constexpr (RN > 1) r_micro(1, 0, 0); WACC_FENCE();
+            WACC_MMA_15(A1[15], B1[15]); if constexpr (RN > 1) r_micro(1, 1, 0), r_micro(1, 6, 1); WACC_FENCE();
             WACC_MMA_0(A0[0], B0[0]); b_micro(0, 2, 1, B1, xb1); g_load_s(0); WACC_FENCE();
             WACC_MMA_1(A0[1], B0[1]); b_micro(1, 2, 1, B1, xb1); g_load_s(1); WACC_FENCE();
             WACC_MMA_2(A0[2], B0[2]); t_micro(4, 2, A1, B1, xb1); g_load_s(2); WACC_FENCE();
@@ -1018,10 +1055,10 @@
             WACC_MMA_9(A1[9], B1[9]); b_micro(4, 5, 0, B0, xb1); WACC_FENCE();
             WACC_MMA_10(A1[10], B1[10]); b_micro(5, 5, 0, B0, xb1); WACC_FENCE();
             WACC_MMA_11(A1[11], B1[11]); b_micro(6, 5, 0, B0, xb1); WACC_FENCE();
-            WACC_MMA_12(A1[12], B1[12]); if constexpr (RI > 0) r_micro(0, 2); WACC_FENCE();
-            WACC_MMA_13(A1[13], B1[13]); if constexpr (RI > 0) r_micro(0, 3); WACC_FENCE();
-            WACC_MMA_14(A1[14], B1[14]); if constexpr (RI > 0) r_micro(0, 4); WACC_FENCE();
-            WACC_MMA_15(A1[15], B1[15]); if constexpr (RI > 0) r_micro(0, 5); WACC_FENCE();
+            WACC_MMA_12(A1[12], B1[12]); if constexpr (RN > 0) r_micro(0, 2, 1); WACC_FENCE();
+            WACC_MMA_13(A1[13], B1[13]); if constexpr (RN > 0) r_micro(0, 3, 1); WACC_FENCE();
+            WACC_MMA_14(A1[14], B1[14]); if constexpr (RN > 0) r_micro(0, 4, 1); WACC_FENCE();
+            WACC_MMA_15(A1[15], B1[15]); if constexpr (RN > 0) r_micro(0, 5, 1); WACC_FENCE();
             WACC_MMA_0(A0[0], B0[0]); b_micro(0, 6, 1, B1, xb1); WACC_FENCE();
             WACC_MMA_1(A0[1], B0[1]); b_micro(1, 6, 1, B1, xb1); WACC_FENCE();
             WACC_MMA_2(A0[2], B0[2]); t_micro(4, 6, A1, B1, xb1); WACC_FENCE();
@@ -1034,10 +1071,10 @@
             WACC_MMA_9(A0[9], B0[9]); b_micro(4, 6, 1, B1, xb1); WACC_FENCE();
             WACC_MMA_10(A0[10], B0[10]); b_micro(5, 6, 1, B1, xb1); WACC_FENCE();
             WACC_MMA_11(A0[11], B0[11]); b_micro(6, 6, 1, B1, xb1); WACC_FENCE();
-            WACC_MMA_12(A0[12], B0[12]); if constexpr (RI > 1) r_micro(1, 2); WACC_FENCE();
-            WACC_MMA_13(A0[13], B0[13]); if constexpr (RI > 1) r_micro(1, 3); WACC_FENCE();
-            WACC_MMA_14(A0[14], B0[14]); if constexpr (RI > 1) r_micro(1, 4); WACC_FENCE();
-            WACC_MMA_15(A0[15], B0[15]); if constexpr (RI > 1) r_micro(1, 5); WACC_FENCE();
+            WACC_MMA_12(A0[12], B0[12]); if constexpr (RN > 1) r_micro(1, 2, 1); WACC_FENCE();
+            WACC_MMA_13(A0[13], B0[13]); if constexpr (RN > 1) r_micro(1, 3, 1); WACC_FENCE();
+            WACC_MMA_14(A0[14], B0[14]); if constexpr (RN > 1) r_micro(1, 4, 1); WACC_FENCE();
+            WACC_MMA_15(A0[15], B0[15]); if constexpr (RN > 1) r_micro(1, 5, 1); WACC_FENCE();
             WACC_MMA_0(A1[0], B1[0]); w_store_s(0, xb0); w_store_s(1, xb0); w_store_s(2, xb0); WACC_FENCE();
             WACC_MMA_1(A1[1], B1[1]); w_store_s(3, xb0); w_store_s(4, xb0); WACC_FENCE();
             WACC_MMA_2(A1[2], B1[2]); w_store_s(5, xb0); w_store_s(6, xb0); WACC_FENCE();
@@ -1535,10 +1572,28 @@
     }
 
     WW_STAMP(3);
+    if constexpr (RV2) {
+        if (nst & 1) {
+#pragma unroll
+            for (int j = 0; j < RN; ++j) {
+                r_micro(j, 6, 1);
+#pragma unroll
+                for (int m = 2; m < 6; ++m) r_micro(j, m, 1);
+            }
+        } else {
+#pragma unroll
+            for (int j = 0; j < RN; ++j) {
+                r_micro(j, 6, 0);
+#pragma unroll
+                for (int m = 2; m < 6; ++m) r_micro(j, m, 0);
+            }
+        }
+    }
     if constexpr (RI > 0) {
         while (rq < rq_end) {
+            r_micro(0, 0, 0), r_micro(0, 1, 0), r_micro(0, 6, 0);
 #pragma unroll
-            for (int m = 0; m < 6; ++m) r_micro(0, m);
+            for (int m = 2; m < 6; ++m) r_micro(0, m, 0);
         }
     }
     WACC_DRAIN();
@@ -1637,8 +1692,12 @@
     const int64_t total = (int64_t)r.N * r.C * rd.ipp, waves = (int64_t)p.g.nkb * p.g.ncb * p.g.nsplit;
     if (waves % 4 != 0 || (waves + 3) / 4 != p.blocks) return false;
     rd.total = (unsigned)total;
-    rd.per = (unsigned)((total + waves - 1) / waves);
-    ri = rd.per <= p.g.su ? 1 : 2;
+    const unsigned each = (unsigned)((total + waves - 1) / waves);
+    ri = each <= p.g.su ? 1 : 2;
+    const int mode = opt_or(OPT_WW_RIDER_V1, 1);
+    if (mode == 0) rd.per = (unsigned)waves, ri += 2;
+    else if (mode == 2) rd.per = kWwContig | each, ri += 2;
+    else rd.per = each;
     return true;
 }
 
@@ -1680,7 +1739,15 @@
             return fail(CPG_E_INVALID, "cpg_conv2d_wgrad(winograd): the rider's result may not alias its inputs or the weight gradient's");
     }
     const dim3 grid((unsigned)p.blocks), block(256);
-    if (p.narrow && ri == 2)
+    if (p.narrow && ri == 4)
+        hipLaunchKernelGGL((k_wgw<true, 4, 4>), grid, block, 0, stream, p.g, x, gy, (float *)ws, rd);
+    else if (p.narrow && ri == 3)
+        hipLaunchKernelGGL((k_wgw<true, 4, 3>), grid, block, 0, stream, p.g, x, gy, (float *)ws, rd);
+    else if (ri == 4)
+        hipLaunchKernelGGL((k_wgw<false, 4, 4>), grid, block, 0, stream, p.g, x, gy, (float *)ws, rd);
+    else if (ri == 3)
+        hipLaunchKernelGGL((k_wgw<false, 4, 3>), grid, block, 0, stream, p.g, x, gy, (float *)ws, rd);
+    else if (p.narrow && ri == 2)
         hipLaunchKernelGGL((k_wgw<true, 4, 2>), grid, block, 0, stream, p.g, x, gy, (float *)ws, rd);
     else if (p.narrow && ri == 1)
         hipLaunchKernelGGL((k_wgw<true, 4, 1>), grid, block, 0, stream, p.g, x, gy, (float *)ws, rd);
diff --git a/cpg_amd/csrc/cpg_common.cpp b/cpg_amd/csrc/cpg_common.cpp
--- a/cpg_amd/csrc/cpg_common.cpp
+++ b/cpg_amd/csrc/cpg_common.cpp
@@ -53,6 +53,7 @@
     {"CPG_WINO_GRIDS", INT},        {"CPG_WW_UNITS", INT},         {"CPG_WW_XCD", INT},            {"CPG_PW_TILE", INT},           {"CPG_WG3_SHARE", INT},
     {"CPG_WW_SHARE", INT},          {"CPG_WINO_TAIL", INT},         {"CPG_FC_SMALL", INT},
     {"CPG_NO_WW_RIDER", BOOL},      {"CPG_NO_GROUPED", BOOL},       {"CPG_GROUPED_WIDE_MIN", INT},
+    {"CPG_WW_RIDER_V1", INT},
 };
 
 struct Table {
diff --git a/cpg_amd/csrc/cpg_common.h b/cpg_amd/csrc/cpg_common.h
--- a/cpg_amd/csrc/cpg_common.h
+++ b/cpg_amd/csrc/cpg_common.h
@@ -42,6 +42,7 @@
     OPT_NO_WW_RIDER,
     OPT_NO_GROUPED,
     OPT_GROUPED_WIDE_MIN,
+    OPT_WW_RIDER_V1,
     OPT_COUNT
 };
 constexpr int OPT_UNSET = INT32_MIN;
diff --git a/cpg_amd/models/fused_bn.py b/cpg_amd/models/fused_bn.py
--- a/cpg_amd/models/fused_bn.py
+++ b/cpg_amd/models/fused_bn.py
@@ -1,4 +1,5 @@
 import ctypes
+import os
 
 import torch
 import torch.nn as nn
@@ -13,6 +14,7 @@
 FUSE_STEM = True
 FUSE_STEM_WGRAD = True
 FUSE_SKIP_ADD = True
+POOL_XMAX = os.environ.get('CPG_NO_POOL_XMAX', '0') in ('', '0')
 
 
 def _batch_stats(stats, nbt, N, C, HW, eps, momentum, running_mean, running_var, training, device):
@@ -144,7 +146,8 @@
 
 
 def _pool_backward(name, ctx, gp):
-    x, gamma, beta, mean, invstd = ctx.saved_tensors
+    x, gamma, beta, mean, invstd = ctx.saved_tensors[:5]
+    tail = tuple(_lib.dptr(t) for t in ctx.saved_tensors[5:])
     N, C, H, W = x.shape
     gp = gp.contiguous()
     gx = torch.empty_like(x)
@@ -152,7 +155,7 @@
     ws, nb = _lib.workspace(_lib.lib().cpg_bn_workspace_bytes(N, C, H * W), x.device)
     _lib.call(name, _lib.dptr(x), _lib.dptr(gp, name='grad_output'), _lib.dptr(gamma), _lib.dptr(beta), _lib.dptr(mean),
               _lib.dptr(invstd), _lib.dptr(gx), _lib.dptr(dgamma), _lib.dptr(dbeta), N, C, H, W, int(ctx.training), _lib.dptr(ws), nb,
-              _lib.stream_ptr())
+              _lib.stream_ptr(), *tail)
     return (gx, dgamma, dbeta) + (None,) * 7
 
 
@@ -167,18 +170,22 @@
         compute_stats = training and stats is None
         mean, invstd, nbt = _batch_stats(stats, nbt, N, C, H * W, eps, momentum, running_mean, running_var, training, x.device)
         ws, nb = _lib.workspace(L.cpg_bn_workspace_bytes(N, C, H * W), x.device)
-        _lib.call('cpg_bn_relu_pool_fwd', _lib.dptr(x, name='input'), _lib.dptr(gamma, name='bn.weight'), _lib.dptr(beta, name='bn.bias'),
+        saved = (training and POOL_XMAX and any(ctx.needs_input_grad) and hasattr(L, 'cpg_bn_relu_pool_fwd_xmax')
+                 and hasattr(L, 'cpg_bn_relu_pool_bwd_xmax'))
+        x_max = (torch.empty_like(y),) if saved else ()
+        _lib.call('cpg_bn_relu_pool_fwd_xmax' if saved else 'cpg_bn_relu_pool_fwd', _lib.dptr(x, name='input'),
+                  _lib.dptr(gamma, name='bn.weight'), _lib.dptr(beta, name='bn.bias'),
                   float(eps), float(momentum), _lib.dptr(running_mean if compute_stats else None),
                   _lib.dptr(running_var if compute_stats else None), _lib.dptr(mean), _lib.dptr(invstd),
-                  _lib.dptr(y), N, C, H, W, int(compute_stats), _lib.dptr(ws), nb, _lib.stream_ptr())
+                  _lib.dptr(y), N, C, H, W, int(compute_stats), _lib.dptr(ws), nb, _lib.stream_ptr(), *(_lib.dptr(t) for t in x_max))
         _count(nbt)
-        ctx.save_for_backward(x, gamma, beta, mean, invstd)
+        ctx.save_for_backward(x, gamma, beta, mean, invstd, *x_max)
         ctx.training = bool(training)
         return y
 
     @staticmethod
     def backward(ctx, gp):
-        return _pool_backward('cpg_bn_relu_pool_bwd', ctx, gp)
+        return _pool_backward('cpg_bn_relu_pool_bwd_xmax' if len(ctx.saved_tensors) > 5 else 'cpg_bn_relu_pool_bwd', ctx, gp)
 
 
 class _BnReluPool3Fn(torch.autograd.Function):
diff --git a/include/cpg_hip.h b/include/cpg_hip.h
--- a/include/cpg_hip.h
+++ b/include/cpg_hip.h
@@ -225,6 +225,15 @@
                          const float *mean, const float *invstd, float *gx, float *dgamma, float *dbeta,
                          int32_t N, int32_t C, int32_t H, int32_t W, int32_t train, void *ws, size_t ws_bytes,
                          void *stream);
+
+int cpg_bn_relu_pool_fwd_xmax(const float *x, const float *gamma, const float *beta, float eps, float momentum,
+                              float *running_mean, float *running_var, float *mean, float *invstd, float *y_pooled,
+                              int32_t N, int32_t C, int32_t H, int32_t W, int32_t train, void *ws, size_t ws_bytes,
+                              void *stream, float *x_max);
+int cpg_bn_relu_pool_bwd_xmax(const float *x, const float *g_pooled, const float *gamma, const float *beta,
+                              const float *mean, const float *invstd, float *gx, float *dgamma, float *dbeta,
+                              int32_t N, int32_t C, int32_t H, int32_t W, int32_t train, void *ws, size_t ws_bytes,
+                              void *stream, const float *x_max);
 
 int32_t cpg_bn_relu_pool3_supported(int32_t H, int32_t W);
 int cpg_bn_relu_pool3_fwd(const float *x, const float *gamma, const float *beta, const float *mean, const float *invstd,
```
